# tangent-T/FACL

Measured on AMD Instinct MI355X. Metric: contrastive-step clips/sec (B=32,T=24,N=2048) at 1/2/4/8 MI355X, higher is better.
Workload: dtype f32

## Files before the change

### facl_amd/_lib.py

```python
import ctypes
import os

import torch

_HERE = os.path.dirname(os.path.abspath(__file__))
_LIB = None

c_p = ctypes.c_void_p
c_i = ctypes.c_int
c_f = ctypes.c_float
c_d = ctypes.c_double
c_l = ctypes.c_longlong

SIGNATURES = {
    "facl_version": [],
    "facl_fps_f32": [c_p, c_i, c_i, c_i, c_i, c_p, c_p, c_p],
    "facl_fps_f64": [c_p, c_i, c_i, c_i, c_i, c_p, c_p, c_p],
    "facl_fps_reorder": [c_p, c_i, c_i, c_i, c_p, c_i, c_p, c_p],
    "facl_group": [c_p, c_i, c_i, c_i, c_i, c_i, c_f, c_p, c_p, c_p, c_p],
    "facl_group_clips": [c_p, c_i, c_i, c_i, c_i, c_i, c_i, c_f, c_p, c_p, c_p, c_p],
    "facl_gather_rows": [c_p, c_i, c_i, c_i, c_i, c_p, c_i, c_p, c_p, c_i, c_i, c_p],
    "facl_scatter_rows": [c_p, c_i, c_i, c_i, c_i, c_i, c_p, c_i, c_p, c_p],
    "facl_sinkhorn": [c_p, c_i, c_i, c_i, c_p, c_p, c_p],
    "facl_kmeans": [c_p, c_i, c_i, c_i, c_i, c_p, c_p, c_p, c_p],
# ... 68 lines not shown
    "facl_build_views_resident_gp_f32": [c_p, c_p, c_p, c_i, c_p, c_i, c_i, c_i, c_l, c_i, c_p, c_p, c_p, c_p],
    "facl_build_views_resident_gp_f64": [c_p, c_p, c_p, c_i, c_p, c_i, c_i, c_i, c_l, c_i, c_p, c_p, c_p, c_p],
    "facl_sa_bwd0": [c_p, c_p, c_l, c_p, c_p, c_p, c_p, c_p],
    "facl_sa_bwd1": [c_p, c_l, c_p, c_p, c_p, c_p, c_p, c_p, c_p, c_p, c_p, c_p, c_p],
    "facl_sa_bwd_w3": [c_p, c_l, c_p, c_p, c_p, c_p, c_p, c_p, c_p],
    "facl_sa_bwd2": [c_p, c_p, c_p, c_l, c_i, c_p, c_p, c_p, c_p, c_p, c_p, c_p],
    "facl_sa_bwd_consts3": [c_p, c_p, c_p, c_p, c_d, c_p, c_p, c_p],
    "facl_sa_bwd_consts2": [c_p, c_p, c_d, c_p, c_p],
    "facl_bn_bwd_consts": [c_p, c_p, c_i, c_d, c_p, c_p, c_p, c_p],
    "facl_rows_center_wgrad": [c_p, c_p, c_l, c_i, c_p, c_p, c_p],
    "facl_viewmax_fwd": [c_p, c_i, c_i, c_i, c_p, c_p, c_p],
    "facl_viewmax_bwd": [c_p, c_p, c_i, c_i, c_i, c_p, c_p],
    "facl_viewmax_bwd_add": [c_p, c_p, c_i, c_i, c_i, c_p, c_p],
    "facl_sa_bwd_final": [c_p] * 13 + [c_i, c_d] + [c_p] * 9 + [c_p],
    "facl_viewmax_stack": [c_p, c_i, c_i, c_i, c_p, c_p, c_p],
    "facl_fc_bn_stats": [c_p, c_l, c_l, c_i, c_p, c_p, c_p],
    "facl_fc_bn_apply": [c_p, c_l, c_l, c_i, c_p, c_p, c_i, c_i, c_d, c_d, c_p, c_p, c_f, c_f, c_p, c_p, c_p, c_p, c_p],
    "facl_fc_bn_bwd_stats": [c_p, c_p, c_l, c_l, c_i, c_p, c_p, c_p, c_p],
    "facl_fc_bn_bwd_apply": [c_p, c_p, c_l, c_l, c_i, c_p, c_p, c_p, c_d, c_d, c_p, c_p, c_p, c_p, c_p],
    "facl_col_sums": [c_p, c_l, c_i, c_p, c_p],
    "facl_contrast_pair_sum": [c_p, c_i, c_i, c_i, c_i, c_p, c_i, c_p, c_p, c_p, c_p, c_p],
    "facl_gemm_wgrad_acc": [c_p, c_p, c_l, c_i, c_i, c_i, c_p, c_i, c_p],
    "facl_contrast_pair_sum_mask": [c_p, c_i, c_i, c_i, c_i, c_p, c_i, c_i, c_p, c_p, c_p, c_p, c_p],
    "facl_loss_rows_fwd": [c_p, c_l, c_i, c_i, c_f, c_p, c_p, c_p],
    "facl_loss_rows_bwd": [c_p, c_p, c_p, c_l, c_i, c_i, c_f, c_p, c_p],
    "facl_contrast_pair_queue": [c_p, c_p, c_i, c_i, c_i, c_i, c_i, c_p, c_i, c_i, c_p, c_p, c_p, c_p, c_p, c_p, c_p],
    "facl_queue_push": [c_p, c_i, c_i, c_p, c_i, c_p, c_p],
    "facl_ema_apply": [c_i, c_p, c_p, c_p, c_f, c_p],
    "facl_grad_sqnorm": [c_i, c_p, c_p, c_p, c_p],
    "facl_adam_prep_ex": [c_p, c_p, c_f, c_f, c_p, c_i, c_d, c_i, c_i, c_i, c_d, c_p, c_p],
    "facl_adamw_apply": [c_i, c_p, c_p, c_p, c_p, c_p, c_p, c_p, c_f, c_f, c_f, c_f, c_p],
    "facl_mailbox_bytes": [c_i, c_i],
    "facl_mailbox_alloc": [c_l, c_p, c_p],
    "facl_mailbox_open": [c_p, c_p],
    "facl_mailbox_close": [c_p],
    "facl_mailbox_free": [c_p],
    "facl_mailbox_allreduce": [c_p, c_p, c_i, c_i, c_p, c_i, c_i, c_p, c_p, c_p],
    "facl_gen3dv_frames": [c_p, c_i, c_i, c_i, c_p, c_p, c_p, c_p],
    "facl_gen3dv_voxelise": [c_p, c_i, c_i, c_i, c_p, c_p, c_p, c_p, c_i, c_i, c_i, c_l, c_l, c_d, c_p, c_p, c_p, c_p, c_p],
    "facl_gen3dv_volumes": [c_p, c_p, c_p, c_p, c_i, c_i, c_l, c_p, c_p, c_p],
    "facl_gen3dv_filter": [c_p, c_p, c_p, c_i, c_i, c_l, c_i, c_i, c_p, c_p, c_p],
    "facl_gen3dv_compact": [c_p, c_p, c_p, c_p, c_i, c_i, c_l, c_p, c_p, c_p],
    "facl_gen3dv_sample": [c_p, c_p, c_p, c_p, c_p, c_i, c_i, c_l, c_p, c_l, c_i, c_p, c_p, c_p, c_p, c_p, c_p],
    "facl_gen3dv_app": [c_p, c_i, c_i, c_i, c_p, c_p, c_p, c_l, c_p, c_i, c_p, c_l, c_i, c_p, c_p, c_p, c_i, c_i, c_l, c_d,
                        c_p, c_p, c_p, c_p, c_p],
    "facl_knn_ws_bytes": [c_i, c_i, c_i],
    "facl_knn_topk": [c_p, c_i, c_i, c_p, c_i, c_i, c_i, c_i, c_p, c_p, c_p, c_p, c_p],
    "facl_knn_vote": [c_p, c_p, c_p, c_i, c_i, c_i, c_i, c_f, c_p, c_p, c_p],
    "facl_cls_gather_norm_fwd": [c_p, c_i, c_i, c_i, c_p, c_p, c_p],
    "facl_cls_gather_norm_bwd": [c_p, c_p, c_p, c_i, c_i, c_i, c_p, c_p],
    "facl_softmax_ce": [c_p, c_i, c_p, c_i, c_i, c_p, c_p, c_p, c_p, c_p],
    "facl_cls_probs_acc": [c_p, c_i, c_i, c_i, c_p, c_i, c_p],
    "facl_cls_topk": [c_p, c_i, c_i, c_i, c_i, c_p, c_p, c_p, c_p, c_p],
}
RESTYPE_I64 = {"facl_ws_bytes", "facl_gemm_rs_planes_bytes", "facl_mailbox_bytes", "facl_knn_ws_bytes"}


def lib_path():
    return os.environ.get("FACL_LIB") or os.path.join(_HERE, "libfacl_hip.so")


def load_library():
    global _LIB
    if _LIB is not None:
        return _LIB
    path = lib_path()
    if not os.path.exists(path):
        raise RuntimeError(
            f"{path} not found: facl_amd has no CPU/eager fallback. Build it with "
            "`python -m facl_amd.build` (hipcc --offload-arch=gfx950).")
    lib = ctypes.CDLL(path)
    for name, argtypes in SIGNATURES.items():
        fn = getattr(lib, name)
        fn.argtypes = argtypes
        fn.restype = ctypes.c_longlong if name in RESTYPE_I64 else ctypes.c_int
    _LIB = lib
    return lib


_ERR = {-1: "unsupported shape", -2: "NULL pointer", -3: "misaligned pointer", -4: "unsupported configuration"}


def check(rc, what):
    if rc != 0:
        msg = _ERR.get(rc, f"hipError {rc}")
        raise RuntimeError(f"{what} failed: {msg} (code {rc})")


AMAX_WORDS = 2048

SA_D_MIN, SA_D_MAX = 3, 8


def sa_l1_cols(D):
    return 8 if D <= 4 else 12


def sa_bwd2_out(D):
    return 64 * 64 + 64 * sa_l1_cols(D)


def amax_buffers(n, device, zero=True):
    if zero:
        return torch.zeros((n, AMAX_WORDS), dtype=torch.int32, device=device)
    return empty((n, AMAX_WORDS), dtype=torch.int32, device=device)


def ptr(t):
# ... 145 lines not shown
```

### facl_amd/cn3d_model_conbag.py

```python
import math

import torch
import torch.nn as nn

from . import sa_mlp
from . import tail as _tail

nstates_plus_1 = [64, 64, 256]
nstates_plus_2 = [128, 128, 256]
nstates_plus_3 = [256, 512, 1024, 1024, 1024]


class _Affine(nn.Module):

    def __init__(self, shape, fan_in, bias=True):
        super().__init__()
        self.weight = nn.Parameter(torch.empty(shape))
        nn.init.kaiming_uniform_(self.weight, a=math.sqrt(5))
        if bias:
            self.bias = nn.Parameter(torch.empty(shape[0]))
            bound = 1 / math.sqrt(fan_in) if fan_in > 0 else 0
            nn.init.uniform_(self.bias, -bound, bound)
        else:
            self.register_parameter("bias", None)
# ... 65 lines not shown
        if self.pooling == "concatenation":
            self.dim_out = 1024
        self._pool_K = _knn_K
        self._pool_S = self.sample_num_level2 if _sample_num_level1 is None else _sample_num_level1

        self.net3DV_1 = _conv_stack(self.INPUT_FEATURE_NUM, nstates_plus_1)
        self.net3DV_3 = _conv_stack(3 + nstates_plus_2[2], nstates_plus_3[:3])
        self.netR_FC = _Slots([(0, _Affine((nstates_plus_3[4], self.dim_out), self.dim_out)),
                               (1, _BatchNormState(nstates_plus_3[4])),
                               (3, _Affine((self.dim, nstates_plus_3[4]), nstates_plus_3[4]))])
        self.mapping = _Affine((self.num_clusters, self.dim), self.dim, bias=False)
        self.bn_reduce_fn = None

    def _sa_args(self):
        n = self.net3DV_1
        params = [n[0].weight, n[0].bias, n[1].weight, n[1].bias, n[3].weight, n[3].bias, n[4].weight, n[4].bias,
                  n[6].weight, n[6].bias, n[7].weight, n[7].bias]
        buffers = {"rm1": n[1].running_mean, "rv1": n[1].running_var, "rm2": n[4].running_mean,
                   "rv2": n[4].running_var, "rm3": n[7].running_mean, "rv3": n[7].running_var}
        return params, buffers

    def forward(self, xt, yt, loss_mode=0):
        if xt.dim() != 4 or yt.dim() != 4:
            raise ValueError("expected xt (M,D,S,K) and yt (M,3,S,1)")
        M, D, S, K = xt.shape
        if D != self.INPUT_FEATURE_NUM:
            raise RuntimeError("input has %d channels, model was built for %d" % (D, self.INPUT_FEATURE_NUM))
        if K != self._pool_K:
            raise RuntimeError("pooling window is %d neighbours, got K=%d" % (self._pool_K, K))
        if S != self._pool_S:
            raise RuntimeError("model pools over %d centroids, got S=%d" % (self._pool_S, S))
        if M % self.gost:
            raise RuntimeError("first dim (%d) must be gost*batch with gost=%d" % (M, self.gost))
        x_rows = xt.permute(0, 2, 3, 1)
        x_rows = x_rows.contiguous().view(M * S * K, D).float()
        centers = yt.permute(0, 2, 1, 3).reshape(M * S, 3)
        training = self.training

        params, buffers = self._sa_args()
        prec = getattr(self, "precision", "f32")
        state = dict(training=training, buffers=buffers, reduce_fn=self.bn_reduce_fn, K=K, precision=prec)
        pooled = sa_mlp.SAMLPFunction.apply(x_rows, state, *params)
        if training:
            for i in (1, 4, 7):
                self.net3DV_1[i].count_batch()
        with _tail.precision(prec):
            return self._tail_forward(pooled, centers, M, S, training, state.get("pooled_amax"))

    def _tail_forward(self, pooled, centers, M, S, training, pooled_amax=None):

        n3 = self.net3DV_3
        widths = (n3[0].weight.shape[1] - 3, n3[0].weight.shape[0], n3[3].weight.shape[0], n3[6].weight.shape[0])
        if _tail.net3dv3_supported(pooled.shape[0], widths, S, _tail.current_precision()):
            x_pre = _tail.net3dv3(pooled, centers, n3, training, S, self.bn_reduce_fn, pooled_amax)
        else:
            h = _tail.linear_bn_relu(pooled, n3[0], n3[1], training, self.bn_reduce_fn, centers=centers)
            h = _tail.linear_bn_relu(h, n3[3], n3[4], training, self.bn_reduce_fn)
            x_pre = _tail.linear_bn_relu_segmax(h, n3[6], n3[7], training, S, self.bn_reduce_fn)
        fc = self.netR_FC
        stacked = _tail.fc_head(x_pre, self.gost, fc[0], fc[1], fc[3], training, self.bn_reduce_fn)
        self._stacked = stacked
        x, x_global = stacked[:M], stacked[M:]
        x_nor, code = _tail.normalize_map(x, self.mapping.weight, lazy=bool(getattr(self, "lazy_code", False)))
        return x, code, x_nor, x_global


class PointNet_Plus_fine(PointNet_Plus):

    def __init__(self, opt, num_clusters=64, gost=10, dim=512, sample_num_level1=32, knn_K=128,
                 normalize_input=True):
        super().__init__(opt, num_clusters=num_clusters, gost=gost, dim=dim, normalize_input=normalize_input,
                         _sample_num_level1=sample_num_level1, _knn_K=knn_K)
```

### facl_amd/csrc/common.h

```cpp
#pragma once
#include <hip/hip_runtime.h>
#include <stdint.h>
#include <stdlib.h>
#include "../../include/facl_hip.h"

#define FACL_WAVE 64

static inline int facl_launch_status() {
    hipError_t e = hipGetLastError();
    return e == hipSuccess ? 0 : (int)e;
}

static inline int facl_env_int(const char* name, int dflt) {
    const char* v = getenv(name);
    return v ? atoi(v) : dflt;
}

static inline int facl_set_dynamic_lds(bool (&done)[64], const void* const* fns, int nfns, int bytes) {
    int dev = 0;
    if (hipGetDevice(&dev) != hipSuccess || dev < 0 || dev >= 64) dev = 0;
    if (done[dev]) return 0;
    for (int i = 0; i < nfns; ++i) {
        hipError_t e = hipFuncSetAttribute(fns[i], hipFuncAttributeMaxDynamicSharedMemorySize, bytes);
        if (e != hipSuccess) return (int)e;
// ... 50 lines not shown

__device__ __forceinline__ double wave_sum_f64(double v) {
#pragma unroll
    for (int o = 32; o > 0; o >>= 1) v += __shfl_xor(v, o, 64);
    return v;
}

typedef float f32x16 __attribute__((ext_vector_type(16)));
typedef float f32x32 __attribute__((ext_vector_type(32)));
#define MFMA32(a, b, c) __builtin_amdgcn_mfma_f32_32x32x2f32((a), (b), (c), 0, 0, 0)
__device__ __forceinline__ constexpr int rowmap(int r, int h) { return (r & 3) + 8 * (r >> 2) + 4 * h; }

#define FACL_UNIT 64
#define FACL_UNIT_ELEMS 4096

template <int D>
__device__ __forceinline__ float l1_chain(const float4* row, const float (&xv)[8]) {
    const float4 w0 = row[0], w1 = row[1];
    const float w[8] = {w0.x, w0.y, w0.z, w0.w, w1.x, w1.y, w1.z, w1.w};
    float v = fmaf(w[0], xv[0], row[2].x);
#pragma unroll
    for (int i = 1; i < D; ++i) v = fmaf(w[i], xv[i], v);
    return v;
}

#define FACL_WS_ROWS 4096
#define FACL_WS_TICKET_BYTES 4096

typedef __bf16 bf16x8 __attribute__((ext_vector_type(8)));
typedef __bf16 bf16x2v __attribute__((ext_vector_type(2)));
typedef float f32x2v __attribute__((ext_vector_type(2)));
#define MFMA_BF16(a, b, c) __builtin_amdgcn_mfma_f32_32x32x16_bf16((a), (b), (c), 0, 0, 0)
#define FACL_SB_PA {2, 0, 1, 1, 0, 0}
#define FACL_SB_PB {0, 2, 1, 0, 1, 0}
#define FACL_SB3_PA {0, 1, 0}
#define FACL_SB3_PB {1, 0, 0}

__device__ __forceinline__ unsigned pk_bf16(float x0, float x1) {
    const f32x2v v = {x0, x1};
    return __builtin_bit_cast(unsigned, __builtin_convertvector(v, bf16x2v));
}
__device__ __forceinline__ float sub_f32(float a, float b) {
    float d;
    asm("v_sub_f32 %0, %1, %2" : "=v"(d) : "v"(a), "v"(b));
    return d;
}
__device__ __forceinline__ void split_pair(float x0, float x1, unsigned& hi, unsigned& mi, unsigned& lo) {
    hi = pk_bf16(x0, x1);
    const float r0 = sub_f32(x0, __builtin_bit_cast(float, hi << 16)), r1 = sub_f32(x1, __builtin_bit_cast(float, hi & 0xffff0000u));
    mi = pk_bf16(r0, r1);
    const float s0 = sub_f32(r0, __builtin_bit_cast(float, mi << 16)), s1 = sub_f32(r1, __builtin_bit_cast(float, mi & 0xffff0000u));
    lo = pk_bf16(s0, s1);
}
__device__ __forceinline__ bf16x8 as_bf16x8(unsigned a, unsigned b, unsigned c, unsigned d) {
    const uint4 u = make_uint4(a, b, c, d);
    return __builtin_bit_cast(bf16x8, u);
}

typedef _Float16 f16x8h __attribute__((ext_vector_type(8)));
typedef _Float16 f16x2h __attribute__((ext_vector_type(2)));
#define MFMA_F16(a, b, c) __builtin_amdgcn_mfma_f32_32x32x16_f16((a), (b), (c), 0, 0, 0)
#define FACL_H3_PA {1, 0, 0}
#define FACL_H3_PB {0, 1, 0}
#define FACL_AMAX_SLOTS 64
#define FACL_AMAX_STRIDE 32
static_assert(FACL_AMAX_SLOTS * FACL_AMAX_STRIDE == FACL_AMAX_WORDS, "amax buffer layout");

__device__ __forceinline__ void split_pair_h(float x0, float x1, unsigned& hi, unsigned& lo) {
    const f32x2v v = {x0, x1};
    const f16x2h h = __builtin_convertvector(v, f16x2h);
    hi = __builtin_bit_cast(unsigned, h);
    float r0, r1;
    asm("v_fma_mix_f32 %0, %1, -1.0, %2 op_sel:[0,0,0] op_sel_hi:[1,0,0]" : "=v"(r0) : "v"(hi), "v"(x0));
    asm("v_fma_mix_f32 %0, %1, -1.0, %2 op_sel:[1,0,0] op_sel_hi:[1,0,0]" : "=v"(r1) : "v"(hi), "v"(x1));
    const f32x2v r = {r0, r1};
    lo = __builtin_bit_cast(unsigned, __builtin_convertvector(r, f16x2h));
}
__device__ __forceinline__ f16x8h as_f16x8(unsigned a, unsigned b, unsigned c, unsigned d) {
    const uint4 u = make_uint4(a, b, c, d);
    return __builtin_bit_cast(f16x8h, u);
}

__device__ __forceinline__ int h3_se(unsigned b) {
    int se = 267 - (int)((b >> 23) & 0xff);
    se = se > 167 ? 167 : se;
    return se < 87 ? 87 : se;
}
__device__ __forceinline__ int h3_se_wide(unsigned b) {
    int se = 267 - (int)((b >> 23) & 0xff);
    se = se > 207 ? 207 : se;
    return se < 47 ? 47 : se;
}
__device__ __forceinline__ float pow2_biased(int e) { return __uint_as_float((unsigned)e << 23); }
template <int CTRL, int RMASK>
__device__ __forceinline__ float facl_dpp_max_step(float v) {
    const int o = __builtin_amdgcn_update_dpp(__builtin_bit_cast(int, v), __builtin_bit_cast(int, v), CTRL, RMASK, 0xf, false);
    return fmaxf(v, __builtin_bit_cast(float, o));
}
__device__ __forceinline__ float facl_wave_max_nonneg(float v) {
    v = facl_dpp_max_step<0x111, 0xf>(v); v = facl_dpp_max_step<0x112, 0xf>(v); v = facl_dpp_max_step<0x114, 0xf>(v);
    v = facl_dpp_max_step<0x118, 0xf>(v); v = facl_dpp_max_step<0x142, 0xa>(v); v = facl_dpp_max_step<0x143, 0xc>(v);
    return __builtin_bit_cast(float, __builtin_amdgcn_readlane(__builtin_bit_cast(int, v), 63));
}

__device__ __forceinline__ float h3_unscale(int seA, int seB) { return pow2_biased(381 - seA - seB); }
__device__ __forceinline__ unsigned amax_bits(const unsigned* amax) {
// ... 21 lines not shown
```

### facl_amd/csrc/fchead.hip

```cpp
#include "rows_common.h"

namespace {

constexpr int FC_SL = 32;

__device__ __forceinline__ void fc_slice(int s, int M, int R, int na, int& r0, int& r1, int& seg) {
    if (s < na) { seg = 0; r0 = s * FC_SL; r1 = r0 + FC_SL < M ? r0 + FC_SL : M; }
    else { seg = 1; r0 = M + (s - na) * FC_SL; r1 = r0 + FC_SL < R ? r0 + FC_SL : R; }
    if (r0 > r1) r0 = r1;
}

__global__ __launch_bounds__(256) void k_fc_stats(const float* __restrict__ y, int M, int R, int na, int C4,
                                                  double* __restrict__ part) {
    const int lane = threadIdx.x & 63, ph = threadIdx.x >> 6;
    const int c4 = blockIdx.x * 64 + lane;
    __shared__ double red[3][64][8];
    int r0, r1, seg;
    fc_slice(blockIdx.y, M, R, na, r0, r1, seg);
    double acc[8] = {};
    if (c4 < C4)
        for (int r = r0 + ph; r < r1; r += 4)
            lane_each<4>([&](int e, float v) { acc[2 * e] += (double)v; acc[2 * e + 1] += (double)v * (double)v; },
                         reinterpret_cast<const float4*>(y)[(size_t)r * C4 + c4]);
    if (phase_sum(acc, red, lane, ph, c4 < C4)) {
// ... 4 lines not shown
}

__global__ void k_fc_reduce(const double* __restrict__ part, int na, int nb, int V, double* __restrict__ sums2) {
    const int v = blockIdx.x * blockDim.x + threadIdx.x;
    if (v >= V) return;
    double a = 0, b = 0;
    for (int s = 0; s < na; ++s) a += part[(size_t)s * V + v];
    for (int s = na; s < na + nb; ++s) b += part[(size_t)s * V + v];
    sums2[v] = a;
    sums2[V + v] = b;
}

__device__ __forceinline__ void fc_slice_sums(const double* __restrict__ part, int na, int nb, int C, int c, int ph, double (&acc)[4]) {
    const int V = 2 * C;
    if (c >= C) return;
    for (int t = ph; t < na; t += 4) { acc[0] += part[(size_t)t * V + 2 * c]; acc[1] += part[(size_t)t * V + 2 * c + 1]; }
    for (int t = na + ph; t < na + nb; t += 4) { acc[2] += part[(size_t)t * V + 2 * c]; acc[3] += part[(size_t)t * V + 2 * c + 1]; }
}

__global__ __launch_bounds__(256) void k_fc_finalize(const double* __restrict__ part, int na, int nb, int C, double count_a,
                                                     double count_b, const float* __restrict__ gamma, const float* __restrict__ beta,
                                                     float eps, float momentum, float* __restrict__ running_mean,
                                                     float* __restrict__ running_var, float* __restrict__ bnc2) {
    const int lane = threadIdx.x & 63, ph = threadIdx.x >> 6;
    const int c = blockIdx.x * 64 + lane;
    __shared__ double red[3][64][4];
    double acc[4] = {};
    fc_slice_sums(part, na, nb, C, c, ph, acc);
    if (!phase_sum(acc, red, lane, ph, c < C)) return;
    const double g = gamma[c], b = beta[c];
    float rm = running_mean ? running_mean[c] : 0.f, rv = running_var ? running_var[c] : 0.f;
#pragma unroll
    for (int seg = 0; seg < 2; ++seg) {
        const double s = acc[2 * seg], q = acc[2 * seg + 1];
        const double count = seg ? count_b : count_a;
        const double mean = s / count;
        double var = q / count - mean * mean;
        if (var < 0) var = 0;
        const double invstd = 1.0 / sqrt(var + (double)eps);
        float* o = bnc2 + (size_t)seg * 5 * C;
        o[c] = (float)mean;
        o[C + c] = (float)invstd;
        o[2 * C + c] = (float)(g * invstd);
        o[3 * C + c] = (float)(b - mean * g * invstd);
        o[4 * C + c] = g < 0 ? -1.0f : 1.0f;
        const double unb = count > 1 ? var * count / (count - 1) : var;
        rm = (float)((1.0 - momentum) * rm + momentum * mean);
        rv = (float)((1.0 - momentum) * rv + momentum * unb);
    }
    if (running_mean) { running_mean[c] = rm; running_var[c] = rv; }
}

__global__ __launch_bounds__(256) void k_fc_apply(const float* __restrict__ y, int M, int R, int C4,
                                                  const float* __restrict__ bnc2, float* __restrict__ out) {
    const int c4 = blockIdx.x * 256 + threadIdx.x;
    if (c4 >= C4) return;
    const int C = 4 * C4;
    const float4 sa = reinterpret_cast<const float4*>(bnc2 + 2 * C)[c4], ta = reinterpret_cast<const float4*>(bnc2 + 3 * C)[c4];
    const float4 sb = reinterpret_cast<const float4*>(bnc2 + 7 * C)[c4], tb = reinterpret_cast<const float4*>(bnc2 + 8 * C)[c4];
    for (int r = blockIdx.y; r < R; r += gridDim.y) {
        const float4 sc = r < M ? sa : sb, sh = r < M ? ta : tb;
        reinterpret_cast<float4*>(out)[(size_t)r * C4 + c4] = lane_map<4>(bn_relu, sc, reinterpret_cast<const float4*>(y)[(size_t)r * C4 + c4], sh);
    }
}

__global__ __launch_bounds__(256) void k_fc_bwd_stats(const float* __restrict__ dout, const float* __restrict__ y, int M, int R,
                                                      int na, int C4, const float* __restrict__ bnc2, double* __restrict__ part) {
    const int lane = threadIdx.x & 63, ph = threadIdx.x >> 6;
    const int c4 = blockIdx.x * 64 + lane;
    __shared__ double red[3][64][8];
    int r0, r1, seg;
    fc_slice(blockIdx.y, M, R, na, r0, r1, seg);
    double acc[8] = {};
    if (c4 < C4) bn_bwd_stats_rows<4>(dout, y, C4, c4, bnc2 + (size_t)seg * 20 * C4, r0 + ph, r1, 4, acc);
    if (phase_sum(acc, red, lane, ph, c4 < C4)) {
        double* pr = part + (size_t)blockIdx.y * 8 * C4 + 8 * c4;
#pragma unroll
        for (int e = 0; e < 8; ++e) pr[e] = acc[e];
    }
}

__global__ __launch_bounds__(256) void k_fc_bwd_consts(const double* __restrict__ part, int na, int nb,
                                                       const double* __restrict__ sums_g, int C, double count_a, double count_b,
                                                       float* __restrict__ dbeta, float* __restrict__ dgamma,
                                                       float* __restrict__ kk2) {
    const int lane = threadIdx.x & 63, ph = threadIdx.x >> 6;
    const int c = blockIdx.x * 64 + lane;
    const int V = 2 * C;
    __shared__ double red[3][64][4];
    double acc[4] = {};
    fc_slice_sums(part, na, nb, C, c, ph, acc);
    if (!phase_sum(acc, red, lane, ph, c < C)) return;
#pragma unroll
    for (int seg = 0; seg < 2; ++seg) {
        const double g0 = sums_g ? sums_g[(size_t)seg * V + 2 * c] : acc[2 * seg];
        const double g1 = sums_g ? sums_g[(size_t)seg * V + 2 * c + 1] : acc[2 * seg + 1];
        const float inv = (float)(1.0 / (seg ? count_b : count_a));
        kk2[(size_t)seg * V + c] = (float)g0 * inv;
        kk2[(size_t)seg * V + C + c] = (float)g1 * inv;
    }
    dbeta[c] = (float)acc[0] + (float)acc[2];
    dgamma[c] = (float)acc[1] + (float)acc[3];
}

__global__ __launch_bounds__(256) void k_fc_bwd_apply(const float* __restrict__ dout, const float* __restrict__ y, int M, int R,
                                                      int C4, const float* __restrict__ bnc2, const float* __restrict__ kk2,
                                                      float* __restrict__ dy) {
    const int c4 = blockIdx.x * 256 + threadIdx.x;
    if (c4 >= C4) return;
    const int C = 4 * C4;
    const BnLanes<4> q[2] = {bn_lanes<4>(bnc2, C, c4), bn_lanes<4>(bnc2 + 5 * C, C, c4)};
    const KkLanes<4> k[2] = {kk_lanes<4>(kk2, C, c4), kk_lanes<4>(kk2 + 2 * C, C, c4)};
    for (int r = blockIdx.y; r < R; r += gridDim.y) {
        const int s = r < M ? 0 : 1;
        const size_t o = (size_t)r * C4 + c4;
        reinterpret_cast<float4*>(dy)[o] = lane_map<4>(bn_relu_bwd, reinterpret_cast<const float4*>(dout)[o], reinterpret_cast<const float4*>(y)[o],
                                                       q[s].mean, q[s].inv, q[s].scale, q[s].shift, k[s].k1, k[s].k2);
    }
}

__global__ __launch_bounds__(1024) void k_col_sums(const float* __restrict__ x, int R, int C4, float* __restrict__ out) {
    __shared__ double red[64][16][4];
    const int qd = threadIdx.x & 15, ph = threadIdx.x >> 4;
    const int c4 = blockIdx.x * 16 + qd;
    double a0 = 0, a1 = 0, a2 = 0, a3 = 0;
    if (c4 < C4)
        for (int r = ph; r < R; r += 64) {
            const float4 v = reinterpret_cast<const float4*>(x)[(size_t)r * C4 + c4];
            a0 += (double)v.x; a1 += (double)v.y; a2 += (double)v.z; a3 += (double)v.w;
        }
    red[ph][qd][0] = a0; red[ph][qd][1] = a1; red[ph][qd][2] = a2; red[ph][qd][3] = a3;
    __syncthreads();
    if (ph < 8) {
#pragma unroll
        for (int e = 0; e < 4; ++e) {
            double t = red[ph][qd][e];
#pragma unroll
            for (int k = 1; k < 8; ++k) t += red[ph + 8 * k][qd][e];
            red[ph][qd][e] = t;
        }
    }
    __syncthreads();
    if (ph == 0 && c4 < C4) {
        float o[4];
#pragma unroll
        for (int e = 0; e < 4; ++e) {
            double t = red[0][qd][e];
#pragma unroll
            for (int k = 1; k < 8; ++k) t += red[k][qd][e];
            o[e] = (float)t;
        }
        reinterpret_cast<float4*>(out)[c4] = make_float4(o[0], o[1], o[2], o[3]);
    }
}

__global__ __launch_bounds__(256) void k_viewmax_stack(const float* __restrict__ x, int G, int B, int C4, float* __restrict__ h,
                                                       int* __restrict__ arg) {
    __shared__ float4 sb[3][64];
    __shared__ int4 si[3][64];
    const int it = threadIdx.x & 63, ph = threadIdx.x >> 6;
    const int i = blockIdx.x * 64 + it;
    const bool live = i < B * C4;
    const int b = live ? i / C4 : 0, c4 = live ? i - b * C4 : 0;
    const int per = (G + 3) >> 2;
    const int g0 = ph * per, g1 = g0 + per < G ? g0 + per : G;
    float4 best = make_float4(0.f, 0.f, 0.f, 0.f);
    int4 bi = make_int4(-1, -1, -1, -1);
    if (live && g0 < g1) {
        const size_t o0 = ((size_t)g0 * B + b) * C4 + c4;
        best = reinterpret_cast<const float4*>(x)[o0];
        reinterpret_cast<float4*>(h)[o0] = best;
        bi = make_int4(g0, g0, g0, g0);
        for (int g = g0 + 1; g < g1; ++g) {
            const size_t o = ((size_t)g * B + b) * C4 + c4;
            const float4 v = reinterpret_cast<const float4*>(x)[o];
            reinterpret_cast<float4*>(h)[o] = v;
            first_max_wins(best, bi, v, g);
        }
    }
    if (ph) { sb[ph - 1][it] = best; si[ph - 1][it] = bi; }
    __syncthreads();
    if (ph == 0 && live) {
#pragma unroll
        for (int t = 0; t < 3; ++t) {
            const float4 v = sb[t][it];
            const int4 vi = si[t][it];
            if (vi.x < 0) continue;
            first_max_wins(best, bi, v, vi);
        }
        reinterpret_cast<float4*>(h)[((size_t)G * B + b) * C4 + c4] = best;
        reinterpret_cast<int4*>(arg)[i] = bi;
    }
}

inline bool fc_shape_ok(int64_t M, int64_t R, int C) {
    return M >= FC_SL && !(M % FC_SL) && R > M && R <= 0x7fffffff && C >= 4 && !(C & 3);
}
inline int fc_na(int64_t M) { return (int)(M / FC_SL); }
inline int fc_nb(int64_t M, int64_t R) { return (int)((R - M + FC_SL - 1) / FC_SL); }

}

extern "C" int64_t facl_ws_bytes(void);

extern "C" int facl_fc_bn_stats(const float* y, int64_t M, int64_t R, int C, double* sums2, void* ws, void* stream) {
    if (!y || !ws) return FACL_E_NULL;
    if (!fc_shape_ok(M, R, C)) return FACL_E_CONFIG;
    if (!aligned16(y)) return FACL_E_ALIGN;
    const int na = fc_na(M), nb = fc_nb(M, R);
    if ((size_t)(na + nb) * 2 * C * sizeof(double) > (size_t)facl_ws_bytes()) return FACL_E_CONFIG;
    hipStream_t st = (hipStream_t)stream;
    hipLaunchKernelGGL(k_fc_stats, dim3((C / 4 + 63) / 64, na + nb), dim3(256), 0, st, y, (int)M, (int)R, na, C / 4, (double*)ws);
    if (sums2) hipLaunchKernelGGL(k_fc_reduce, dim3((2 * C + 255) / 256), dim3(256), 0, st, (const double*)ws, na, nb, 2 * C, sums2);
    return facl_launch_status();
}

extern "C" int facl_fc_bn_apply(const float* y, int64_t M, int64_t R, int C, const double* sums2, const double* part,
                                int nslices_a, int nslices_b, double count_a, double count_b, const float* gamma,
                                const float* beta, float eps, float momentum, float* running_mean, float* running_var,
                                float* bnc2, float* a, void* stream) {
    if (!y || !gamma || !beta || !bnc2 || !a || (!sums2 && !part)) return FACL_E_NULL;
    if (M < 1 || R <= M || R > 0x7fffffff || C < 4 || (C & 3) || count_a < 1 || count_b < 1) return FACL_E_SHAPE;
    if (!sums2 && (nslices_a < 1 || nslices_b < 1)) return FACL_E_SHAPE;
    if (!aligned16(y, a, bnc2)) return FACL_E_ALIGN;
    hipStream_t st = (hipStream_t)stream;
    hipLaunchKernelGGL(k_fc_finalize, dim3((C + 63) / 64), dim3(256), 0, st, sums2 ? sums2 : part, sums2 ? 1 : nslices_a,
                       sums2 ? 1 : nslices_b, C, count_a, count_b, gamma, beta, eps, momentum, running_mean, running_var, bnc2);
    const int gx = (C / 4 + 255) / 256;
    int gy = 1024 / gx;
    if (gy > R) gy = (int)R;
    hipLaunchKernelGGL(k_fc_apply, dim3(gx, gy), dim3(256), 0, st, y, (int)M, (int)R, C / 4, bnc2, a);
    return facl_launch_status();
}

extern "C" int facl_fc_bn_bwd_stats(const float* dact, const float* y, int64_t M, int64_t R, int C, const float* bnc2,
                                    double* sums2, void* ws, void* stream) {
    if (!dact || !y || !bnc2 || !ws) return FACL_E_NULL;
    if (!fc_shape_ok(M, R, C)) return FACL_E_CONFIG;
    if (!aligned16(y, dact, bnc2)) return FACL_E_ALIGN;
    const int na = fc_na(M), nb = fc_nb(M, R);
    if ((size_t)(na + nb) * 2 * C * sizeof(double) > (size_t)facl_ws_bytes()) return FACL_E_CONFIG;
    hipStream_t st = (hipStream_t)stream;
    hipLaunchKernelGGL(k_fc_bwd_stats, dim3((C / 4 + 63) / 64, na + nb), dim3(256), 0, st, dact, y, (int)M, (int)R, na, C / 4, bnc2,
                       (double*)ws);
    if (sums2) hipLaunchKernelGGL(k_fc_reduce, dim3((2 * C + 255) / 256), dim3(256), 0, st, (const double*)ws, na, nb, 2 * C, sums2);
    return facl_launch_status();
}

extern "C" int facl_fc_bn_bwd_apply(const float* dact, const float* y, int64_t M, int64_t R, int C, const float* bnc2,
                                    const double* sums2_g, const void* ws, double count_a, double count_b, float* dgamma,
                                    float* dbeta, float* kk2, float* dy, void* stream) {
    if (!dact || !y || !bnc2 || !ws || !dgamma || !dbeta || !kk2 || !dy) return FACL_E_NULL;
    if (!fc_shape_ok(M, R, C)) return FACL_E_CONFIG;
    if (count_a < 1 || count_b < 1) return FACL_E_SHAPE;
    if (!aligned16(y, dact, bnc2, kk2, dy)) return FACL_E_ALIGN;
    const int na = fc_na(M), nb = fc_nb(M, R);
    hipStream_t st = (hipStream_t)stream;
    hipLaunchKernelGGL(k_fc_bwd_consts, dim3((C + 63) / 64), dim3(256), 0, st, (const double*)ws, na, nb, sums2_g, C, count_a,
                       count_b, dbeta, dgamma, kk2);
    const int gx = (C / 4 + 255) / 256;
    int gy = 1024 / gx;
    if (gy > R) gy = (int)R;
    hipLaunchKernelGGL(k_fc_bwd_apply, dim3(gx, gy), dim3(256), 0, st, dact, y, (int)M, (int)R, C / 4, bnc2, kk2, dy);
    return facl_launch_status();
}

extern "C" int facl_col_sums(const float* x, int64_t R, int C, float* out, void* stream) {
    if (!x || !out) return FACL_E_NULL;
    if (R < 1 || R > 0x7fffffff || C < 4 || (C & 3)) return FACL_E_SHAPE;
    if (!aligned16(x, out)) return FACL_E_ALIGN;
    hipLaunchKernelGGL(k_col_sums, dim3((C / 4 + 15) / 16), dim3(1024), 0, (hipStream_t)stream, x, (int)R, C / 4, out);
    return facl_launch_status();
}

extern "C" int facl_viewmax_stack(const float* x, int G, int B, int C, float* h, int32_t* arg, void* stream) {
    if (!x || !h || !arg) return FACL_E_NULL;
    if (G < 1 || B < 1 || C < 4 || (C & 3)) return FACL_E_SHAPE;
    if (!aligned16(x, h, arg)) return FACL_E_ALIGN;
    const int n = B * (C / 4);
    hipLaunchKernelGGL(k_viewmax_stack, dim3((n + 63) / 64), dim3(256), 0, (hipStream_t)stream, x, G, B, C / 4, h, arg);
    return facl_launch_status();
}
```

### facl_amd/csrc/gemm.hip

```cpp
#include "common.h"

int facl_reduce_rows(const double* part, int rows, int V, double* out, hipStream_t st);

namespace {

constexpr int BK = 32;
constexpr int LDK = BK + 4;
enum { KC = 0, IC = 1 };

struct GemmArgs {
    const float* A = nullptr; int lda = 0;
    const float* B = nullptr; int ldb = 0;
    float* C = nullptr; int ldc = 0;
    int MI = 0, NJ = 0, KK = 0;
    const float* bias = nullptr;
    const float* pscale = nullptr; const float* pshift = nullptr;
    const float* xa = nullptr; const float* xb = nullptr; int ldxb = 0;
    double* part = nullptr;
    int kchunk = 0;
    const float* sgn = nullptr; float* smax = nullptr; int* sarg = nullptr;
    int prec = 0;
    const unsigned* amax = nullptr;
    const unsigned* amax_b = nullptr;
    int accum = 0;
};

template <int LAY, int T>
__device__ __forceinline__ void load_tile(const float* __restrict__ P, int ld, int idx0, int nidx, int k0, int kend,
                                          float4 (&r)[2 * T], int tid) {
    if (LAY == IC) {
#pragma unroll
        for (int i = 0; i < 2 * T; ++i) {
            const int k = k0 + tid / (16 * T) + (16 / T) * i, idx = idx0 + 4 * (tid % (16 * T));
            if (k < kend && idx + 3 < nidx) r[i] = *reinterpret_cast<const float4*>(P + (size_t)k * ld + idx);
            else {
                float t[4];
#pragma unroll
                for (int e = 0; e < 4; ++e) t[e] = (k < kend && idx + e < nidx) ? P[(size_t)k * ld + idx + e] : 0.f;
                r[i] = make_float4(t[0], t[1], t[2], t[3]);
            }
        }
    } else {
#pragma unroll
        for (int i = 0; i < 2 * T; ++i) {
            const int idx = idx0 + (tid >> 3) + 32 * i, k = k0 + 4 * (tid & 7);
            if (idx < nidx && k + 3 < kend) r[i] = *reinterpret_cast<const float4*>(P + (size_t)idx * ld + k);
            else {
                float t[4];
#pragma unroll
                for (int e = 0; e < 4; ++e) t[e] = (idx < nidx && k + e < kend) ? P[(size_t)idx * ld + k + e] : 0.f;
                r[i] = make_float4(t[0], t[1], t[2], t[3]);
            }
        }
    }
}

template <int LAY, bool PRO, int TT>
__device__ __forceinline__ void store_tile(float* __restrict__ T, const float4 (&r)[2 * TT], int tid, int k0,
                                           const float* __restrict__ ps, const float* __restrict__ pt) {
    constexpr int LDT = 64 * TT + 4;
    if (LAY == IC) {
#pragma unroll
        for (int i = 0; i < 2 * TT; ++i) {
            const int k = tid / (16 * TT) + (16 / TT) * i;
            *reinterpret_cast<float4*>(&T[k * LDT + 4 * (tid % (16 * TT))]) = r[i];
        }
    } else {
#pragma unroll
        for (int i = 0; i < 2 * TT; ++i) {
            const int k = 4 * (tid & 7), il = (tid >> 3) + 32 * i;
            float v[4] = {r[i].x, r[i].y, r[i].z, r[i].w};
            if (PRO) {
                const float4 s = *reinterpret_cast<const float4*>(ps + k0 + k);
                const float4 t = *reinterpret_cast<const float4*>(pt + k0 + k);
                v[0] = relu_nan(fmaf(s.x, v[0], t.x)); v[1] = relu_nan(fmaf(s.y, v[1], t.y));
                v[2] = relu_nan(fmaf(s.z, v[2], t.z)); v[3] = relu_nan(fmaf(s.w, v[3], t.w));
            }
// ... 417 lines not shown
        }
}
template <int T, int NP>
__device__ __forceinline__ void write_tile_ic8(unsigned short* __restrict__ S, const unsigned (&pk)[12 * T], int tid) {
    constexpr int PLANE = 64 * T * SBROW;
    const int il = tid % (64 * T), kc = tid / (64 * T);
#pragma unroll
    for (int i = 0; i < T; ++i) {
        unsigned short* d = S + il * SBROW + 8 * (kc + (4 / T) * i);
#pragma unroll
        for (int p = 0; p < (NP == 4 ? 2 : NP); ++p)
            *reinterpret_cast<uint4*>(d + p * PLANE) =
                make_uint4(pk[12 * i + 4 * p], pk[12 * i + 4 * p + 1], pk[12 * i + 4 * p + 2], pk[12 * i + 4 * p + 3]);
    }
}

template <bool PRO, int T, int NP>
__device__ __forceinline__ void split_tile_kc4(const float4 (&r)[2 * T], unsigned (&pk)[12 * T], int tid, int k0,
                                               const float* __restrict__ ps, const float* __restrict__ pt, float sc = 1.f) {
#pragma unroll
    for (int i = 0; i < 2 * T; ++i) {
        float v[4] = {r[i].x, r[i].y, r[i].z, r[i].w};
        if (PRO) {
            const int k = 4 * (tid & 7);
            const float4 s = *reinterpret_cast<const float4*>(ps + k0 + k);
            const float4 t = *reinterpret_cast<const float4*>(pt + k0 + k);
            v[0] = relu_nan(fmaf(s.x, v[0], t.x)); v[1] = relu_nan(fmaf(s.y, v[1], t.y));
            v[2] = relu_nan(fmaf(s.z, v[2], t.z)); v[3] = relu_nan(fmaf(s.w, v[3], t.w));
        }
        if (NP == 4) {
            split_pair_h(v[0] * sc, v[1] * sc, pk[6 * i], pk[6 * i + 2]);
            split_pair_h(v[2] * sc, v[3] * sc, pk[6 * i + 1], pk[6 * i + 3]);
        } else if (NP >= 2) {
            split_pair(v[0], v[1], pk[6 * i], pk[6 * i + 2], pk[6 * i + 4]);
            split_pair(v[2], v[3], pk[6 * i + 1], pk[6 * i + 3], pk[6 * i + 5]);
        } else {
            pk[6 * i] = pk_f16(v[0], v[1]);
            pk[6 * i + 1] = pk_f16(v[2], v[3]);
        }
    }
}
template <int T, int NP>
__device__ __forceinline__ void write_tile_kc4(unsigned short* __restrict__ S, const unsigned (&pk)[12 * T], int tid) {
    constexpr int PLANE = 64 * T * SBROW;
#pragma unroll
    for (int i = 0; i < 2 * T; ++i) {
        unsigned short* d = S + ((tid >> 3) + 32 * i) * SBROW + 4 * (tid & 7);
#pragma unroll
        for (int p = 0; p < (NP == 4 ? 2 : NP); ++p) *reinterpret_cast<uint2*>(d + p * PLANE) = make_uint2(pk[6 * i + 2 * p], pk[6 * i + 2 * p + 1]);
    }
}


template <int LAY, int T, int NP, bool PRO>
struct SplitOperand {
    static constexpr int NPL = NP == 4 ? 2 : NP;
    static constexpr int PLANE = 64 * T * SBROW;
    const float* P; int ld, idx0, nidx;
    const float* ps; const float* pt;
    float psi = 1.f, pti = 0.f;
    float4 r4[2 * T];
    float r8[8 * T];
    unsigned pk[12 * T];
    __device__ __forceinline__ SplitOperand(const float* P_, int ld_, int idx0_, int nidx_, const float* ps_, const float* pt_, int tid)
        : P(P_), ld(ld_), idx0(idx0_), nidx(nidx_), ps(ps_), pt(pt_) {
        if (PRO && LAY == IC) {
            int j = idx0 + tid % (64 * T);
            j = j < nidx ? j : nidx - 1;
            psi = ps[j]; pti = pt[j];
        }
    }
    template <bool FULL>
    __device__ __forceinline__ void fetch(int k0, int kend, int tid) {
        if (LAY == KC) load_tile_kc4<T, FULL>(P, ld, idx0, nidx, k0, kend, r4, tid);
        else load_tile_ic8<T, FULL>(P, ld, idx0, nidx, k0, kend, r8, tid);
    }
    __device__ __forceinline__ float absmax() const {
        float m = 0.f;
        if (LAY == KC) {
#pragma unroll
            for (int i = 0; i < 2 * T; ++i) m = fmaxf(fmaxf(m, fmaxf(fabsf(r4[i].x), fabsf(r4[i].y))), fmaxf(fabsf(r4[i].z), fabsf(r4[i].w)));
        } else {
#pragma unroll
            for (int i = 0; i < 8 * T; ++i) m = fmaxf(m, fabsf(r8[i]));
        }
        return m;
    }
    __device__ __forceinline__ void split(int k0, float sc, int tid) {
        if (LAY == KC) split_tile_kc4<PRO, T, NP>(r4, pk, tid, k0, ps, pt, sc);
        else split_tile_ic8<T, NP, PRO>(r8, pk, psi, pti, sc);
    }
    __device__ __forceinline__ void write(unsigned short* S, int tid) const {
        if (LAY == KC) write_tile_kc4<T, NP>(S, pk, tid);
        else write_tile_ic8<T, NP>(S, pk, tid);
    }
    static __device__ __forceinline__ bf16x8 frag(const unsigned short* S, int p, int row, int kk, int h) {
        return *reinterpret_cast<const bf16x8*>(S + p * PLANE + row * SBROW + 16 * kk + 8 * h);
    }
};

template <class OA, class OB>
__device__ __forceinline__ void fetch_stage(OA& A, OB& B, int k0, int kend, int tid) {
    if (k0 + BK <= kend) { A.template fetch<true>(k0, kend, tid); B.template fetch<true>(k0, kend, tid); }
    else { A.template fetch<false>(k0, kend, tid); B.template fetch<false>(k0, kend, tid); }
}

template <int NP, int TM, int TN, class OA, class OB>
__device__ __forceinline__ void mfma_block(const unsigned short* sA, const unsigned short* sB, int kk, int wr, int wc, int q, int h,
                                           f32x16 (&acc)[TM][TN]) {
    constexpr int NPL = OA::NPL;
    bf16x8 af[TM][NPL], bf[TN][NPL];
#pragma unroll
    for (int a = 0; a < TM; ++a)
#pragma unroll
        for (int p = 0; p < NPL; ++p) af[a][p] = OA::frag(sA, p, 32 * TM * wr + 32 * a + q, kk, h);
#pragma unroll
    for (int b = 0; b < TN; ++b)
#pragma unroll
        for (int p = 0; p < NPL; ++p) bf[b][p] = OB::frag(sB, p, 32 * TN * wc + 32 * b + q, kk, h);
    constexpr int PA6[6] = FACL_SB_PA, PB6[6] = FACL_SB_PB, PA3[3] = FACL_SB3_PA, PB3[3] = FACL_SB3_PB, HA[3] = FACL_H3_PA, HB[3] = FACL_H3_PB;
#pragma unroll
    for (int t = 0; t < (NP == 3 ? 6 : NP == 1 ? 1 : 3); ++t)
#pragma unroll
        for (int a = 0; a < TM; ++a)
#pragma unroll
            for (int b = 0; b < TN; ++b) {
                if constexpr (NP == 4) acc[a][b] = MFMA_F16(__builtin_bit_cast(f16x8h, af[a][HA[t]]), __builtin_bit_cast(f16x8h, bf[b][HB[t]]), acc[a][b]);
                else if constexpr (NP == 1) acc[a][b] = MFMA_F16(__builtin_bit_cast(f16x8h, af[a][0]), __builtin_bit_cast(f16x8h, bf[b][0]), acc[a][b]);
                else acc[a][b] = MFMA_BF16(af[a][NP == 3 ? PA6[t] : PA3[t]], bf[b][NP == 3 ? PB6[t] : PB3[t]], acc[a][b]);
            }
}

template <int LA, int LB, bool PRO, int TM, int TN, int NP = 3>
__global__ __launch_bounds__(256, NP == 1 ? 3 : 2) void k_gemm_sb(GemmArgs g) {
    constexpr int BM = 64 * TM, BN = 64 * TN;
    constexpr int APL = BM * SBROW, BPL = BN * SBROW;
    constexpr int STG = NP == 1 ? 4 * 32 * (32 * TN + 4) : 4 * (32 * TM) * (32 * TN + 4);
    static_assert(NP != 4 || (LA == IC && LB == IC), "fp16x3 is wired for the weight gradient (both operands idx-contiguous)");
    constexpr int TILE_F = ((NP == 1 ? 1 : NP == 4 ? 2 : 3) * (APL + BPL) * 2 + 3) / 4;
    constexpr int SMEM = TILE_F > STG ? TILE_F : STG;
    __shared__ __attribute__((aligned(16))) float smem[SMEM];
    unsigned short* const sA = reinterpret_cast<unsigned short*>(smem);
    unsigned short* const sB = sA + (NP == 1 ? 1 : NP == 4 ? 2 : 3) * APL;
    const int tid = threadIdx.x, lane = tid & 63, wave = tid >> 6, h = lane >> 5, q = lane & 31;
    const int wr = wave >> 1, wc = wave & 1;
    const TileId tile = xcd_tile();
    float sca = 1.f, scb = 1.f, uns = 1.f;
    if (NP == 4) {
        const int seA = h3_se_wide_of(g.amax), seB = h3_se_of(g.amax_b);
        sca = pow2_biased(seA); scb = pow2_biased(seB); uns = h3_unscale(seA, seB);
    }
    const int i0 = tile.y * BM, j0 = tile.x * BN;
    const int kbeg = tile.z * g.kchunk;
    const int kend = (kbeg + g.kchunk < g.KK) ? kbeg + g.kchunk : g.KK;

    f32x16 acc[TM][TN];
#pragma unroll
    for (int a = 0; a < TM; ++a)
#pragma unroll
        for (int b = 0; b < TN; ++b)
#pragma unroll
            for (int r = 0; r < 16; ++r) acc[a][b][r] = 0.f;

    using OpA = SplitOperand<LA, TM, NP, PRO && LA == KC>;
    using OpB = SplitOperand<LB, TN, NP, PRO && LA == IC && LB == IC>;
    OpA opa(g.A, g.lda, i0, g.MI, g.pscale, g.pshift, tid);
    OpB opb(g.B, g.ldb, j0, g.NJ, g.pscale, g.pshift, tid);
    auto fetch = [&](int k0) { fetch_stage(opa, opb, k0, kend, tid); };
    auto split = [&](int k0) { opa.split(k0, sca, tid); opb.split(k0, scb, tid); };
    auto write = [&]() { opa.write(sA, tid); opb.write(sB, tid); };
    auto mfma = [&](int kk) { mfma_block<NP, TM, TN, OpA, OpB>(sA, sB, kk, wr, wc, q, h, acc); };
    fetch(kbeg);
    split(kbeg);
    write();
    __syncthreads();
    for (int k0 = kbeg; k0 < kend; k0 += BK) {
        const int kn = (k0 + BK < kend) ? k0 + BK : k0;
        fetch(kn);
        __builtin_amdgcn_sched_barrier(0);
        mfma(0);
        __builtin_amdgcn_sched_barrier(0);
        mfma(1);
        split(kn);
        __syncthreads();
        write();
        __syncthreads();
    }
    if constexpr (NP == 4) {
#pragma unroll
        for (int a = 0; a < TM; ++a)
#pragma unroll
            for (int b = 0; b < TN; ++b)
#pragma unroll
                for (int r = 0; r < 16; ++r) acc[a][b][r] *= uns;
    }
    if constexpr (NP == 1) gemm_epilogue_h<TM, TN>(g, acc, smem, i0, j0, wave, lane, tile.y, tile.z);
    else gemm_epilogue<TM, TN>(g, acc, smem, i0, j0, wave, lane, tile.y, tile.z);
}

template <int LA, int LB, bool PRO, int NP, int KG>
__global__ __launch_bounds__(256 * KG, 1) void k_gemm_sbk(GemmArgs g) {
    constexpr int NPL = NP == 4 ? 2 : NP;
    constexpr int PL = 64 * SBROW;
    constexpr int TILE_F = NPL * 2 * PL * 2 / 4;
    constexpr int STG = 4 * 32 * 36;
    constexpr int MXOFF = KG * TILE_F > STG + (KG - 1) * 4096 ? KG * TILE_F : STG + (KG - 1) * 4096;
    static_assert(NP != 4 || !PRO, "the self-scaled form takes the maximum of the raw registers: no prologue");
    extern __shared__ __attribute__((aligned(16))) float smem[];
    const int grp = __builtin_amdgcn_readfirstlane((int)(threadIdx.x >> 8));
    const int tid = threadIdx.x & 255, lane = tid & 63, wave = tid >> 6, h = lane >> 5, q = lane & 31;
    const int wr = wave >> 1, wc = wave & 1;
    unsigned short* const sA = reinterpret_cast<unsigned short*>(smem + grp * TILE_F);
    unsigned short* const sB = sA + NPL * PL;
    const TileId tile = xcd_tile();
    const int i0 = tile.y * 64, j0 = tile.x * 64;
    const int kbeg = tile.z * g.kchunk;
    const int kend = (kbeg + g.kchunk < g.KK) ? kbeg + g.kchunk : g.KK;
    const int nst = (kend - kbeg + BK - 1) / BK, nit = (nst + KG - 1) / KG;

    f32x16 acc[1][1];
#pragma unroll
    for (int r = 0; r < 16; ++r) acc[0][0][r] = 0.f;

    using OpA = SplitOperand<LA, 1, NP, PRO && LA == KC>;
    using OpB = SplitOperand<LB, 1, NP, PRO && LA == IC && LB == IC>;
    OpA opa(g.A, g.lda, i0, g.MI, g.pscale, g.pshift, tid);
    OpB opb(g.B, g.ldb, j0, g.NJ, g.pscale, g.pshift, tid);
    auto fetch = [&](int k0) { fetch_stage(opa, opb, k0, kend, tid); };
    float* const mxs = smem + MXOFF;
    float uns_nxt = 1.f;
    auto split = [&](int k0) {
        float sca = 1.f, scb = 1.f;
        if constexpr (NP == 4) {
            float ma = facl_wave_max_nonneg(opa.absmax()), mb = facl_wave_max_nonneg(opb.absmax());
            if (lane == 0) { mxs[(grp * 4 + wave) * 2] = ma; mxs[(grp * 4 + wave) * 2 + 1] = mb; }
            __syncthreads();
            const float4 m01 = *reinterpret_cast<const float4*>(mxs + grp * 8), m23 = *reinterpret_cast<const float4*>(mxs + grp * 8 + 4);
            ma = fmaxf(fmaxf(m01.x, m01.z), fmaxf(m23.x, m23.z));
            mb = fmaxf(fmaxf(m01.y, m01.w), fmaxf(m23.y, m23.w));
            const int seA = h3_se(__float_as_uint(ma)), seB = h3_se(__float_as_uint(mb));
            sca = pow2_biased(seA); scb = pow2_biased(seB);
            uns_nxt = h3_unscale(seA, seB);
        }
        opa.split(k0, sca, tid); opb.split(k0, scb, tid);
    };
    auto write = [&]() { opa.write(sA, tid); opb.write(sB, tid); };
    f32x16 stg_acc[1][1];
    auto mfma = [&](int kk) { mfma_block<NP, 1, 1, OpA, OpB>(sA, sB, kk, wr, wc, q, h, NP == 4 ? stg_acc : acc); };
    auto kof = [&](int it) {
        int s = grp + KG * it;
        s = s < nst ? s : nst - 1;
        return kbeg + s * BK;
    };
    { const int k0 = kof(0); fetch(k0); split(k0); write(); }
    __syncthreads();
    float uns_cur = uns_nxt;
    for (int it = 0; it < nit; ++it) {
        const int kn = kof(it + 1 < nit ? it + 1 : it);
        fetch(kn);
        if (grp + KG * it < nst) {
            if constexpr (NP == 4) {
#pragma unroll
                for (int r = 0; r < 16; ++r) stg_acc[0][0][r] = 0.f;
            }
            mfma(0);
            mfma(1);
            if constexpr (NP == 4) {
#pragma unroll
                for (int r = 0; r < 16; ++r) acc[0][0][r] = fmaf(stg_acc[0][0][r], uns_cur, acc[0][0][r]);
            }
        }
        split(kn);
        if constexpr (NP != 4) __syncthreads();
        write();
        __syncthreads();
        uns_cur = uns_nxt;
    }
    float* red = smem + STG;
    if (grp > 0) {
#pragma unroll
        for (int r = 0; r < 16; ++r) red[(grp - 1) * 4096 + wave * 1024 + r * 64 + lane] = acc[0][0][r];
    }
    __syncthreads();
    if (grp > 0) return;
#pragma unroll
    for (int gg = 0; gg < KG - 1; ++gg)
#pragma unroll
        for (int r = 0; r < 16; ++r) acc[0][0][r] += red[gg * 4096 + wave * 1024 + r * 64 + lane];
    gemm_epilogue<1, 1>(g, acc, smem, i0, j0, wave, lane, tile.y, tile.z);
}

constexpr int SBK_KG = 4;
template <int LA, int LB, bool PRO, int NP>
int launch_sbk(const GemmArgs& g, int nz, hipStream_t st) {
    constexpr int TILE_F = (NP == 4 ? 2 : NP) * 2 * 64 * SBROW * 2 / 4, STG = 4 * 32 * 36;
    constexpr int F = SBK_KG * TILE_F > STG + (SBK_KG - 1) * 4096 ? SBK_KG * TILE_F : STG + (SBK_KG - 1) * 4096;
    constexpr int lds = (F + SBK_KG * 8) * 4;
    const dim3 grid((g.NJ + 63) / 64, (g.MI + 63) / 64, nz);
    return facl_launch_dynamic_lds<k_gemm_sbk<LA, LB, PRO, NP, SBK_KG>>(grid, dim3(256 * SBK_KG), lds, st, g);
}

bool use_f32_mfma() {
    static const int use_f32 = facl_env_int("FACL_GEMM_F32", 0);
    return use_f32 != 0;
}

enum TileFamily { SBK, T128, T64 };
struct TileChoice { TileFamily family; int rows_per_part; bool fills128; };
TileChoice choose_tile(const GemmArgs& g, int nz) {
    static const int nosbk = facl_env_int("FACL_GEMM_NOSBK", 0);
    const long long t64 = (long long)((g.NJ + 63) / 64) * ((g.MI + 63) / 64) * nz;
    const bool fills128 = (long long)((g.NJ + 127) / 128) * ((g.MI + 127) / 128) * nz >= 256;
    if (!nosbk && t64 <= 320 && g.kchunk >= 2 * SBK_KG * BK) return {SBK, 32, fills128};
    return fills128 ? TileChoice{T128, 64, true} : TileChoice{T64, 32, false};
}

template <int LA, int LB, bool PRO, int NP>
int launch_split(const GemmArgs& g, int nz, const TileChoice& tc, hipStream_t st) {
    if (tc.family == SBK) return launch_sbk<LA, LB, PRO, NP>(g, nz, st);
    if (tc.family == T128)
        hipLaunchKernelGGL((k_gemm_sb<LA, LB, PRO, 2, 2, NP>), dim3((g.NJ + 127) / 128, (g.MI + 127) / 128, nz), dim3(256), 0, st, g);
    else hipLaunchKernelGGL((k_gemm_sb<LA, LB, PRO, 1, 1, NP>), dim3((g.NJ + 63) / 64, (g.MI + 63) / 64, nz), dim3(256), 0, st, g);
    return facl_launch_status();
}

template <int LA, int LB, bool PRO>
int launch(const GemmArgs& g, int nz, hipStream_t st, int* rows_per_part) {
    const TileChoice tc = choose_tile(g, nz);
    if (rows_per_part) *rows_per_part = tc.rows_per_part;
    if (g.prec == 1) return launch_split<LA, LB, PRO, 1>(g, nz, tc, st);
    if (g.prec == 2) return launch_split<LA, LB, PRO, 2>(g, nz, tc, st);
    if (!use_f32_mfma()) {
        if constexpr (!PRO) {
            static const int sbk_h3 = facl_env_int("FACL_SBK_H3", 0);
            if (tc.family == SBK && sbk_h3) return launch_sbk<LA, LB, false, 4>(g, nz, st);
        }
        return launch_split<LA, LB, PRO, 3>(g, nz, tc, st);
    }
    static const int use_dma = facl_env_int("FACL_GEMM_DMA", 1);
    const bool dma_ok = use_dma && !PRO && LA == IC && LB == IC && !(g.lda & 3) && !(g.ldb & 3) && !(g.MI & 3) &&
                        !(g.NJ & 3) && !(((uintptr_t)g.A | (uintptr_t)g.B) & 15);
    if (rows_per_part) *rows_per_part = tc.fills128 ? 64 : 32;
    if (tc.fills128) {
        const dim3 grid((g.NJ + 127) / 128, (g.MI + 127) / 128, nz);
        if (dma_ok) hipLaunchKernelGGL((k_gemm_dma<LA, LB, 2, 2>), grid, dim3(256), 0, st, g);
        else hipLaunchKernelGGL((k_gemm<LA, LB, PRO, 2, 2>), grid, dim3(256), 0, st, g);
    } else {
        const dim3 grid((g.NJ + 63) / 64, (g.MI + 63) / 64, nz);
        if (dma_ok) hipLaunchKernelGGL((k_gemm_dma<LA, LB, 1, 1>), grid, dim3(256), 0, st, g);
        else hipLaunchKernelGGL((k_gemm<LA, LB, PRO, 1, 1>), grid, dim3(256), 0, st, g);
    }
    return facl_launch_status();
}

__global__ void k_sum_slices(const float* __restrict__ part, int nz, long long n4, float* __restrict__ out) {
    const long long stride = (long long)gridDim.x * blockDim.x;
    const float4* p4 = reinterpret_cast<const float4*>(part);
    for (long long i = (long long)blockIdx.x * blockDim.x + threadIdx.x; i < n4; i += stride) {
        float4 s = p4[i];
        int z = 1;
        for (; z + 3 < nz; z += 4) {
            const float4 v0 = p4[(size_t)z * n4 + i], v1 = p4[(size_t)(z + 1) * n4 + i];
            const float4 v2 = p4[(size_t)(z + 2) * n4 + i], v3 = p4[(size_t)(z + 3) * n4 + i];
            s.x += v0.x; s.y += v0.y; s.z += v0.z; s.w += v0.w;
            s.x += v1.x; s.y += v1.y; s.z += v1.z; s.w += v1.w;
            s.x += v2.x; s.y += v2.y; s.z += v2.z; s.w += v2.w;
            s.x += v3.x; s.y += v3.y; s.z += v3.z; s.w += v3.w;
        }
        for (; z < nz; ++z) {
            const float4 v = p4[(size_t)z * n4 + i];
            s.x += v.x; s.y += v.y; s.z += v.z; s.w += v.w;
        }
        reinterpret_cast<float4*>(out)[i] = s;
    }
}


__global__ __launch_bounds__(256) void k_sum_slices_par(const float* __restrict__ part, int nz, long long n4, float* __restrict__ out) {
    __shared__ float4 red[3][64];
    const int col = threadIdx.x & 63, ph = threadIdx.x >> 6;
    const long long i = (long long)blockIdx.x * 64 + col;
    const float4* p4 = reinterpret_cast<const float4*>(part);
    const int per = (nz + 3) >> 2;
    const int z0 = ph * per, z1 = z0 + per < nz ? z0 + per : nz;
    float4 s = make_float4(0.f, 0.f, 0.f, 0.f);
    if (i < n4) {
        int z = z0;
        for (; z + 3 < z1; z += 4) {
            const float4 v0 = p4[(size_t)z * n4 + i], v1 = p4[(size_t)(z + 1) * n4 + i];
            const float4 v2 = p4[(size_t)(z + 2) * n4 + i], v3 = p4[(size_t)(z + 3) * n4 + i];
            s.x += v0.x; s.y += v0.y; s.z += v0.z; s.w += v0.w;
            s.x += v1.x; s.y += v1.y; s.z += v1.z; s.w += v1.w;
            s.x += v2.x; s.y += v2.y; s.z += v2.z; s.w += v2.w;
            s.x += v3.x; s.y += v3.y; s.z += v3.z; s.w += v3.w;
        }
        for (; z < z1; ++z) {
            const float4 v = p4[(size_t)z * n4 + i];
            s.x += v.x; s.y += v.y; s.z += v.z; s.w += v.w;
        }
    }
    if (ph) red[ph - 1][col] = s;
    __syncthreads();
    if (ph == 0 && i < n4) {
#pragma unroll
        for (int t = 0; t < 3; ++t) { const float4 v = red[t][col]; s.x += v.x; s.y += v.y; s.z += v.z; s.w += v.w; }
        reinterpret_cast<float4*>(out)[i] = s;
    }
}

}

int facl_sum_slices(const float* slices, int nz, long long n4, float* out, bool par_ok, hipStream_t st) {
    static const int par = facl_env_int("FACL_SUM_SLICES_PAR", 1);
    if (par_ok && par && nz >= 8) {
        hipLaunchKernelGGL(k_sum_slices_par, dim3((unsigned)((n4 + 63) / 64)), dim3(256), 0, st, slices, nz, n4, out);
    } else {
        const int grid = (int)((n4 + 255) / 256 < 2048 ? (n4 + 255) / 256 : 2048);
        hipLaunchKernelGGL(k_sum_slices, dim3(grid), dim3(256), 0, st, slices, nz, n4, out);
    }
    return facl_launch_status();
}

template <class LAUNCH>
static int split_k(GemmArgs g, int nz, float* dW, hipStream_t st, LAUNCH launch_kernel) {
    g.kchunk = (int)(((long long)g.KK + nz - 1) / nz);
    g.kchunk = (g.kchunk + BK - 1) / BK * BK;
    nz = (int)(((long long)g.KK + g.kchunk - 1) / g.kchunk);
    if (int rc = launch_kernel(g, nz)) return rc;
    return facl_sum_slices(g.C, nz, (long long)g.MI * g.NJ / 4, dW, true, st);
}

static bool stats_rows_fit(int64_t M, int N, int rows_per_part, int* prow) {
    *prow = (int)((M + 2 * rows_per_part - 1) / (2 * rows_per_part)) * 2;
    return (size_t)*prow * N * 2 * sizeof(double) <= (size_t)facl_ws_bytes() - FACL_WS_TICKET_BYTES;
}

static int gemm_fwd_p(const float* a, int64_t M, int K, const float* W, int ldw, int N, const float* bias,
                      const float* pscale, const float* pshift, const float* centers, const float* Wc,
                      int ldwc, float* y, double* sums, void* ws, void* stream, int prec) {
    if (!a || !W || !y || (sums && !ws)) return FACL_E_NULL;
    if (M < 1 || M > 0x7fffffff || K < 4 || (K & 3) || N < 1 || (ldw & 3)) return FACL_E_SHAPE;
    if ((pscale == nullptr) != (pshift == nullptr) || (centers == nullptr) != (Wc == nullptr)) return FACL_E_NULL;
    hipStream_t st = (hipStream_t)stream;
    GemmArgs g{a, K, W, ldw, y, N, (int)M, N, K};
    g.bias = bias; g.pscale = pscale; g.pshift = pshift;
    g.xa = centers; g.xb = Wc; g.ldxb = ldwc;
    g.part = sums ? (double*)ws : nullptr;
    g.kchunk = K; g.prec = prec;
    int rpp = 64, prow = 0;
    if (sums && !stats_rows_fit(M, N, choose_tile(g, 1).rows_per_part, &prow)) return FACL_E_SHAPE;
    int rc = pscale ? launch<KC, KC, true>(g, 1, st, &rpp) : launch<KC, KC, false>(g, 1, st, &rpp);
    if (rc || !sums) return rc;
    if (!stats_rows_fit(M, N, rpp, &prow)) return FACL_E_SHAPE;
    return facl_reduce_rows((const double*)ws, prow, 2 * N, sums, st);
}

static int gemm_fwd_segmax_p(const float* a, int64_t M, int K, const float* W, int ldw, int N, const float* bias,
                             const float* sgn, float* y, double* sums, float* ymax, int32_t* arg, void* ws,
                             void* stream, int prec) {
    if (!a || !W || !y || !sgn || !ymax || !arg || (sums && !ws)) return FACL_E_NULL;
    if (M < 64 || M > 0x7fffffff || (M & 63) || K < 4 || (K & 3) || N < 1 || (ldw & 3)) return FACL_E_SHAPE;
    GemmArgs g{a, K, W, ldw, y, N, (int)M, N, K};
    g.bias = bias;
    g.part = sums ? (double*)ws : nullptr;
    g.sgn = sgn; g.smax = ymax; g.sarg = arg;
    g.kchunk = K; g.prec = prec;
    const TileChoice tc = choose_tile(g, 1);
    if (tc.family != T128) return FACL_E_CONFIG;
    hipStream_t st = (hipStream_t)stream;
    int rpp = 64, prow = 0;
    if (sums && !stats_rows_fit(M, N, tc.rows_per_part, &prow)) return FACL_E_SHAPE;
    int rc = launch<KC, KC, false>(g, 1, st, &rpp);
    if (rc || !sums) return rc;
    if (!stats_rows_fit(M, N, rpp, &prow)) return FACL_E_SHAPE;
    return facl_reduce_rows((const double*)ws, prow, 2 * N, sums, st);
}

static int gemm_dgrad_p(const float* dy, int64_t M, int N, const float* W, int ldw, int K, float* da,
                        void* stream, int prec) {
    if (!dy || !W || !da) return FACL_E_NULL;
    if (M < 1 || M > 0x7fffffff || N < 4 || (N & 3) || K < 1) return FACL_E_SHAPE;
    GemmArgs g{dy, N, W, ldw, da, K, (int)M, K, N};
    g.kchunk = N; g.prec = prec;
    return launch<KC, IC, false>(g, 1, (hipStream_t)stream, nullptr);
}

static int gemm_wgrad_p(const float* dy, const float* a, int64_t M, int N, int K, int lda, float* dW,
                        float* slices, int nz, void* stream, int prec) {
    if (!dy || !a || !dW || !slices) return FACL_E_NULL;
    if (M < 1 || M > 0x7fffffff || N < 4 || (N & 3) || K < 4 || (K & 3) || nz < 1 || nz > 1024) return FACL_E_SHAPE;
    hipStream_t st = (hipStream_t)stream;
    GemmArgs g{dy, N, a, lda, dW, K, N, K, (int)M};
    g.kchunk = (int)M; g.prec = prec;
    if (M <= 8192 && choose_tile(g, 1).family == SBK) return launch<IC, IC, false>(g, 1, st, nullptr);
    g.C = slices;
    return split_k(g, nz, dW, st, [&](const GemmArgs& gz, int z) { return launch<IC, IC, false>(gz, z, st, nullptr); });
}

static int gemm_wgrad_pro_p(const float* dy, const float* y, int64_t M, int N, int K, int ldy, const float* pscale,
                            const float* pshift, float* dW, float* slices, int nz, void* stream, int prec) {
    if (!dy || !y || !pscale || !pshift || !dW || !slices) return FACL_E_NULL;
    if (M < 1 || M > 0x7fffffff || N < 4 || (N & 3) || K < 4 || (K & 3) || nz < 1 || nz > 1024) return FACL_E_SHAPE;
    if (use_f32_mfma() || prec == 1) return FACL_E_CONFIG;
    hipStream_t st = (hipStream_t)stream;
    GemmArgs g{dy, N, y, ldy, slices, K, N, K, (int)M};
    g.pscale = pscale; g.pshift = pshift; g.prec = prec;
    return split_k(g, nz, dW, st, [&](const GemmArgs& gz, int z) {
        if (choose_tile(gz, z).family != T128) return (int)FACL_E_CONFIG;
        const dim3 grid((K + 127) / 128, (N + 127) / 128, z);
        if (prec == 2) hipLaunchKernelGGL((k_gemm_sb<IC, IC, true, 2, 2, 2>), grid, dim3(256), 0, st, gz);
        else hipLaunchKernelGGL((k_gemm_sb<IC, IC, true, 2, 2, 3>), grid, dim3(256), 0, st, gz);
        return facl_launch_status();
    });
}

extern "C" int facl_gemm_wgrad_h3(const float* dy, const float* y, int64_t M, int N, int K, int ldy, const float* pscale,
                                  const float* pshift, const uint32_t* amax, const uint32_t* amax_b, float* dW, float* slices,
                                  int nz, void* stream) {
    if (!dy || !y || !amax || !amax_b || !dW || !slices || (pscale == nullptr) != (pshift == nullptr)) return FACL_E_NULL;
    if (M < 1 || M > 0x7fffffff || N < 4 || (N & 3) || K < 4 || (K & 3) || nz < 1 || nz > 1024) return FACL_E_SHAPE;
    if (use_f32_mfma()) return FACL_E_CONFIG;
    hipStream_t st = (hipStream_t)stream;
    GemmArgs g{dy, N, y, ldy, slices, K, N, K, (int)M};
    g.pscale = pscale; g.pshift = pshift; g.amax = amax; g.amax_b = amax_b;
    return split_k(g, nz, dW, st, [&](const GemmArgs& gz, int z) {
        if (choose_tile(gz, z).family != T128) return (int)FACL_E_CONFIG;
        const dim3 grid((K + 127) / 128, (N + 127) / 128, z);
        if (pscale) hipLaunchKernelGGL((k_gemm_sb<IC, IC, true, 2, 2, 4>), grid, dim3(256), 0, st, gz);
        else hipLaunchKernelGGL((k_gemm_sb<IC, IC, false, 2, 2, 4>), grid, dim3(256), 0, st, gz);
        return facl_launch_status();
    });
}

extern "C" int facl_gemm_wgrad_pro(const float* dy, const float* y, int64_t M, int N, int K, int ldy, const float* pscale,
                                   const float* pshift, float* dW, float* slices, int nz, void* stream) {
    return gemm_wgrad_pro_p(dy, y, M, N, K, ldy, pscale, pshift, dW, slices, nz, stream, 0);
}
extern "C" int facl_gemm_wgrad_pro_x3(const float* dy, const float* y, int64_t M, int N, int K, int ldy, const float* pscale,
                                      const float* pshift, float* dW, float* slices, int nz, void* stream) {
    return gemm_wgrad_pro_p(dy, y, M, N, K, ldy, pscale, pshift, dW, slices, nz, stream, 2);
}

extern "C" int facl_gemm_fwd(const float* a, int64_t M, int K, const float* W, int ldw, int N, const float* bias,
                             const float* pscale, const float* pshift, const float* centers, const float* Wc,
                             int ldwc, float* y, double* sums, void* ws, void* stream) {
    return gemm_fwd_p(a, M, K, W, ldw, N, bias, pscale, pshift, centers, Wc, ldwc, y, sums, ws, stream, 0);
}
extern "C" int facl_gemm_fwd_f16(const float* a, int64_t M, int K, const float* W, int ldw, int N, const float* bias,
                                 const float* pscale, const float* pshift, const float* centers, const float* Wc,
                                 int ldwc, float* y, double* sums, void* ws, void* stream) {
    return gemm_fwd_p(a, M, K, W, ldw, N, bias, pscale, pshift, centers, Wc, ldwc, y, sums, ws, stream, 1);
}
extern "C" int facl_gemm_fwd_segmax(const float* a, int64_t M, int K, const float* W, int ldw, int N, const float* bias,
                                    const float* sgn, float* y, double* sums, float* ymax, int32_t* arg, void* ws,
                                    void* stream) {
    return gemm_fwd_segmax_p(a, M, K, W, ldw, N, bias, sgn, y, sums, ymax, arg, ws, stream, 0);
}
extern "C" int facl_gemm_fwd_segmax_f16(const float* a, int64_t M, int K, const float* W, int ldw, int N, const float* bias,
                                        const float* sgn, float* y, double* sums, float* ymax, int32_t* arg, void* ws,
                                        void* stream) {
    return gemm_fwd_segmax_p(a, M, K, W, ldw, N, bias, sgn, y, sums, ymax, arg, ws, stream, 1);
}
extern "C" int facl_gemm_dgrad(const float* dy, int64_t M, int N, const float* W, int ldw, int K, float* da, void* stream) {
    return gemm_dgrad_p(dy, M, N, W, ldw, K, da, stream, 0);
}
extern "C" int facl_gemm_dgrad_f16(const float* dy, int64_t M, int N, const float* W, int ldw, int K, float* da, void* stream) {
    return gemm_dgrad_p(dy, M, N, W, ldw, K, da, stream, 1);
}
extern "C" int facl_gemm_wgrad(const float* dy, const float* a, int64_t M, int N, int K, int lda, float* dW,
                               float* slices, int nz, void* stream) {
    return gemm_wgrad_p(dy, a, M, N, K, lda, dW, slices, nz, stream, 0);
}
extern "C" int facl_gemm_wgrad_f16(const float* dy, const float* a, int64_t M, int N, int K, int lda, float* dW,
                                   float* slices, int nz, void* stream) {
    return gemm_wgrad_p(dy, a, M, N, K, lda, dW, slices, nz, stream, 1);
}

extern "C" int facl_gemm_fwd_x3(const float* a, int64_t M, int K, const float* W, int ldw, int N, const float* bias,
                                const float* pscale, const float* pshift, const float* centers, const float* Wc,
                                int ldwc, float* y, double* sums, void* ws, void* stream) {
    return gemm_fwd_p(a, M, K, W, ldw, N, bias, pscale, pshift, centers, Wc, ldwc, y, sums, ws, stream, 2);
}
extern "C" int facl_gemm_fwd_segmax_x3(const float* a, int64_t M, int K, const float* W, int ldw, int N, const float* bias,
                                       const float* sgn, float* y, double* sums, float* ymax, int32_t* arg, void* ws,
                                       void* stream) {
    return gemm_fwd_segmax_p(a, M, K, W, ldw, N, bias, sgn, y, sums, ymax, arg, ws, stream, 2);
}
extern "C" int facl_gemm_dgrad_x3(const float* dy, int64_t M, int N, const float* W, int ldw, int K, float* da, void* stream) {
    return gemm_dgrad_p(dy, M, N, W, ldw, K, da, stream, 2);
}
extern "C" int facl_gemm_wgrad_x3(const float* dy, const float* a, int64_t M, int N, int K, int lda, float* dW,
                                  float* slices, int nz, void* stream) {
    return gemm_wgrad_p(dy, a, M, N, K, lda, dW, slices, nz, stream, 2);
}

extern "C" int facl_gemm_wgrad_acc(const float* dy, const float* a, int64_t M, int N, int K, int lda, float* dW, int prec,
                                   void* stream) {
    if (!dy || !a || !dW) return FACL_E_NULL;
    if (M < 1 || M > 8192 || N < 4 || (N & 3) || K < 4 || (K & 3) || prec < 0 || prec > 2) return FACL_E_SHAPE;
    GemmArgs g{dy, N, a, lda, dW, K, N, K, (int)M};
    g.kchunk = (int)M; g.prec = prec; g.accum = 1;
    if (choose_tile(g, 1).family != SBK) return FACL_E_CONFIG;
    return launch<IC, IC, false>(g, 1, (hipStream_t)stream, nullptr);
}
```

### facl_amd/csrc/gemm_rs.hip

```cpp
#include "rows_common.h"

int facl_reduce_rows(const double* part, int rows, int V, double* out, hipStream_t st);
int facl_sum_slices(const float* slices, int nz, long long n4, float* out, bool par_ok, hipStream_t st);
extern "C" int64_t facl_ws_bytes(void);

namespace {

constexpr int RS_CT = 8;
constexpr int RS_WAVES = 4;
constexpr int RS_WPP = RS_CT * 3 / RS_WAVES;
constexpr int RS_WSLOT = RS_CT * 3 * 1024;
constexpr int RS_ASLOT = 32 * 128;
constexpr int RS_LDS_W = 2 * RS_WSLOT;
constexpr int RS_LDS_A = RS_WAVES * RS_ASLOT;
constexpr int RS_KMAX = 1024;
#ifndef RS_PREP_IN_ODD
#define RS_PREP_IN_ODD 1
#endif
#ifndef RS_H3_AHEAD2
#define RS_H3_AHEAD2 0
#endif
constexpr int RS_KPRO = 512;
constexpr int RS_LDS = RS_LDS_W + RS_LDS_A + 2 * RS_KPRO * 4;

// ... 47 lines not shown
    if (half) {
#pragma unroll
        for (int t = 0; t < RS_PL_ITEMS; ++t)
#pragma unroll
            for (int j = 0; j < 8; ++j) m = fmaxf(m, fabsf(v[t][j]));
#pragma unroll
        for (int o = 32; o > 0; o >>= 1) m = fmaxf(m, __shfl_xor(m, o, 64));
        if ((threadIdx.x & 63) == 0) red[threadIdx.x >> 6] = m;
        __syncthreads();
        m = fmaxf(fmaxf(red[0], red[1]), fmaxf(red[2], red[3]));
        const int se = h3_se(__float_as_uint(m));
        if (threadIdx.x == 0) hdr[ot] = se;
        sw = pow2_biased(se);
    }
#pragma unroll
    for (int t = 0; t < RS_PL_ITEMS; ++t) {
        const int item = threadIdx.x + 256 * t;
        if (item >= nitems) break;
        const int ln = item & 63, ks = item >> 6;
        unsigned hi[4], mi[4], lo[4];
        if (half) {
#pragma unroll
            for (int j = 0; j < 4; ++j) split_pair_h(v[t][2 * j] * sw, v[t][2 * j + 1] * sw, hi[j], lo[j]);
            uint4* d = out + ((long long)(ks * NT + ot) * 2) * 64 + ln;
            d[0] = make_uint4(hi[0], hi[1], hi[2], hi[3]);
            d[64] = make_uint4(lo[0], lo[1], lo[2], lo[3]);
            continue;
        }
#pragma unroll
        for (int j = 0; j < 4; ++j) split_pair(v[t][2 * j], v[t][2 * j + 1], hi[j], mi[j], lo[j]);
        uint4* d = out + ((long long)(ks * NT + ot) * 3) * 64 + ln;
        d[0] = make_uint4(hi[0], hi[1], hi[2], hi[3]);
        d[64] = make_uint4(mi[0], mi[1], mi[2], mi[3]);
        d[128] = make_uint4(lo[0], lo[1], lo[2], lo[3]);
    }
}

__device__ __forceinline__ void rs_absmax_block(const float* __restrict__ x, long long n, unsigned* __restrict__ amax, int b, int nb) {
    float m = 0.f;
    for (long long i = (long long)b * 256 + threadIdx.x; i < n; i += (long long)nb * 256) m = fmaxf(m, fabsf(x[i]));
#pragma unroll
    for (int o = 32; o > 0; o >>= 1) m = fmaxf(m, __shfl_xor(m, o, 64));
    if ((threadIdx.x & 63) == 0)
        atomicMax(amax + ((b * 4 + (threadIdx.x >> 6)) & (FACL_AMAX_SLOTS - 1)) * FACL_AMAX_STRIDE, __float_as_uint(m));
}

__global__ __launch_bounds__(256) void k_rs_planes(const float* __restrict__ W, long long so, long long sc, int NO, int NC,
                                                   const float* __restrict__ xc, int ldxc, uint4* __restrict__ out, int half,
                                                   int* __restrict__ hdr) {
    rs_planes_tile(W, so, sc, NO, NC, xc, ldxc, out, half, hdr, blockIdx.x);
}

constexpr int RS_MAXJOBS = 8;
struct RsPlaneJobs {
    int n;
    const float* W[RS_MAXJOBS]; long long so[RS_MAXJOBS]; long long sc[RS_MAXJOBS]; int NO[RS_MAXJOBS]; int NC[RS_MAXJOBS];
    const float* xc[RS_MAXJOBS]; int ldxc[RS_MAXJOBS]; uint4* out[RS_MAXJOBS]; int* hdr[RS_MAXJOBS]; int first[RS_MAXJOBS + 1];
    int half[RS_MAXJOBS];
    const float* ax; long long an; unsigned* aamax; int anb;
};
__global__ __launch_bounds__(256) void k_rs_planes_multi(RsPlaneJobs jb) {
    if ((int)blockIdx.x >= jb.first[jb.n]) {
        rs_absmax_block(jb.ax, jb.an, jb.aamax, (int)blockIdx.x - jb.first[jb.n], jb.anb);
        return;
    }
    int j = 0;
#pragma unroll
    for (int t = 1; t < RS_MAXJOBS; ++t) j += (t < jb.n && (int)blockIdx.x >= jb.first[t]) ? 1 : 0;
    rs_planes_tile(jb.W[j], jb.so[j], jb.sc[j], jb.NO[j], jb.NC[j], jb.xc[j], jb.ldxc[j], jb.out[j], jb.half[j], jb.hdr[j],
                   (int)blockIdx.x - jb.first[j]);
}

struct RsTile { int x, y; };
__device__ __forceinline__ RsTile rs_tile() {
    const int nbx = gridDim.x;
    const int L = facl_xcd_tile(blockIdx.x + nbx * blockIdx.y, nbx * gridDim.y);
    RsTile t;
    t.x = L % nbx; t.y = L / nbx;
    return t;
}

__device__ __forceinline__ void rs_dma16(const void* gsrc, unsigned lds_dst) {
    unsigned keep;
    asm volatile("s_mov_b32 %0, m0\n\ts_mov_b32 m0, %2\n\ts_nop 0\n\tglobal_load_lds_dwordx4 %1, off\n\ts_mov_b32 m0, %0"
                 : "=&s"(keep) : "v"(gsrc), "s"(lds_dst) : "memory");
}
__device__ __forceinline__ unsigned lds_addr(const void* p) {
    return (unsigned)(uintptr_t)(const __attribute__((address_space(3))) char*)p;
}

template <bool PRO, bool SEG, bool BST, bool H3 = false, int WV = RS_WAVES>
__global__ __launch_bounds__(64 * WV, WV == 8 ? 1 : 2) void k_gemm_rs(RsArgs g) {
    constexpr int NPL = H3 ? 2 : 3;
    constexpr int WPP = RS_CT * NPL / WV;
    extern __shared__ __attribute__((aligned(16))) char lds[];
    if ((int)(blockIdx.x + gridDim.x * blockIdx.y) < g.first_round) facl_phase_wait(g.phase_ticks);
    const int tid = threadIdx.x, lane = tid & 63, h = lane >> 5, q = lane & 31;
    const int wave = __builtin_amdgcn_readfirstlane(tid >> 6);
    char* const wring = lds;
    char* const abuf = lds + RS_LDS_W + wave * RS_ASLOT;
    float* const tab = reinterpret_cast<float*>(lds + RS_LDS_W + WV * RS_ASLOT);
    const unsigned wring_a = __builtin_amdgcn_readfirstlane(lds_addr(wring));
    const unsigned abuf_a = __builtin_amdgcn_readfirstlane(lds_addr(abuf));
    const RsTile tile = rs_tile();
    const int cb = tile.x;
    const int row0 = (tile.y * WV + wave) * 32;
    const int nks = g.K >> 4, nst = g.K >> 5;
    const int nks_all = nks + (g.centers ? 1 : 0);
    int seA = 127;
    if (H3) seA = h3_se_wide_of(g.amax);
    const float sA = pow2_biased(seA);


    const uint4* wsrc = g.Wp + ((size_t)(RS_CT * cb) * NPL + wave * WPP) * 64 + lane;
// ... 525 lines not shown
    static const int w8 = facl_env_int("FACL_RS_W8", 0);
    return (h3 && w8) ? 8 : RS_WAVES;
}

template <bool PRO, bool SEG, bool BST, bool H3, int WV>
int rs_launch_k(const RsArgs& g, hipStream_t st) {
    const dim3 grid(g.N / 256, (g.M + 32 * WV - 1) / (32 * WV));
    return facl_launch_dynamic_lds<k_gemm_rs<PRO, SEG, BST, H3, WV>>(grid, dim3(64 * WV), WV == 8 ? RS_LDS8 : RS_LDS, st, g);
}
template <bool H3, int WV>
int rs_launch_form(const RsArgs& g, hipStream_t st) {
    if (g.by) return rs_launch_k<false, false, true, H3, WV>(g, st);
    if (g.pscale && g.smax) return rs_launch_k<true, true, false, H3, WV>(g, st);
    if (g.pscale) return rs_launch_k<true, false, false, H3, WV>(g, st);
    if (g.smax) return rs_launch_k<false, true, false, H3, WV>(g, st);
    return rs_launch_k<false, false, false, H3, WV>(g, st);
}

int rs_launch(const RsArgs& g0, hipStream_t st) {
    RsArgs g = g0;
    {
        static const int per_ks = facl_env_int("FACL_RS_PHASE", 30);
        const long long wgs = (long long)(g.N / 256) * ((g.M + 32 * rs_waves(g.h3) - 1) / (32 * rs_waves(g.h3)));
        g.first_round = 512;
        g.phase_ticks = (per_ks > 0 && wgs > g.first_round && rs_waves(g.h3) == RS_WAVES) ? per_ks * (g.K >> 4) + 500 : 0;
    }
    if (rs_waves(g.h3) == 8) return rs_launch_form<true, 8>(g, st);
    return g.h3 ? rs_launch_form<true, RS_WAVES>(g, st) : rs_launch_form<false, RS_WAVES>(g, st);
}

}

static int64_t rs_planes_only_bytes(int N, int K, int with_centers) {
    return (int64_t)(K / 16 + (with_centers ? 1 : 0)) * (N / 32) * 3 * 64 * 16;
}
extern "C" int64_t facl_gemm_rs_planes_bytes(int N, int K, int with_centers) {
    if (N < 32 || K < 16) return 0;
    return rs_planes_only_bytes(N, K, with_centers) + (((int64_t)(N / 32) * 4 + 255) / 256) * 256;
}

extern "C" int facl_gemm_rs_planes(const float* W, int ldw, int N, int K, int transposed, const float* Wc, int ldwc,
                                   int half, void* planes, void* stream) {
    if (!W || !planes) return FACL_E_NULL;
    if (N < 1 || K < 1 || ldw < K) return FACL_E_SHAPE;
    const int NO = transposed ? K : N, NC = transposed ? N : K;
    if ((NO & 31) || (NC & 15) || (transposed && Wc) || NC / 16 + (Wc ? 1 : 0) > RS_PL_ITEMS * 4) return FACL_E_SHAPE;
    const long long so = transposed ? 1 : ldw, sc = transposed ? ldw : 1;
    int* hdr = (int*)((char*)planes + rs_planes_only_bytes(NO, NC, Wc ? 1 : 0));
    hipLaunchKernelGGL(k_rs_planes, dim3(NO / 32), dim3(256), 0, (hipStream_t)stream, W, so, sc, NO, NC, Wc, ldwc, (uint4*)planes,
                       half ? 1 : 0, hdr);
    return facl_launch_status();
}

extern "C" int facl_gemm_rs_planes_multi(int n, const float* const* W, const int* ldw, const int* N, const int* K,
                                         const int* transposed, const float* const* Wc, const int* ldwc, const int* half,
                                         void* const* planes, const float* absmax_x, int64_t absmax_n, uint32_t* absmax_amax,
                                         void* stream) {
    if (!W || !ldw || !N || !K || !transposed || !Wc || !ldwc || !half || !planes) return FACL_E_NULL;
    if ((absmax_x == nullptr) != (absmax_amax == nullptr)) return FACL_E_NULL;
    if (n < 1 || n > RS_MAXJOBS || (absmax_x && absmax_n < 1)) return FACL_E_SHAPE;
    RsPlaneJobs jb;
    jb.n = n;
    jb.first[0] = 0;
    for (int j = 0; j < RS_MAXJOBS; ++j) {
        if (j >= n) { jb.W[j] = nullptr; jb.xc[j] = nullptr; jb.out[j] = nullptr; jb.hdr[j] = nullptr; jb.so[j] = jb.sc[j] = 0; jb.NO[j] = jb.NC[j] = 32; jb.ldxc[j] = 0; jb.half[j] = 0; jb.first[j + 1] = jb.first[j]; continue; }
        if (!W[j] || !planes[j]) return FACL_E_NULL;
        if (N[j] < 1 || K[j] < 1 || ldw[j] < K[j]) return FACL_E_SHAPE;
        const int NO = transposed[j] ? K[j] : N[j], NC = transposed[j] ? N[j] : K[j];
        if ((NO & 31) || (NC & 15) || (transposed[j] && Wc[j]) || NC / 16 + (Wc[j] ? 1 : 0) > RS_PL_ITEMS * 4) return FACL_E_SHAPE;
        jb.W[j] = W[j]; jb.so[j] = transposed[j] ? 1 : ldw[j]; jb.sc[j] = transposed[j] ? ldw[j] : 1;
        jb.NO[j] = NO; jb.NC[j] = NC; jb.xc[j] = Wc[j]; jb.ldxc[j] = ldwc[j]; jb.out[j] = (uint4*)planes[j];
        jb.hdr[j] = (int*)((char*)planes[j] + rs_planes_only_bytes(NO, NC, Wc[j] ? 1 : 0));
        jb.half[j] = half[j] ? 1 : 0;
        jb.first[j + 1] = jb.first[j] + NO / 32;
    }
    jb.ax = absmax_x; jb.an = absmax_n; jb.aamax = absmax_amax;
    jb.anb = absmax_x ? (int)((absmax_n + 4095) / 4096 < 16 ? (absmax_n + 4095) / 4096 : 16) : 0;
    hipLaunchKernelGGL(k_rs_planes_multi, dim3(jb.first[n] + jb.anb), dim3(256), 0, (hipStream_t)stream, jb);
    return facl_launch_status();
}

extern "C" int facl_gemm_rs_supported(int64_t M, int K, int N) {
    return (M >= 2048 && M <= 0x7fffffff && K >= 64 && K <= RS_KMAX && !(K & 31) && N >= 256 && !(N & 255)) ? 1 : 0;
}

extern "C" int facl_gemm_rs_fwd(const float* a, int64_t M, int K, const void* planes, int half, const uint32_t* amax_a, int N,
                                const float* bias, const float* pscale, const float* pshift, const float* centers, float* y,
                                double* sums, const float* sgn, float* ymax, int32_t* arg, void* ws, void* stream) {
    if (!a || !planes || !y || (sums && !ws) || (half && !amax_a)) return FACL_E_NULL;
    if (!facl_gemm_rs_supported(M, K, N)) return FACL_E_SHAPE;
    if ((pscale == nullptr) != (pshift == nullptr)) return FACL_E_NULL;
    if (pscale && K > RS_KPRO) return FACL_E_SHAPE;
    if ((sgn == nullptr) != (ymax == nullptr) || (sgn == nullptr) != (arg == nullptr)) return FACL_E_NULL;
    if (sgn && (M & 63)) return FACL_E_SHAPE;
    if (((uintptr_t)a | (uintptr_t)planes) & 15) return FACL_E_ALIGN;
    const int rpw = 32 * rs_waves(half ? 1 : 0);
    const int prow = (int)((M + rpw - 1) / rpw);
    if (sums && (size_t)prow * N * 2 * sizeof(double) > ((size_t)facl_ws_bytes() - FACL_WS_TICKET_BYTES)) return FACL_E_SHAPE;
    hipStream_t st = (hipStream_t)stream;
    const int* wse = (const int*)((const char*)planes + rs_planes_only_bytes(N, K, centers ? 1 : 0));
    RsArgs g{a, K, (int)M, K, (const uint4*)planes, N / 32, N};
    g.C = y; g.ldc = N;
    g.bias = bias; g.pscale = pscale; g.pshift = pshift; g.centers = centers;
    g.part = sums ? (double*)ws : nullptr;
    g.sgn = sgn; g.smax = ymax; g.sarg = arg;
    g.h3 = half ? 1 : 0; g.amax = amax_a; g.wse = wse;
    int rc = rs_launch(g, st);
    if (rc || !sums) return rc;
    return facl_reduce_rows((const double*)ws, prow, 2 * N, sums, st);
}

extern "C" int facl_gemm_rs_dgrad(const float* dy, int64_t M, int N, const void* planes, int half, const uint32_t* amax,
                                  int K, float* da, void* stream) {
    if (!dy || !planes || !da || (half && !amax)) return FACL_E_NULL;
    if (!facl_gemm_rs_supported(M, N, K)) return FACL_E_SHAPE;
    if (((uintptr_t)dy | (uintptr_t)planes) & 15) return FACL_E_ALIGN;
    const int* wse = (const int*)((const char*)planes + rs_planes_only_bytes(K, N, 0));
    RsArgs g{dy, N, (int)M, N, (const uint4*)planes, K / 32, K};
    g.C = da; g.ldc = K;
    g.h3 = half ? 1 : 0; g.amax = amax; g.wse = wse;
    return rs_launch(g, (hipStream_t)stream);
}

extern "C" int facl_gemm_rs_dgrad_bnstats(const float* dy, int64_t M, int N, const void* planes, int half,
                                          const uint32_t* amax, int K, float* da, const float* y, const float* bnc,
                                          double* sums, void* ws, void* stream) {
    if (!dy || !planes || !da || !y || !bnc || !sums || !ws || (half && !amax)) return FACL_E_NULL;
    if (!facl_gemm_rs_supported(M, N, K)) return FACL_E_SHAPE;
    if (((uintptr_t)dy | (uintptr_t)planes) & 15) return FACL_E_ALIGN;
    const int rpw = 32 * rs_waves(half ? 1 : 0);
    const int prow = (int)((M + rpw - 1) / rpw);
    if ((size_t)prow * K * 2 * sizeof(double) > ((size_t)facl_ws_bytes() - FACL_WS_TICKET_BYTES)) return FACL_E_SHAPE;
// ... 51 lines not shown
```

### facl_amd/tail.py

```python
import os
import threading

import torch

from . import _lib
from .sa_mlp import BN_EPS, BN_MOMENTUM, _Workspace, _bn_eval, _bn_finalize, act_amax_eval


PRECISIONS = ("f32", "f16", "x3", "x3b")
_SUFFIX = {"f32": "", "f16": "_f16", "x3": "_x3", "x3b": ""}
_LABEL = {"f32": "", "f16": " f16", "x3": " x3", "x3b": ""}
_SCOPE = threading.local()


class precision:

    def __init__(self, p):
        if p not in PRECISIONS:
            raise ValueError("precision must be one of %s" % (PRECISIONS,))
        self.p = p

    def __enter__(self):
        stack = _SCOPE.__dict__.setdefault("stack", [])
        stack.append(self.p)
        return self

    def __exit__(self, *exc):
        _SCOPE.stack.pop()
        return False


def current_precision():
    stack = getattr(_SCOPE, "stack", None)
    return stack[-1] if stack else "f32"


def backward_precision(p):
    return "x3" if p == "x3b" else p


def _fn(lib, name, prec):
    return getattr(lib, name + _SUFFIX[prec])


def _env_on(name, default="1"):
    return os.environ.get(name, default) != "0"


def gemm_fwd(a, W, bias, want_stats=False, centers=None, Wc=None, prec=None):
    lib = _lib.load_library()
    M, K = a.shape
    N = W.shape[0]
    y = _lib.empty((M, N), dtype=torch.float32, device=a.device)
    sums = _lib.empty((N, 2), dtype=torch.float64, device=a.device) if want_stats else None
    ws = _Workspace.get(a.device)
    prec = current_precision() if prec is None else prec
    with _lib.timed("facl_gemm_fwd %dx%dx%d%s" % (M, K, N, _LABEL[prec])):
        _lib.check(_fn(lib, "facl_gemm_fwd", prec)(_lib.ptr(a), M, K, _lib.ptr(W), W.stride(0), N, _lib.ptr(bias), None, None,
                                     _lib.ptr(centers), _lib.ptr(Wc), 3 if Wc is not None else 0, _lib.ptr(y),
                                     _lib.ptr(sums), _lib.ptr(ws), _lib.stream()), "facl_gemm_fwd")
    return y, sums


def gemm_dgrad(dy, W, prec=None):
    lib = _lib.load_library()
    M, N = dy.shape
    K = W.shape[1]
    da = _lib.empty((M, K), dtype=torch.float32, device=dy.device)
    prec = current_precision() if prec is None else prec
    with _lib.timed("facl_gemm_dgrad %dx%dx%d%s" % (M, N, K, _LABEL[prec])):
        _lib.check(_fn(lib, "facl_gemm_dgrad", prec)(_lib.ptr(dy), M, N, W.data_ptr(), W.stride(0), K, _lib.ptr(da), _lib.stream()),
                   "facl_gemm_dgrad")
    return da


def _wgrad_slices(M, N, K):
    tiles = ((N + 127) // 128) * ((K + 127) // 128)
    return max(1, min((M + 255) // 256, 512 // tiles))


def _wgrad_h3(dy, a, bnc, amax, amax_b, dW, slices, nz):
    lib = _lib.load_library()
    M, N = dy.shape
    K = a.shape[1]
    ps, pt = (bnc[2], bnc[3]) if bnc is not None else (None, None)
    with _lib.timed("facl_gemm_wgrad %dx%dx%d h3" % (M, N, K)):
        rc = lib.facl_gemm_wgrad_h3(_lib.ptr(dy), _lib.ptr(a), M, N, K, a.stride(0), _lib.ptr(ps), _lib.ptr(pt), _lib.ptr(amax),
                                    _lib.ptr(amax_b), _lib.ptr(dW), _lib.ptr(slices), nz, _lib.stream())
    if rc == -4:
        return False
    _lib.check(rc, "facl_gemm_wgrad_h3")
    return True


def gemm_wgrad(dy, a, prec=None, amax=None, amax_b=None):
    lib = _lib.load_library()
    M, N = dy.shape
    K = a.shape[1]
    nz = _wgrad_slices(M, N, K)
    dW = _lib.empty((N, K), dtype=torch.float32, device=dy.device)
    slices = _lib.empty(nz * N * K, dtype=torch.float32, device=dy.device)
    prec = current_precision() if prec is None else prec
    if amax is not None and amax_b is not None and prec == "f32" and _wgrad_h3(dy, a, None, amax, amax_b, dW, slices, nz):
        return dW
    with _lib.timed("facl_gemm_wgrad %dx%dx%d%s" % (M, N, K, _LABEL[prec])):
        _lib.check(_fn(lib, "facl_gemm_wgrad", prec)(_lib.ptr(dy), _lib.ptr(a), M, N, K, a.stride(0), _lib.ptr(dW), _lib.ptr(slices), nz,
                                       _lib.stream()), "facl_gemm_wgrad")
    return dW


def _stats(y, ws):
    lib = _lib.load_library()
    R, C = y.shape
    sums = _lib.empty((C, 2), dtype=torch.float64, device=y.device)
    _lib.check(lib.facl_rows_stats(_lib.ptr(y), R, C, _lib.ptr(sums), _lib.ptr(ws), _lib.stream()), "facl_rows_stats")
    return sums


def _bn_bwd_consts(sums, C, count, reduce_fn):
    lib = _lib.load_library()
    f32 = dict(dtype=torch.float32, device=sums.device)
    dbeta, dgamma, kk = _lib.empty(C, **f32), _lib.empty(C, **f32), _lib.empty((2, C), **f32)
    sums_g = reduce_fn(sums.clone()) if reduce_fn is not None else sums
    _lib.check(lib.facl_bn_bwd_consts(_lib.ptr(sums), _lib.ptr(sums_g), C, float(count), _lib.ptr(dbeta), _lib.ptr(dgamma),
                                      _lib.ptr(kk), _lib.stream()), "facl_bn_bwd_consts")
    return dbeta, dgamma, kk


def _bn_relu_backward(da, y, bnc, count, reduce_fn, ws, sums=None, amax=None):
    lib = _lib.load_library()
    R, C = y.shape
    if sums is None:
        sums = _lib.empty((C, 2), dtype=torch.float64, device=y.device)
        _lib.check(lib.facl_rows_bwd_stats(_lib.ptr(da), _lib.ptr(y), R, C, _lib.ptr(bnc), _lib.ptr(sums), _lib.ptr(ws),
                                           _lib.stream()), "facl_rows_bwd_stats")
    dbeta, dgamma, kk = _bn_bwd_consts(sums, C, count, reduce_fn)
    dy = _lib.empty_like(y)
    _lib.check(lib.facl_rows_bwd_apply_amax(_lib.ptr(da), _lib.ptr(y), R, C, _lib.ptr(bnc), _lib.ptr(kk), _lib.ptr(dy),
                                            _lib.ptr(amax), _lib.stream()), "facl_rows_bwd_apply_amax")
    return dy, dgamma, dbeta


def _first_layer_wgrad(dy, h, centers, ws, prec, amax=None, amax_b=None):
    lib = _lib.load_library()
    R, C = dy.shape
    dWh = gemm_wgrad(dy, h, prec=prec, amax=amax, amax_b=amax_b)
    dWc = _lib.empty((C, 3), dtype=torch.float64, device=dy.device)
    _lib.check(lib.facl_rows_center_wgrad(_lib.ptr(dy), _lib.ptr(centers), R, C, _lib.ptr(dWc), _lib.ptr(ws), _lib.stream()),
               "facl_rows_center_wgrad")
    return torch.cat((dWc.float(), dWh), dim=1)


def _forward_bn_consts(y, bn, training, reduce_fn, ws, sums=None, aamax=None):
    R, C = y.shape
    if not training:
        bnc = _bn_eval(C, bn.weight.detach(), bn.bias.detach(), bn.running_mean, bn.running_var)
# ... 109 lines not shown
        sums = _lib.empty((C, 2), dtype=torch.float64, device=y.device)
        _lib.check(lib.facl_segmax_bwd_stats(_lib.ptr(dxpre), _lib.ptr(xpre), _lib.ptr(y), _lib.ptr(arg), M, S, C,
                                             _lib.ptr(bnc), _lib.ptr(sums), _lib.ptr(ws), _lib.stream()),
                   "facl_segmax_bwd_stats")
        dbeta, dgamma, kk = _bn_bwd_consts(sums, C, ctx.count, ctx.reduce_fn)
        dy = _lib.empty_like(y)
        _lib.check(lib.facl_segmax_bwd_apply(_lib.ptr(dxpre), _lib.ptr(xpre), _lib.ptr(y), _lib.ptr(arg), M, S, C,
                                             _lib.ptr(bnc), _lib.ptr(kk), _lib.ptr(dy), _lib.stream()),
                   "facl_segmax_bwd_apply")
        dW = gemm_wgrad(dy, h, prec=bp)
        dh = gemm_dgrad(dy, W, prec=bp)
        return dh, dW, None, dgamma, dbeta, None, None, None, None


def linear_bn_relu(h, affine, bn, training, reduce_fn=None, centers=None):
    W = affine.weight.view(affine.weight.shape[0], -1)
    return _LinearBNReLU.apply(h, W, affine.bias, bn.weight, bn.bias, bn, training, reduce_fn, centers)


class _Linear(torch.autograd.Function):

    @staticmethod
    def forward(ctx, h, W, b):
        ctx.prec = current_precision()
        h, W = h.contiguous(), W.contiguous()
        y, _ = gemm_fwd(h, W, b, prec=ctx.prec)
        ctx.save_for_backward(h, W)
        return y

    @staticmethod
    def backward(ctx, dy):
        bp = backward_precision(ctx.prec)
        h, W = ctx.saved_tensors
        dy = dy.contiguous()
        return gemm_dgrad(dy, W, prec=bp), gemm_wgrad(dy, h, prec=bp), dy.sum(0)


_FC_FUSED = _env_on("FACL_FC_FUSED")


class _FCHead(torch.autograd.Function):

    @staticmethod
    def forward(ctx, x_pre, G, W1, b1, gamma, beta, bn, W2, b2, training, reduce_fn):
        ctx.prec = current_precision()
        lib = _lib.load_library()
        _lib.require_cuda(x_pre)
        ws = _Workspace.get(x_pre.device)
        x_pre = x_pre.contiguous()
        M, Cin = x_pre.shape
        B = M // G
        h = _lib.empty((M + B, Cin), dtype=torch.float32, device=x_pre.device)
        arg = _lib.empty((B, Cin), dtype=torch.int32, device=x_pre.device)
        _lib.check(lib.facl_viewmax_stack(_lib.ptr(x_pre), G, B, Cin, _lib.ptr(h), _lib.ptr(arg), _lib.stream()), "facl_viewmax_stack")
        _lib.tap("view_arg", arg)
        W1, W2 = W1.contiguous(), W2.contiguous()
        R, C = M + B, W1.shape[0]
        segs = ((0, M), (M, R))
        fused = _FC_FUSED and training and M % 32 == 0 and C % 4 == 0
        ctx.fused = fused
        if fused:
            f32 = dict(dtype=torch.float32, device=x_pre.device)
            world = 1 if reduce_fn is None else reduce_fn.world_size
            counts = [float(M) * world, float(B) * world]
            sums2 = part = None
            na = nb = 0
            y = gemm_fwd(h, W1, b1, prec=ctx.prec)[0]
            if reduce_fn is not None:
                sums2 = _lib.empty((2, C, 2), dtype=torch.float64, device=y.device)
            _lib.check(lib.facl_fc_bn_stats(_lib.ptr(y), M, R, C, _lib.ptr(sums2), _lib.ptr(ws), _lib.stream()), "facl_fc_bn_stats")
            if reduce_fn is not None:
                reduce_fn(sums2)
            else:
                part, na, nb = ws, M // 32, (B + 31) // 32
            a = _lib.empty_like(y)
            bnc2 = _lib.empty((2, 5, C), **f32)
            _lib.check(lib.facl_fc_bn_apply(_lib.ptr(y), M, R, C, _lib.ptr(sums2), _lib.ptr(part), na, nb, counts[0], counts[1],
                                            _lib.ptr(gamma.detach()), _lib.ptr(beta.detach()), BN_EPS, BN_MOMENTUM,
                                            _lib.ptr(bn.running_mean), _lib.ptr(bn.running_var), _lib.ptr(bnc2), _lib.ptr(a),
                                            _lib.stream()), "facl_fc_bn_apply")
            bn.count_batch()
            bn.count_batch()
            bncs = [bnc2]
        else:
            y, _ = gemm_fwd(h, W1, b1, prec=ctx.prec)
            a = _lib.empty_like(y)
            bncs, counts = [], []
            if training:
                sums2 = _lib.empty((2, C, 2), dtype=torch.float64, device=y.device)
                for i, (r0, r1) in enumerate(segs):
                    _lib.check(lib.facl_rows_stats(_lib.ptr(y[r0:r1]), r1 - r0, C, _lib.ptr(sums2[i]), _lib.ptr(ws), _lib.stream()),
                               "facl_rows_stats")
                world = 1
                if reduce_fn is not None:
                    reduce_fn(sums2)
                    world = reduce_fn.world_size
            for i, (r0, r1) in enumerate(segs):
                if training:
                    count = float(r1 - r0) * world
                    bnc = _bn_finalize(sums2[i], C, count, gamma.detach(), beta.detach(), bn.running_mean, bn.running_var)
                    bn.count_batch()
                else:
                    bnc, count = _forward_bn_consts(y[r0:r1], bn, False, None, ws)
                _lib.check(lib.facl_rows_bn_relu(_lib.ptr(y[r0:r1]), r1 - r0, C, _lib.ptr(bnc[2]), _lib.ptr(bnc[3]),
                                                 _lib.ptr(a[r0:r1]), _lib.stream()), "facl_rows_bn_relu")
                bncs.append(bnc)
                counts.append(count)
        _lib.tap_relu("relu_fc", a=a)
        out, _ = gemm_fwd(a, W2, b2, prec=ctx.prec)
        ctx.save_for_backward(h, W1, y, a, W2, arg, *bncs)
        ctx.segs, ctx.counts, ctx.reduce_fn, ctx.training, ctx.G = segs, counts, reduce_fn, training, G
        return out

    @staticmethod
    def backward(ctx, dout):
        bp = backward_precision(ctx.prec)
        if not ctx.training:
            raise RuntimeError("backward through the eval-mode (folded BN) encoder is not supported")
        lib = _lib.load_library()
        h, W1, y, a, W2, arg, *bncs = ctx.saved_tensors
        bnc2 = bncs[0] if ctx.fused else None
        bnc_a, bnc_b = (bnc2[0], bnc2[1]) if ctx.fused else bncs
        ws = _Workspace.get(y.device)
        R, C = y.shape
        M = ctx.segs[0][1]
        B = R - M
        dout = dout.contiguous()
        f32 = dict(dtype=torch.float32, device=y.device)
        side = ctx.reduce_fn is None
        with _lib.fork(enabled=side) as f2:
            dW2 = gemm_wgrad(dout, a, prec=bp)
            if dout.shape[1] % 4 == 0:
                db2 = _lib.empty(dout.shape[1], **f32)
                _lib.check(lib.facl_col_sums(_lib.ptr(dout), R, dout.shape[1], _lib.ptr(db2), _lib.stream()), "facl_col_sums")
            else:
                db2 = dout.sum(0)
        dact = gemm_dgrad(dout, W2, prec=bp)
        dy = _lib.empty_like(y)
        if ctx.fused:
            sums2 = sums2_g = None
            if ctx.reduce_fn is not None:
                sums2 = _lib.empty((2, C, 2), dtype=torch.float64, device=y.device)
            _lib.check(lib.facl_fc_bn_bwd_stats(_lib.ptr(dact), _lib.ptr(y), M, R, C, _lib.ptr(bnc2), _lib.ptr(sums2), _lib.ptr(ws),
                                                _lib.stream()), "facl_fc_bn_bwd_stats")
            if ctx.reduce_fn is not None:
                sums2_g = ctx.reduce_fn(sums2)
            dgamma, dbeta, kk2 = _lib.empty(C, **f32), _lib.empty(C, **f32), _lib.empty((2, 2, C), **f32)
            _lib.check(lib.facl_fc_bn_bwd_apply(_lib.ptr(dact), _lib.ptr(y), M, R, C, _lib.ptr(bnc2), _lib.ptr(sums2_g), _lib.ptr(ws),
                                                ctx.counts[0], ctx.counts[1], _lib.ptr(dgamma), _lib.ptr(dbeta), _lib.ptr(kk2),
                                                _lib.ptr(dy), _lib.stream()), "facl_fc_bn_bwd_apply")
        else:
            sums2 = _lib.empty((2, C, 2), dtype=torch.float64, device=y.device)
            for i, ((r0, r1), bnc) in enumerate(zip(ctx.segs, (bnc_a, bnc_b))):
                _lib.check(lib.facl_rows_bwd_stats(_lib.ptr(dact[r0:r1]), _lib.ptr(y[r0:r1]), r1 - r0, C, _lib.ptr(bnc),
                                                   _lib.ptr(sums2[i]), _lib.ptr(ws), _lib.stream()), "facl_rows_bwd_stats")
            sums2_g = ctx.reduce_fn(sums2.clone()) if ctx.reduce_fn is not None else sums2
            dbe, dga, kk = _lib.empty((2, C), **f32), _lib.empty((2, C), **f32), _lib.empty((2, 2, C), **f32)
            for i, ((r0, r1), bnc, count) in enumerate(zip(ctx.segs, (bnc_a, bnc_b), ctx.counts)):
                _lib.check(lib.facl_bn_bwd_consts(_lib.ptr(sums2[i]), _lib.ptr(sums2_g[i]), C, float(count), _lib.ptr(dbe[i]),
                                                  _lib.ptr(dga[i]), _lib.ptr(kk[i]), _lib.stream()), "facl_bn_bwd_consts")
                _lib.check(lib.facl_rows_bwd_apply(_lib.ptr(dact[r0:r1]), _lib.ptr(y[r0:r1]), r1 - r0, C, _lib.ptr(bnc),
                                                   _lib.ptr(kk[i]), _lib.ptr(dy[r0:r1]), _lib.stream()), "facl_rows_bwd_apply")
            dgamma, dbeta = dga[0] + dga[1], dbe[0] + dbe[1]
        with _lib.fork(enabled=side) as f1:
            dW1 = gemm_wgrad(dy, h, prec=bp)
        dh = gemm_dgrad(dy, W1, prec=bp)
        _lib.check(lib.facl_viewmax_bwd_add(dh[M:].data_ptr(), _lib.ptr(arg), ctx.G, B, dh.shape[1], _lib.ptr(dh), _lib.stream()),
                   "facl_viewmax_bwd_add")
        f2.join(dW2, db2)
        f1.join(dW1)
        return dh[:M], None, dW1, None, dgamma, dbeta, None, dW2, db2, None, None


def fc_head(x_pre, G, affine1, bn, affine2, training, reduce_fn=None):
    return _FCHead.apply(x_pre, G, affine1.weight, affine1.bias, bn.weight, bn.bias, bn, affine2.weight, affine2.bias,
                         training, reduce_fn)


class _NormalizeMap(torch.autograd.Function):

    @staticmethod
    def forward(ctx, x, Wm, lazy=False):
        lib = _lib.load_library()
        _lib.require_cuda(x)
        x, Wm = x.contiguous(), Wm.contiguous()
        M, C = x.shape
        K = Wm.shape[0]
        xn = _lib.empty_like(x)
        code = _lib.empty((M, K), dtype=torch.float32, device=x.device)
        with _lib.fork(enabled=lazy) as f:
            _lib.check(lib.facl_normalize_map(_lib.ptr(x), M, C, _lib.ptr(Wm), K, _lib.ptr(xn), _lib.ptr(code), _lib.stream()),
                       "facl_normalize_map")
        if f.on:
            _lib._PENDING.append((f, (xn, code)))
        ctx.save_for_backward(x, xn, Wm)
        return xn, code

    @staticmethod
    def backward(ctx, dxn, dcode):
        x, xn, Wm = ctx.saved_tensors
        dxn_t = dcode @ Wm if dxn is None else dxn + dcode @ Wm
        dWm = dcode.t() @ xn
        nrm = x.norm(dim=1, keepdim=True).clamp_min(1e-12)
        dx = (dxn_t - xn * (dxn_t * xn).sum(1, keepdim=True)) / nrm
        return dx, dWm, None


def normalize_map(x, mapping_weight, lazy=False):
    return _NormalizeMap.apply(x, mapping_weight, lazy)


class _ViewMax(torch.autograd.Function):

    @staticmethod
    def forward(ctx, x_pre, G):
        lib = _lib.load_library()
        _lib.require_cuda(x_pre)
        x_pre = x_pre.contiguous()
        B, C = x_pre.shape[0] // G, x_pre.shape[1]
        out = _lib.empty((B, C), dtype=torch.float32, device=x_pre.device)
        arg = _lib.empty((B, C), dtype=torch.int32, device=x_pre.device)
        _lib.check(lib.facl_viewmax_fwd(_lib.ptr(x_pre), G, B, C, _lib.ptr(out), _lib.ptr(arg), _lib.stream()), "facl_viewmax_fwd")
        ctx.save_for_backward(arg)
        ctx.G = G
        return out

    @staticmethod
    def backward(ctx, dout):
        lib = _lib.load_library()
        arg, = ctx.saved_tensors
        B, C = arg.shape
        dout = dout.contiguous()
        dx = _lib.empty((ctx.G * B, C), dtype=torch.float32, device=dout.device)
        _lib.check(lib.facl_viewmax_bwd(_lib.ptr(dout), _lib.ptr(arg), ctx.G, B, C, _lib.ptr(dx), _lib.stream()), "facl_viewmax_bwd")
        return dx, None


def view_max(x_pre, G):
    return _ViewMax.apply(x_pre, G)


def linear(h, affine):
    return _Linear.apply(h, affine.weight, affine.bias)


def linear_bn_relu_segmax(h, affine, bn, training, S, reduce_fn=None):
    W = affine.weight.view(affine.weight.shape[0], -1)
    xpre, _ = _LinearBNSegmax.apply(h, W, affine.bias, bn.weight, bn.bias, bn, training, reduce_fn, S)
    return xpre


def rs_planes(W, transposed, centers_cols=None, half=False):
    lib = _lib.load_library()
    N, K = W.shape
    nb = lib.facl_gemm_rs_planes_bytes(K if transposed else N, N if transposed else K, 0 if centers_cols is None else 1)
    planes = _lib.empty(nb, dtype=torch.uint8, device=W.device)
    _lib.check(lib.facl_gemm_rs_planes(W.data_ptr(), W.stride(0), N, K, 1 if transposed else 0,
                                       None if centers_cols is None else centers_cols.data_ptr(),
                                       0 if centers_cols is None else centers_cols.stride(0), 1 if half else 0,
                                       _lib.ptr(planes), _lib.stream()), "facl_gemm_rs_planes")
    return planes


def rs_planes_multi(jobs, absmax=None):
    jobs = [(j + (False,))[:4] for j in jobs]
    import ctypes
    lib = _lib.load_library()
    n = len(jobs)
    outs = []
    for W, tr, xc, _h in jobs:
        N, K = W.shape
        nb = lib.facl_gemm_rs_planes_bytes(K if tr else N, N if tr else K, 0 if xc is None else 1)
        outs.append(_lib.empty(nb, dtype=torch.uint8, device=W.device))
    vp, ip = ctypes.c_void_p * n, ctypes.c_int * n
    _lib.check(lib.facl_gemm_rs_planes_multi(
        n, vp(*[j[0].data_ptr() for j in jobs]), ip(*[j[0].stride(0) for j in jobs]), ip(*[j[0].shape[0] for j in jobs]),
        ip(*[j[0].shape[1] for j in jobs]), ip(*[1 if j[1] else 0 for j in jobs]),
        vp(*[None if j[2] is None else j[2].data_ptr() for j in jobs]),
        ip(*[0 if j[2] is None else j[2].stride(0) for j in jobs]), ip(*[1 if j[3] else 0 for j in jobs]),
        vp(*[o.data_ptr() for o in outs]), None if absmax is None else _lib.ptr(absmax[0]),
        0 if absmax is None else absmax[0].numel(), None if absmax is None else _lib.ptr(absmax[1]), _lib.stream()),
        "facl_gemm_rs_planes_multi")
    return outs


FWD_H3 = _env_on("FACL_FWD_H3")
BWD_H3 = _env_on("FACL_BWD_H3")


def _rs_fwd(a, planes, N, bias, pro, centers, want_stats, seg_sgn, ws, half=False, amax_a=None):
    lib = _lib.load_library()
    M, K = a.shape
    y = _lib.empty((M, N), dtype=torch.float32, device=a.device)
    sums = _lib.empty((N, 2), dtype=torch.float64, device=a.device) if want_stats else None
    ymax = arg = None
    if seg_sgn is not None:
        ymax = _lib.empty((M // 64, N), dtype=torch.float32, device=a.device)
        arg = _lib.empty((M // 64, N), dtype=torch.int32, device=a.device)
    ps, pt = (pro[2], pro[3]) if pro is not None else (None, None)
    with _lib.timed("facl_gemm_rs_fwd %dx%dx%d%s" % (M, K, N, " h3" if half else "")):
        _lib.check(lib.facl_gemm_rs_fwd(_lib.ptr(a), M, K, _lib.ptr(planes), 1 if half else 0, _lib.ptr(amax_a), N, _lib.ptr(bias), _lib.ptr(ps), _lib.ptr(pt),
                                        _lib.ptr(centers), _lib.ptr(y), _lib.ptr(sums), _lib.ptr(seg_sgn), _lib.ptr(ymax),
                                        _lib.ptr(arg), _lib.ptr(ws), _lib.stream()), "facl_gemm_rs_fwd")
    return y, sums, ymax, arg


_FUSE_BNSTATS = _env_on("FACL_RS_BNSTATS")


def _rs_dgrad(dy, W, prec, planes=None, bn_y=None, bn_c=None, ws=None, amax=None):
    if prec != "f32":
        return gemm_dgrad(dy, W, prec=prec), None
    lib = _lib.load_library()
    M, N = dy.shape
    K = W.shape[1]
    half = 0 if amax is None else 1
    if planes is None:
        planes = rs_planes(W, True, half=bool(half))
    da = _lib.empty((M, K), dtype=torch.float32, device=dy.device)
    sums = None
    with _lib.timed("facl_gemm_rs_dgrad %dx%dx%d%s" % (M, N, K, " h3" if half else "")):
# ... 148 lines not shown
```

### include/facl_hip.h

```cpp
#ifndef FACL_HIP_H
#define FACL_HIP_H

#include <stdint.h>

#ifdef __cplusplus
extern "C" {
#endif

#define FACL_E_SHAPE  (-1)
#define FACL_E_NULL   (-2)
#define FACL_E_ALIGN  (-3)
#define FACL_E_CONFIG (-4)

int facl_version(void);

int facl_fps_f32(const float* xyz, int M, int N, int ld, int m, const int32_t* start,
                 int32_t* out_idx, void* stream);
int facl_fps_f64(const double* xyz, int M, int N, int ld, int m, const int32_t* start,
                 int32_t* out_idx, void* stream);

int facl_fps_reorder(const float* points, int M, int N, int D, const int32_t* picks, int m,
                     float* out, void* stream);

int facl_group(const float* points, int M, int N, int D, int S, int K, float r2,
// ... 59 lines not shown
                      const double* R1_g, const double* mom_l, const float* bnc1, const float* W1,
                      const float* b1, int D, double P, float* dW3, float* dg3, float* dbe3, float* dW2,
                      float* dg2, float* dbe2, float* dW1, float* dg1, float* dbe1, void* stream);

int facl_rows_stats(const float* y, int64_t R, int C, double* sums, void* ws, void* stream);
int facl_rows_bn_relu(const float* y, int64_t R, int C, const float* scale, const float* shift, float* out,
                      void* stream);
int facl_rows_segmax(const float* y, int64_t M, int S, int C, const float* bnc, float* out, int32_t* arg,
                     void* stream);
int facl_rows_bwd_stats(const float* dout, const float* y, int64_t R, int C, const float* bnc, double* sums,
                        void* ws, void* stream);
int facl_viewmax_fwd(const float* x, int G, int B, int C, float* out, int32_t* arg, void* stream);
int facl_viewmax_bwd(const float* dout, const int32_t* arg, int G, int B, int C, float* dx, void* stream);
int facl_viewmax_bwd_add(const float* dout, const int32_t* arg, int G, int B, int C, float* dx, void* stream);
int facl_viewmax_stack(const float* x, int G, int B, int C, float* h, int32_t* arg, void* stream);

int facl_fc_bn_stats(const float* y, int64_t M, int64_t R, int C, double* sums2, void* ws, void* stream);
int facl_fc_bn_apply(const float* y, int64_t M, int64_t R, int C, const double* sums2, const double* part, int nslices_a,
                     int nslices_b, double count_a, double count_b, const float* gamma, const float* beta, float eps,
                     float momentum, float* running_mean, float* running_var, float* bnc2, float* a_out, void* stream);
int facl_fc_bn_bwd_stats(const float* dact, const float* y, int64_t M, int64_t R, int C, const float* bnc2, double* sums2,
                         void* ws, void* stream);
int facl_fc_bn_bwd_apply(const float* dact, const float* y, int64_t M, int64_t R, int C, const float* bnc2,
                         const double* sums2_g, const void* ws, double count_a, double count_b, float* dgamma, float* dbeta,
                         float* kk2, float* dy, void* stream);
int facl_col_sums(const float* x, int64_t R, int C, float* out, void* stream);
int facl_rows_center_wgrad(const float* dy, const float* centers, int64_t R, int C, double* dWc, void* ws,
                           void* stream);
int facl_rows_bwd_apply(const float* dout, const float* y, int64_t R, int C, const float* bnc,
                        const float* kk, float* dy, void* stream);
int facl_segmax_bwd_stats(const float* dxpre, const float* xpre, const float* y, const int32_t* arg,
                          int64_t M, int S, int C, const float* bnc, double* sums, void* ws, void* stream);
int facl_segmax_bwd_stats_ymax(const float* dxpre, const float* xpre, const float* ymax, int64_t M, int C,
                               const float* bnc, double* sums, void* ws, uint32_t* zamax, int zwords, void* stream);
int facl_segmax_bwd_apply(const float* dxpre, const float* xpre, const float* y, const int32_t* arg,
                          int64_t M, int S, int C, const float* bnc, const float* kk, float* dy, void* stream);
#define FACL_AMAX_WORDS 2048
int facl_rows_bwd_apply_amax(const float* dout, const float* y, int64_t R, int C, const float* bnc, const float* kk,
                             float* dy, uint32_t* amax, void* stream);
int facl_segmax_bwd_apply_amax(const float* dxpre, const float* xpre, const float* y, const int32_t* arg, int64_t M, int S,
                               int C, const float* bnc, const float* kk, float* dy, uint32_t* amax, void* stream);

int facl_gemm_fwd(const float* a, int64_t M, int K, const float* W, int ldw, int N, const float* bias,
                  const float* pscale, const float* pshift, const float* centers, const float* Wc,
                  int ldwc, float* y, double* sums, void* ws, void* stream);
int facl_gemm_fwd_segmax(const float* a, int64_t M, int K, const float* W, int ldw, int N, const float* bias,
                         const float* sgn, float* y, double* sums, float* ymax, int32_t* arg, void* ws,
                         void* stream);
int facl_gemm_dgrad(const float* dy, int64_t M, int N, const float* W, int ldw, int K, float* da,
                    void* stream);
int facl_gemm_wgrad(const float* dy, const float* a, int64_t M, int N, int K, int lda, float* dW,
                    float* slices, int nz, void* stream);
int facl_gemm_wgrad_acc(const float* dy, const float* a, int64_t M, int N, int K, int lda, float* dW, int prec, void* stream);
int facl_gemm_fwd_f16(const float* a, int64_t M, int K, const float* W, int ldw, int N, const float* bias,
                      const float* pscale, const float* pshift, const float* centers, const float* Wc, int ldwc,
                      float* y, double* sums, void* ws, void* stream);
int facl_gemm_fwd_segmax_f16(const float* a, int64_t M, int K, const float* W, int ldw, int N, const float* bias,
                             const float* sgn, float* y, double* sums, float* ymax, int32_t* arg, void* ws,
                             void* stream);
int facl_gemm_dgrad_f16(const float* dy, int64_t M, int N, const float* W, int ldw, int K, float* da,
                        void* stream);
int facl_gemm_wgrad_f16(const float* dy, const float* a, int64_t M, int N, int K, int lda, float* dW,
                        float* slices, int nz, void* stream);
int facl_gemm_wgrad_pro(const float* dy, const float* y, int64_t M, int N, int K, int ldy, const float* pscale,
                        const float* pshift, float* dW, float* slices, int nz, void* stream);
int facl_gemm_wgrad_pro_x3(const float* dy, const float* y, int64_t M, int N, int K, int ldy, const float* pscale,
                           const float* pshift, float* dW, float* slices, int nz, void* stream);
int facl_gemm_wgrad_h3(const float* dy, const float* y, int64_t M, int N, int K, int ldy, const float* pscale,
                       const float* pshift, const uint32_t* amax, const uint32_t* amax_b, float* dW, float* slices, int nz,
                       void* stream);
int facl_gemm_rs_wgrad_slices(int64_t M, int N, int K);
int facl_gemm_rs_wgrad(const float* dy, const float* y, int64_t M, int N, int K, const float* pscale, const float* pshift,
                       const uint32_t* amax, const uint32_t* amax_b, float* dW, float* slices, void* stream);
int64_t facl_gemm_rs_planes_bytes(int N, int K, int with_centers);
int facl_gemm_rs_planes(const float* W, int ldw, int N, int K, int transposed, const float* Wc, int ldwc, int half,
                        void* planes, void* stream);
int facl_gemm_rs_planes_multi(int n, const float* const* W, const int* ldw, const int* N, const int* K,
                              const int* transposed, const float* const* Wc, const int* ldwc, const int* half,
                              void* const* planes, const float* absmax_x, int64_t absmax_n, uint32_t* absmax_amax,
                              void* stream);
int facl_gemm_rs_supported(int64_t M, int K, int N);
int facl_gemm_rs_fwd(const float* a, int64_t M, int K, const void* planes, int half, const uint32_t* amax_a, int N,
                     const float* bias, const float* pscale, const float* pshift, const float* centers, float* y, double* sums,
                     const float* sgn, float* ymax, int32_t* arg, void* ws, void* stream);
int facl_gemm_rs_dgrad(const float* dy, int64_t M, int N, const void* planes, int half, const uint32_t* amax, int K,
                       float* da, void* stream);
int facl_gemm_rs_dgrad_bnstats(const float* dy, int64_t M, int N, const void* planes, int half, const uint32_t* amax, int K,
                               float* da, const float* y, const float* bnc, double* sums, void* ws, void* stream);
int facl_gemm_fwd_x3(const float* a, int64_t M, int K, const float* W, int ldw, int N, const float* bias,
                     const float* pscale, const float* pshift, const float* centers, const float* Wc, int ldwc,
                     float* y, double* sums, void* ws, void* stream);
int facl_gemm_fwd_segmax_x3(const float* a, int64_t M, int K, const float* W, int ldw, int N, const float* bias,
                            const float* sgn, float* y, double* sums, float* ymax, int32_t* arg, void* ws,
                            void* stream);
int facl_gemm_dgrad_x3(const float* dy, int64_t M, int N, const float* W, int ldw, int K, float* da,
                       void* stream);
int facl_gemm_wgrad_x3(const float* dy, const float* a, int64_t M, int N, int K, int lda, float* dW,
                       float* slices, int nz, void* stream);
int facl_sa_fwd3_x3(const float* y2f, int64_t nunits, const float* scale2, const float* shift2, const float* W3,
                    const float* b3, const float* sgn3, float* ymax, uint8_t* arg, double* sums3, void* ws,
                    void* stream);

int facl_gather_rows(const float* feat, int ldf, int M, int S1, int C, const int32_t* idx, int rows_per_cloud,
                     const float* xyz, float* out, int ldo, int col_off, void* stream);
int facl_scatter_rows(const float* drows, int ldd, int col_off, int M, int S1, int C, const int32_t* idx,
                      int rows_per_cloud, float* dfeat, void* stream);

int facl_contrast(const float* sim, int R, int J, int B, int Bk, int nA, int nS, int slot_rows,
                  const int32_t* poscol, int clip_offset, float* dsim, double* loss, void* ws, void* stream);
int facl_contrast_pair(const float* sim, int G, int B, int Bk, int J, const int64_t* order, int clip_offset,
                       float* dsim, double* losses, void* ws, void* stream);
int facl_contrast_pair_sum(const float* sim, int G, int B, int Bk, int J, const int64_t* order, int clip_offset,
                           float* dsim, double* losses, float* losses32, void* ws, void* stream);
int facl_contrast_pair_sum_mask(const float* sim, int G, int B, int Bk, int J, const int64_t* order, int clip_offset,
                                int mask_mode, float* dsim, double* losses, float* losses32, void* ws, void* stream);
int facl_loss_rows_fwd(const float* x, int64_t R, int C, int normalize, float s, float* n, float* inv_norm, void* stream);
int facl_loss_rows_bwd(const float* dn, const float* n, const float* inv_norm, int64_t R, int C, int normalize, float s,
                       float* dx, void* stream);
int facl_contrast_pair_queue(const float* sim, const float* sim_q, int G, int B, int Bk, int J, int L, const int64_t* order,
                             int clip_offset, int mask_mode, const int32_t* qstate, float* dsim, float* dsim_q, double* losses,
                             float* losses32, void* ws, void* stream);
int facl_queue_push(const float* rows, int P, int C, float* queue, int L, int32_t* qstate, void* stream);
int facl_scale_rows2(const float* src, float* dst, int64_t R1, int64_t R, int J, const float* g1, const float* g2,
                     void* stream);

int facl_normalize_map(const float* x, int64_t M, int C, const float* Wm, int K, float* x_nor, float* code,
                       void* stream);

int64_t facl_mailbox_bytes(int R, int n_max);
int facl_mailbox_alloc(int64_t bytes, void** ptr, void* handle64);
int facl_mailbox_open(const void* handle64, void** ptr);
int facl_mailbox_close(void* ptr);
int facl_mailbox_free(void* ptr);
// ... 111 lines not shown
```

Before: 10780.

## Precompute bf16 split planes for FC head operands in producer kernels

```diff
diff --git a/facl_amd/_lib.py b/facl_amd/_lib.py
--- a/facl_amd/_lib.py
+++ b/facl_amd/_lib.py
@@ -144,8 +144,18 @@
     "facl_softmax_ce": [c_p, c_i, c_p, c_i, c_i, c_p, c_p, c_p, c_p, c_p],
     "facl_cls_probs_acc": [c_p, c_i, c_i, c_i, c_p, c_i, c_p],
     "facl_cls_topk": [c_p, c_i, c_i, c_i, c_i, c_p, c_p, c_p, c_p, c_p],
+    "facl_gemm_planes_bytes": [c_l, c_l],
+    "facl_gemm_fwd_pl": [c_p, c_l, c_i, c_p, c_i, c_i, c_p, c_p, c_p, c_p, c_p, c_i, c_p, c_p, c_p, c_p, c_p, c_p],
+    "facl_gemm_dgrad_pl": [c_p, c_l, c_i, c_p, c_i, c_i, c_p, c_p, c_p, c_p],
+    "facl_gemm_wgrad_pl": [c_p, c_p, c_l, c_i, c_i, c_i, c_p, c_p, c_i, c_p, c_p, c_p],
+    "facl_gemm_wgrad_acc_pl": [c_p, c_p, c_l, c_i, c_i, c_i, c_p, c_i, c_p, c_p, c_p],
+    "facl_viewmax_stack_pl": [c_p, c_i, c_i, c_i, c_p, c_p, c_p, c_p],
+    "facl_fc_bn_apply_pl": [c_p, c_l, c_l, c_i, c_p, c_p, c_i, c_i, c_d, c_d, c_p, c_p, c_f, c_f, c_p, c_p, c_p, c_p, c_p, c_p],
+    "facl_fc_bn_bwd_apply_pl": [c_p, c_p, c_l, c_l, c_i, c_p, c_p, c_p, c_d, c_d, c_p, c_p, c_p, c_p, c_p, c_p],
+    "facl_gemm_rs_planes_multi_ew": [c_i, c_p, c_p, c_p, c_p, c_p, c_p, c_p, c_p, c_p, c_p, c_l, c_p,
+                                     c_i, c_p, c_p, c_p, c_p, c_p, c_p],
 }
-RESTYPE_I64 = {"facl_ws_bytes", "facl_gemm_rs_planes_bytes", "facl_mailbox_bytes", "facl_knn_ws_bytes"}
+RESTYPE_I64 = {"facl_ws_bytes", "facl_gemm_rs_planes_bytes", "facl_mailbox_bytes", "facl_knn_ws_bytes", "facl_gemm_planes_bytes"}
 
 
 def lib_path():
diff --git a/facl_amd/cn3d_model_conbag.py b/facl_amd/cn3d_model_conbag.py
--- a/facl_amd/cn3d_model_conbag.py
+++ b/facl_amd/cn3d_model_conbag.py
@@ -141,6 +141,9 @@
         n3 = self.net3DV_3
         widths = (n3[0].weight.shape[1] - 3, n3[0].weight.shape[0], n3[3].weight.shape[0], n3[6].weight.shape[0])
         if _tail.net3dv3_supported(pooled.shape[0], widths, S, _tail.current_precision()):
+            fcw = self.netR_FC
+            if training and fcw[0].weight.dim() == 2 and fcw[3].weight.dim() == 2:
+                _tail.request_weight_planes(fcw[0].weight, fcw[3].weight)
             x_pre = _tail.net3dv3(pooled, centers, n3, training, S, self.bn_reduce_fn, pooled_amax)
         else:
             h = _tail.linear_bn_relu(pooled, n3[0], n3[1], training, self.bn_reduce_fn, centers=centers)
@@ -148,6 +151,7 @@
             x_pre = _tail.linear_bn_relu_segmax(h, n3[6], n3[7], training, S, self.bn_reduce_fn)
         fc = self.netR_FC
         stacked = _tail.fc_head(x_pre, self.gost, fc[0], fc[1], fc[3], training, self.bn_reduce_fn)
+        _tail.request_weight_planes()
         self._stacked = stacked
         x, x_global = stacked[:M], stacked[M:]
         x_nor, code = _tail.normalize_map(x, self.mapping.weight, lazy=bool(getattr(self, "lazy_code", False)))
diff --git a/facl_amd/csrc/common.h b/facl_amd/csrc/common.h
--- a/facl_amd/csrc/common.h
+++ b/facl_amd/csrc/common.h
@@ -126,6 +126,16 @@
     const float s0 = sub_f32(r0, __builtin_bit_cast(float, mi << 16)), s1 = sub_f32(r1, __builtin_bit_cast(float, mi & 0xffff0000u));
     lo = pk_bf16(s0, s1);
 }
+__host__ __device__ inline long long facl_planes_ld(long long C) { return (C + 1) & ~1LL; }
+__host__ __device__ inline long long facl_planes_stride(long long R, long long C) { return (R * facl_planes_ld(C) + 7) & ~7LL; }
+__device__ __forceinline__ void facl_planes_store4(unsigned short* __restrict__ pl, long long ps, size_t off, float4 v) {
+    unsigned h0, m0, l0, h1, m1, l1;
+    split_pair(v.x, v.y, h0, m0, l0);
+    split_pair(v.z, v.w, h1, m1, l1);
+    *reinterpret_cast<uint2*>(pl + off) = make_uint2(h0, h1);
+    *reinterpret_cast<uint2*>(pl + ps + off) = make_uint2(m0, m1);
+    *reinterpret_cast<uint2*>(pl + 2 * ps + off) = make_uint2(l0, l1);
+}
 __device__ __forceinline__ bf16x8 as_bf16x8(unsigned a, unsigned b, unsigned c, unsigned d) {
     const uint4 u = make_uint4(a, b, c, d);
     return __builtin_bit_cast(bf16x8, u);
diff --git a/facl_amd/csrc/fchead.hip b/facl_amd/csrc/fchead.hip
--- a/facl_amd/csrc/fchead.hip
+++ b/facl_amd/csrc/fchead.hip
@@ -80,7 +80,8 @@
 }
 
 __global__ __launch_bounds__(256) void k_fc_apply(const float* __restrict__ y, int M, int R, int C4,
-                                                  const float* __restrict__ bnc2, float* __restrict__ out) {
+                                                  const float* __restrict__ bnc2, float* __restrict__ out,
+                                                  unsigned short* __restrict__ pl, long long ps) {
     const int c4 = blockIdx.x * 256 + threadIdx.x;
     if (c4 >= C4) return;
     const int C = 4 * C4;
@@ -88,7 +89,9 @@
     const float4 sb = reinterpret_cast<const float4*>(bnc2 + 7 * C)[c4], tb = reinterpret_cast<const float4*>(bnc2 + 8 * C)[c4];
     for (int r = blockIdx.y; r < R; r += gridDim.y) {
         const float4 sc = r < M ? sa : sb, sh = r < M ? ta : tb;
-        reinterpret_cast<float4*>(out)[(size_t)r * C4 + c4] = lane_map<4>(bn_relu, sc, reinterpret_cast<const float4*>(y)[(size_t)r * C4 + c4], sh);
+        const float4 v = lane_map<4>(bn_relu, sc, reinterpret_cast<const float4*>(y)[(size_t)r * C4 + c4], sh);
+        reinterpret_cast<float4*>(out)[(size_t)r * C4 + c4] = v;
+        if (pl) facl_planes_store4(pl, ps, ((size_t)r * C4 + c4) * 4, v);
     }
 }
 
@@ -133,7 +136,7 @@
 
 __global__ __launch_bounds__(256) void k_fc_bwd_apply(const float* __restrict__ dout, const float* __restrict__ y, int M, int R,
                                                       int C4, const float* __restrict__ bnc2, const float* __restrict__ kk2,
-                                                      float* __restrict__ dy) {
+                                                      float* __restrict__ dy, unsigned short* __restrict__ pl, long long ps) {
     const int c4 = blockIdx.x * 256 + threadIdx.x;
     if (c4 >= C4) return;
     const int C = 4 * C4;
@@ -142,8 +145,10 @@
     for (int r = blockIdx.y; r < R; r += gridDim.y) {
         const int s = r < M ? 0 : 1;
         const size_t o = (size_t)r * C4 + c4;
-        reinterpret_cast<float4*>(dy)[o] = lane_map<4>(bn_relu_bwd, reinterpret_cast<const float4*>(dout)[o], reinterpret_cast<const float4*>(y)[o],
-                                                       q[s].mean, q[s].inv, q[s].scale, q[s].shift, k[s].k1, k[s].k2);
+        const float4 v = lane_map<4>(bn_relu_bwd, reinterpret_cast<const float4*>(dout)[o], reinterpret_cast<const float4*>(y)[o],
+                                     q[s].mean, q[s].inv, q[s].scale, q[s].shift, k[s].k1, k[s].k2);
+        reinterpret_cast<float4*>(dy)[o] = v;
+        if (pl) facl_planes_store4(pl, ps, o * 4, v);
     }
 }
 
@@ -183,7 +188,7 @@
 }
 
 __global__ __launch_bounds__(256) void k_viewmax_stack(const float* __restrict__ x, int G, int B, int C4, float* __restrict__ h,
-                                                       int* __restrict__ arg) {
+                                                       int* __restrict__ arg, unsigned short* __restrict__ pl, long long ps) {
     __shared__ float4 sb[3][64];
     __shared__ int4 si[3][64];
     const int it = threadIdx.x & 63, ph = threadIdx.x >> 6;
@@ -198,11 +203,13 @@
         const size_t o0 = ((size_t)g0 * B + b) * C4 + c4;
         best = reinterpret_cast<const float4*>(x)[o0];
         reinterpret_cast<float4*>(h)[o0] = best;
+        if (pl) facl_planes_store4(pl, ps, o0 * 4, best);
         bi = make_int4(g0, g0, g0, g0);
         for (int g = g0 + 1; g < g1; ++g) {
             const size_t o = ((size_t)g * B + b) * C4 + c4;
             const float4 v = reinterpret_cast<const float4*>(x)[o];
             reinterpret_cast<float4*>(h)[o] = v;
+            if (pl) facl_planes_store4(pl, ps, o * 4, v);
             first_max_wins(best, bi, v, g);
         }
     }
@@ -217,6 +224,7 @@
             first_max_wins(best, bi, v, vi);
         }
         reinterpret_cast<float4*>(h)[((size_t)G * B + b) * C4 + c4] = best;
+        if (pl) facl_planes_store4(pl, ps, (((size_t)G * B + b) * C4 + c4) * 4, best);
         reinterpret_cast<int4*>(arg)[i] = bi;
     }
 }
@@ -243,22 +251,37 @@
     return facl_launch_status();
 }
 
-extern "C" int facl_fc_bn_apply(const float* y, int64_t M, int64_t R, int C, const double* sums2, const double* part,
-                                int nslices_a, int nslices_b, double count_a, double count_b, const float* gamma,
-                                const float* beta, float eps, float momentum, float* running_mean, float* running_var,
-                                float* bnc2, float* a, void* stream) {
+static int fc_bn_apply(const float* y, int64_t M, int64_t R, int C, const double* sums2, const double* part,
+                       int nslices_a, int nslices_b, double count_a, double count_b, const float* gamma,
+                       const float* beta, float eps, float momentum, float* running_mean, float* running_var,
+                       float* bnc2, float* a, void* a_planes, void* stream) {
     if (!y || !gamma || !beta || !bnc2 || !a || (!sums2 && !part)) return FACL_E_NULL;
     if (M < 1 || R <= M || R > 0x7fffffff || C < 4 || (C & 3) || count_a < 1 || count_b < 1) return FACL_E_SHAPE;
     if (!sums2 && (nslices_a < 1 || nslices_b < 1)) return FACL_E_SHAPE;
-    if (!aligned16(y, a, bnc2)) return FACL_E_ALIGN;
+    if (!aligned16(y, a, bnc2) || ((uintptr_t)a_planes & 15)) return FACL_E_ALIGN;
     hipStream_t st = (hipStream_t)stream;
     hipLaunchKernelGGL(k_fc_finalize, dim3((C + 63) / 64), dim3(256), 0, st, sums2 ? sums2 : part, sums2 ? 1 : nslices_a,
                        sums2 ? 1 : nslices_b, C, count_a, count_b, gamma, beta, eps, momentum, running_mean, running_var, bnc2);
     const int gx = (C / 4 + 255) / 256;
     int gy = 1024 / gx;
     if (gy > R) gy = (int)R;
-    hipLaunchKernelGGL(k_fc_apply, dim3(gx, gy), dim3(256), 0, st, y, (int)M, (int)R, C / 4, bnc2, a);
-    return facl_launch_status();
+    hipLaunchKernelGGL(k_fc_apply, dim3(gx, gy), dim3(256), 0, st, y, (int)M, (int)R, C / 4, bnc2, a, (unsigned short*)a_planes,
+                       facl_planes_stride(R, C));
+    return facl_launch_status();
+}
+extern "C" int facl_fc_bn_apply(const float* y, int64_t M, int64_t R, int C, const double* sums2, const double* part,
+                                int nslices_a, int nslices_b, double count_a, double count_b, const float* gamma,
+                                const float* beta, float eps, float momentum, float* running_mean, float* running_var,
+                                float* bnc2, float* a, void* stream) {
+    return fc_bn_apply(y, M, R, C, sums2, part, nslices_a, nslices_b, count_a, count_b, gamma, beta, eps, momentum, running_mean,
+                       running_var, bnc2, a, nullptr, stream);
+}
+extern "C" int facl_fc_bn_apply_pl(const float* y, int64_t M, int64_t R, int C, const double* sums2, const double* part,
+                                   int nslices_a, int nslices_b, double count_a, double count_b, const float* gamma,
+                                   const float* beta, float eps, float momentum, float* running_mean, float* running_var,
+                                   float* bnc2, float* a, void* stream, void* a_planes) {
+    return fc_bn_apply(y, M, R, C, sums2, part, nslices_a, nslices_b, count_a, count_b, gamma, beta, eps, momentum, running_mean,
+                       running_var, bnc2, a, a_planes, stream);
 }
 
 extern "C" int facl_fc_bn_bwd_stats(const float* dact, const float* y, int64_t M, int64_t R, int C, const float* bnc2,
@@ -275,13 +298,13 @@
     return facl_launch_status();
 }
 
-extern "C" int facl_fc_bn_bwd_apply(const float* dact, const float* y, int64_t M, int64_t R, int C, const float* bnc2,
-                                    const double* sums2_g, const void* ws, double count_a, double count_b, float* dgamma,
-                                    float* dbeta, float* kk2, float* dy, void* stream) {
+static int fc_bn_bwd_apply(const float* dact, const float* y, int64_t M, int64_t R, int C, const float* bnc2,
+                           const double* sums2_g, const void* ws, double count_a, double count_b, float* dgamma,
+                           float* dbeta, float* kk2, float* dy, void* dy_planes, void* stream) {
     if (!dact || !y || !bnc2 || !ws || !dgamma || !dbeta || !kk2 || !dy) return FACL_E_NULL;
     if (!fc_shape_ok(M, R, C)) return FACL_E_CONFIG;
     if (count_a < 1 || count_b < 1) return FACL_E_SHAPE;
-    if (!aligned16(y, dact, bnc2, kk2, dy)) return FACL_E_ALIGN;
+    if (!aligned16(y, dact, bnc2, kk2, dy) || ((uintptr_t)dy_planes & 15)) return FACL_E_ALIGN;
     const int na = fc_na(M), nb = fc_nb(M, R);
     hipStream_t st = (hipStream_t)stream;
     hipLaunchKernelGGL(k_fc_bwd_consts, dim3((C + 63) / 64), dim3(256), 0, st, (const double*)ws, na, nb, sums2_g, C, count_a,
@@ -289,8 +312,19 @@
     const int gx = (C / 4 + 255) / 256;
     int gy = 1024 / gx;
     if (gy > R) gy = (int)R;
-    hipLaunchKernelGGL(k_fc_bwd_apply, dim3(gx, gy), dim3(256), 0, st, dact, y, (int)M, (int)R, C / 4, bnc2, kk2, dy);
-    return facl_launch_status();
+    hipLaunchKernelGGL(k_fc_bwd_apply, dim3(gx, gy), dim3(256), 0, st, dact, y, (int)M, (int)R, C / 4, bnc2, kk2, dy,
+                       (unsigned short*)dy_planes, facl_planes_stride(R, C));
+    return facl_launch_status();
+}
+extern "C" int facl_fc_bn_bwd_apply(const float* dact, const float* y, int64_t M, int64_t R, int C, const float* bnc2,
+                                    const double* sums2_g, const void* ws, double count_a, double count_b, float* dgamma,
+                                    float* dbeta, float* kk2, float* dy, void* stream) {
+    return fc_bn_bwd_apply(dact, y, M, R, C, bnc2, sums2_g, ws, count_a, count_b, dgamma, dbeta, kk2, dy, nullptr, stream);
+}
+extern "C" int facl_fc_bn_bwd_apply_pl(const float* dact, const float* y, int64_t M, int64_t R, int C, const float* bnc2,
+                                       const double* sums2_g, const void* ws, double count_a, double count_b, float* dgamma,
+                                       float* dbeta, float* kk2, float* dy, void* stream, void* dy_planes) {
+    return fc_bn_bwd_apply(dact, y, M, R, C, bnc2, sums2_g, ws, count_a, count_b, dgamma, dbeta, kk2, dy, dy_planes, stream);
 }
 
 extern "C" int facl_col_sums(const float* x, int64_t R, int C, float* out, void* stream) {
@@ -301,11 +335,15 @@
     return facl_launch_status();
 }
 
-extern "C" int facl_viewmax_stack(const float* x, int G, int B, int C, float* h, int32_t* arg, void* stream) {
+extern "C" int facl_viewmax_stack_pl(const float* x, int G, int B, int C, float* h, int32_t* arg, void* stream, void* h_planes) {
     if (!x || !h || !arg) return FACL_E_NULL;
     if (G < 1 || B < 1 || C < 4 || (C & 3)) return FACL_E_SHAPE;
-    if (!aligned16(x, h, arg)) return FACL_E_ALIGN;
+    if (!aligned16(x, h, arg) || ((uintptr_t)h_planes & 15)) return FACL_E_ALIGN;
     const int n = B * (C / 4);
-    hipLaunchKernelGGL(k_viewmax_stack, dim3((n + 63) / 64), dim3(256), 0, (hipStream_t)stream, x, G, B, C / 4, h, arg);
-    return facl_launch_status();
-}
+    hipLaunchKernelGGL(k_viewmax_stack, dim3((n + 63) / 64), dim3(256), 0, (hipStream_t)stream, x, G, B, C / 4, h, arg,
+                       (unsigned short*)h_planes, facl_planes_stride((long long)G * B + B, C));
+    return facl_launch_status();
+}
+extern "C" int facl_viewmax_stack(const float* x, int G, int B, int C, float* h, int32_t* arg, void* stream) {
+    return facl_viewmax_stack_pl(x, G, B, C, h, arg, stream, nullptr);
+}
diff --git a/facl_amd/csrc/gemm.hip b/facl_amd/csrc/gemm.hip
--- a/facl_amd/csrc/gemm.hip
+++ b/facl_amd/csrc/gemm.hip
@@ -23,6 +23,9 @@
     const unsigned* amax = nullptr;
     const unsigned* amax_b = nullptr;
     int accum = 0;
+    const unsigned short* Apl = nullptr; const unsigned short* Bpl = nullptr;
+    int ldap = 0, ldbp = 0;
+    long long psa = 0, psb = 0;
 };
 
 template <int LAY, int T>
@@ -546,18 +549,96 @@
 }
 
 
-template <int LAY, int T, int NP, bool PRO>
+template <int T, bool FULL>
+__device__ __forceinline__ void load_planes_kc4(const unsigned short* __restrict__ Q, int ld, long long ps, int idx0, int nidx,
+                                                int k0, int kend, unsigned (&pk)[12 * T], int tid) {
+    const int k = k0 + 4 * (tid & 7);
+    const int kc = FULL ? k : (k + 3 < kend ? k : kend - 4);
+#pragma unroll
+    for (int i = 0; i < 2 * T; ++i) {
+        int idx = idx0 + (tid >> 3) + 32 * i;
+        idx = idx < nidx ? idx : nidx - 1;
+        const unsigned short* s = Q + (size_t)idx * ld + kc;
+#pragma unroll
+        for (int p = 0; p < 3; ++p) {
+            uint2 v = *reinterpret_cast<const uint2*>(s + (size_t)p * ps);
+            if (!FULL && k >= kend) v = make_uint2(0u, 0u);
+            pk[6 * i + 2 * p] = v.x; pk[6 * i + 2 * p + 1] = v.y;
+        }
+    }
+}
+template <int T>
+__device__ __forceinline__ void ic_item(int e, int& pr, int& ch) {
+    pr = (e & 15) + 16 * ((e >> 6) % (2 * T));
+    ch = ((e >> 4) & 3) + 4 * (e / (128 * T));
+}
+template <int T, bool FULL>
+__device__ __forceinline__ void load_planes_ic(const unsigned short* __restrict__ Q, int ld, long long ps, int idx0, int nidx,
+                                               int k0, int kend, unsigned (&rp)[12 * T], int tid) {
+    const int last = (nidx - 1) & ~1;
+#pragma unroll
+    for (int i = 0; i < T; ++i) {
+        int pr, ch;
+        ic_item<T>(tid + 256 * i, pr, ch);
+        int idx = idx0 + 2 * pr;
+        idx = idx < last ? idx : last;
+#pragma unroll
+        for (int j = 0; j < 4; ++j) {
+            const int k = k0 + 4 * ch + j;
+            const int kk = FULL ? k : (k < kend ? k : kend - 1);
+            const unsigned short* s = Q + (size_t)kk * ld + idx;
+#pragma unroll
+            for (int p = 0; p < 3; ++p) {
+                unsigned v = *reinterpret_cast<const unsigned*>(s + (size_t)p * ps);
+                if (!FULL && k >= kend) v = 0u;
+                rp[12 * i + 4 * p + j] = v;
+            }
+        }
+    }
+}
+template <int T>
+__device__ __forceinline__ void exchange_planes_ic(const unsigned (&rp)[12 * T], unsigned (&pk)[12 * T]) {
+#pragma unroll
+    for (int i = 0; i < 3 * T; ++i) {
+        const unsigned d0 = rp[4 * i], d1 = rp[4 * i + 1], d2 = rp[4 * i + 2], d3 = rp[4 * i + 3];
+        pk[4 * i] = __builtin_amdgcn_perm(d1, d0, 0x05040100u);
+        pk[4 * i + 1] = __builtin_amdgcn_perm(d3, d2, 0x05040100u);
+        pk[4 * i + 2] = __builtin_amdgcn_perm(d1, d0, 0x07060302u);
+        pk[4 * i + 3] = __builtin_amdgcn_perm(d3, d2, 0x07060302u);
+    }
+}
+template <int T>
+__device__ __forceinline__ void write_planes_ic(unsigned short* __restrict__ S, const unsigned (&pk)[12 * T], int tid) {
+    constexpr int PLANE = 64 * T * SBROW;
+#pragma unroll
+    for (int i = 0; i < T; ++i) {
+        int pr, ch;
+        ic_item<T>(tid + 256 * i, pr, ch);
+        unsigned short* d = S + 2 * pr * SBROW + 4 * ch;
+#pragma unroll
+        for (int p = 0; p < 3; ++p) {
+            *reinterpret_cast<uint2*>(d + p * PLANE) = make_uint2(pk[12 * i + 4 * p], pk[12 * i + 4 * p + 1]);
+            *reinterpret_cast<uint2*>(d + p * PLANE + SBROW) = make_uint2(pk[12 * i + 4 * p + 2], pk[12 * i + 4 * p + 3]);
+        }
+    }
+}
+
+template <int LAY, int T, int NP, bool PRO, bool PL = false>
 struct SplitOperand {
+    static_assert(!PL || (NP == 3 && !PRO), "planes hold the three pieces of the raw tensor: bf16x6 without prologue");
     static constexpr int NPL = NP == 4 ? 2 : NP;
     static constexpr int PLANE = 64 * T * SBROW;
     const float* P; int ld, idx0, nidx;
     const float* ps; const float* pt;
     float psi = 1.f, pti = 0.f;
+    const unsigned short* Q; int ldq; long long qs;
     float4 r4[2 * T];
     float r8[8 * T];
+    unsigned rp[12 * T];
     unsigned pk[12 * T];
-    __device__ __forceinline__ SplitOperand(const float* P_, int ld_, int idx0_, int nidx_, const float* ps_, const float* pt_, int tid)
-        : P(P_), ld(ld_), idx0(idx0_), nidx(nidx_), ps(ps_), pt(pt_) {
+    __device__ __forceinline__ SplitOperand(const float* P_, int ld_, int idx0_, int nidx_, const float* ps_, const float* pt_, int tid,
+                                            const unsigned short* Q_ = nullptr, int ldq_ = 0, long long qs_ = 0)
+        : P(P_), ld(ld_), idx0(idx0_), nidx(nidx_), ps(ps_), pt(pt_), Q(Q_), ldq(ldq_), qs(qs_) {
         if (PRO && LAY == IC) {
             int j = idx0 + tid % (64 * T);
             j = j < nidx ? j : nidx - 1;
@@ -566,7 +647,10 @@
     }
     template <bool FULL>
     __device__ __forceinline__ void fetch(int k0, int kend, int tid) {
-        if (LAY == KC) load_tile_kc4<T, FULL>(P, ld, idx0, nidx, k0, kend, r4, tid);
+        if constexpr (PL) {
+            if (LAY == KC) load_planes_kc4<T, FULL>(Q, ldq, qs, idx0, nidx, k0, kend, pk, tid);
+            else load_planes_ic<T, FULL>(Q, ldq, qs, idx0, nidx, k0, kend, rp, tid);
+        } else if (LAY == KC) load_tile_kc4<T, FULL>(P, ld, idx0, nidx, k0, kend, r4, tid);
         else load_tile_ic8<T, FULL>(P, ld, idx0, nidx, k0, kend, r8, tid);
     }
     __device__ __forceinline__ float absmax() const {
@@ -581,11 +665,14 @@
         return m;
     }
     __device__ __forceinline__ void split(int k0, float sc, int tid) {
-        if (LAY == KC) split_tile_kc4<PRO, T, NP>(r4, pk, tid, k0, ps, pt, sc);
+        if constexpr (PL) {
+            if (LAY == IC) exchange_planes_ic<T>(rp, pk);
+        } else if (LAY == KC) split_tile_kc4<PRO, T, NP>(r4, pk, tid, k0, ps, pt, sc);
         else split_tile_ic8<T, NP, PRO>(r8, pk, psi, pti, sc);
     }
     __device__ __forceinline__ void write(unsigned short* S, int tid) const {
-        if (LAY == KC) write_tile_kc4<T, NP>(S, pk, tid);
+        if (PL && LAY == IC) write_planes_ic<T>(S, pk, tid);
+        else if (LAY == KC) write_tile_kc4<T, NP>(S, pk, tid);
         else write_tile_ic8<T, NP>(S, pk, tid);
     }
     static __device__ __forceinline__ bf16x8 frag(const unsigned short* S, int p, int row, int kk, int h) {
@@ -625,7 +712,7 @@
             }
 }
 
-template <int LA, int LB, bool PRO, int TM, int TN, int NP = 3>
+template <int LA, int LB, bool PRO, int TM, int TN, int NP = 3, bool PLA = false, bool PLB = false>
 __global__ __launch_bounds__(256, NP == 1 ? 3 : 2) void k_gemm_sb(GemmArgs g) {
     constexpr int BM = 64 * TM, BN = 64 * TN;
     constexpr int APL = BM * SBROW, BPL = BN * SBROW;
@@ -656,10 +743,10 @@
 #pragma unroll
             for (int r = 0; r < 16; ++r) acc[a][b][r] = 0.f;
 
-    using OpA = SplitOperand<LA, TM, NP, PRO && LA == KC>;
-    using OpB = SplitOperand<LB, TN, NP, PRO && LA == IC && LB == IC>;
-    OpA opa(g.A, g.lda, i0, g.MI, g.pscale, g.pshift, tid);
-    OpB opb(g.B, g.ldb, j0, g.NJ, g.pscale, g.pshift, tid);
+    using OpA = SplitOperand<LA, TM, NP, PRO && LA == KC, PLA>;
+    using OpB = SplitOperand<LB, TN, NP, PRO && LA == IC && LB == IC, PLB>;
+    OpA opa(g.A, g.lda, i0, g.MI, g.pscale, g.pshift, tid, g.Apl, g.ldap, g.psa);
+    OpB opb(g.B, g.ldb, j0, g.NJ, g.pscale, g.pshift, tid, g.Bpl, g.ldbp, g.psb);
     auto fetch = [&](int k0) { fetch_stage(opa, opb, k0, kend, tid); };
     auto split = [&](int k0) { opa.split(k0, sca, tid); opb.split(k0, scb, tid); };
     auto write = [&]() { opa.write(sA, tid); opb.write(sB, tid); };
@@ -692,7 +779,7 @@
     else gemm_epilogue<TM, TN>(g, acc, smem, i0, j0, wave, lane, tile.y, tile.z);
 }
 
-template <int LA, int LB, bool PRO, int NP, int KG>
+template <int LA, int LB, bool PRO, int NP, int KG, bool PLA = false, bool PLB = false>
 __global__ __launch_bounds__(256 * KG, 1) void k_gemm_sbk(GemmArgs g) {
     constexpr int NPL = NP == 4 ? 2 : NP;
     constexpr int PL = 64 * SBROW;
@@ -716,10 +803,10 @@
 #pragma unroll
     for (int r = 0; r < 16; ++r) acc[0][0][r] = 0.f;
 
-    using OpA = SplitOperand<LA, 1, NP, PRO && LA == KC>;
-    using OpB = SplitOperand<LB, 1, NP, PRO && LA == IC && LB == IC>;
-    OpA opa(g.A, g.lda, i0, g.MI, g.pscale, g.pshift, tid);
-    OpB opb(g.B, g.ldb, j0, g.NJ, g.pscale, g.pshift, tid);
+    using OpA = SplitOperand<LA, 1, NP, PRO && LA == KC, PLA>;
+    using OpB = SplitOperand<LB, 1, NP, PRO && LA == IC && LB == IC, PLB>;
+    OpA opa(g.A, g.lda, i0, g.MI, g.pscale, g.pshift, tid, g.Apl, g.ldap, g.psa);
+    OpB opb(g.B, g.ldb, j0, g.NJ, g.pscale, g.pshift, tid, g.Bpl, g.ldbp, g.psb);
     auto fetch = [&](int k0) { fetch_stage(opa, opb, k0, kend, tid); };
     float* const mxs = smem + MXOFF;
     float uns_nxt = 1.f;
@@ -785,13 +872,13 @@
 }
 
 constexpr int SBK_KG = 4;
-template <int LA, int LB, bool PRO, int NP>
+template <int LA, int LB, bool PRO, int NP, bool PLA = false, bool PLB = false>
 int launch_sbk(const GemmArgs& g, int nz, hipStream_t st) {
     constexpr int TILE_F = (NP == 4 ? 2 : NP) * 2 * 64 * SBROW * 2 / 4, STG = 4 * 32 * 36;
     constexpr int F = SBK_KG * TILE_F > STG + (SBK_KG - 1) * 4096 ? SBK_KG * TILE_F : STG + (SBK_KG - 1) * 4096;
     constexpr int lds = (F + SBK_KG * 8) * 4;
     const dim3 grid((g.NJ + 63) / 64, (g.MI + 63) / 64, nz);
-    return facl_launch_dynamic_lds<k_gemm_sbk<LA, LB, PRO, NP, SBK_KG>>(grid, dim3(256 * SBK_KG), lds, st, g);
+    return facl_launch_dynamic_lds<k_gemm_sbk<LA, LB, PRO, NP, SBK_KG, PLA, PLB>>(grid, dim3(256 * SBK_KG), lds, st, g);
 }
 
 bool use_f32_mfma() {
@@ -809,12 +896,12 @@
     return fills128 ? TileChoice{T128, 64, true} : TileChoice{T64, 32, false};
 }
 
-template <int LA, int LB, bool PRO, int NP>
+template <int LA, int LB, bool PRO, int NP, bool PLA = false, bool PLB = false>
 int launch_split(const GemmArgs& g, int nz, const TileChoice& tc, hipStream_t st) {
-    if (tc.family == SBK) return launch_sbk<LA, LB, PRO, NP>(g, nz, st);
+    if (tc.family == SBK) return launch_sbk<LA, LB, PRO, NP, PLA, PLB>(g, nz, st);
     if (tc.family == T128)
-        hipLaunchKernelGGL((k_gemm_sb<LA, LB, PRO, 2, 2, NP>), dim3((g.NJ + 127) / 128, (g.MI + 127) / 128, nz), dim3(256), 0, st, g);
-    else hipLaunchKernelGGL((k_gemm_sb<LA, LB, PRO, 1, 1, NP>), dim3((g.NJ + 63) / 64, (g.MI + 63) / 64, nz), dim3(256), 0, st, g);
+        hipLaunchKernelGGL((k_gemm_sb<LA, LB, PRO, 2, 2, NP, PLA, PLB>), dim3((g.NJ + 127) / 128, (g.MI + 127) / 128, nz), dim3(256), 0, st, g);
+    else hipLaunchKernelGGL((k_gemm_sb<LA, LB, PRO, 1, 1, NP, PLA, PLB>), dim3((g.NJ + 63) / 64, (g.MI + 63) / 64, nz), dim3(256), 0, st, g);
     return facl_launch_status();
 }
 
@@ -828,6 +915,9 @@
         if constexpr (!PRO) {
             static const int sbk_h3 = facl_env_int("FACL_SBK_H3", 0);
             if (tc.family == SBK && sbk_h3) return launch_sbk<LA, LB, false, 4>(g, nz, st);
+            if (g.Apl && g.Bpl) return launch_split<LA, LB, false, 3, true, true>(g, nz, tc, st);
+            if (g.Apl) return launch_split<LA, LB, false, 3, true, false>(g, nz, tc, st);
+            if (g.Bpl) return launch_split<LA, LB, false, 3, false, true>(g, nz, tc, st);
         }
         return launch_split<LA, LB, PRO, 3>(g, nz, tc, st);
     }
@@ -929,14 +1019,30 @@
     return (size_t)*prow * N * 2 * sizeof(double) <= (size_t)facl_ws_bytes() - FACL_WS_TICKET_BYTES;
 }
 
+static bool planes_aligned(const void* p) { return !((uintptr_t)p & 15); }
+static void set_planes(GemmArgs& g, const void* Apl, long long Ar, long long Ac, const void* Bpl, long long Br, long long Bc) {
+    g.Apl = (const unsigned short*)Apl; g.ldap = (int)facl_planes_ld(Ac); g.psa = facl_planes_stride(Ar, Ac);
+    g.Bpl = (const unsigned short*)Bpl; g.ldbp = (int)facl_planes_ld(Bc); g.psb = facl_planes_stride(Br, Bc);
+    if (g.prec != 0 || g.pscale) g.Apl = g.Bpl = nullptr;
+}
+
+extern "C" int64_t facl_gemm_planes_bytes(int64_t R, int64_t C) {
+    if (R < 1 || C < 1) return 0;
+    return 3 * facl_planes_stride(R, C) * 2;
+}
+
 static int gemm_fwd_p(const float* a, int64_t M, int K, const float* W, int ldw, int N, const float* bias,
                       const float* pscale, const float* pshift, const float* centers, const float* Wc,
-                      int ldwc, float* y, double* sums, void* ws, void* stream, int prec) {
+                      int ldwc, float* y, double* sums, void* ws, void* stream, int prec, const void* apl = nullptr,
+                      const void* wpl = nullptr) {
     if (!a || !W || !y || (sums && !ws)) return FACL_E_NULL;
     if (M < 1 || M > 0x7fffffff || K < 4 || (K & 3) || N < 1 || (ldw & 3)) return FACL_E_SHAPE;
     if ((pscale == nullptr) != (pshift == nullptr) || (centers == nullptr) != (Wc == nullptr)) return FACL_E_NULL;
+    if (!planes_aligned(apl) || !planes_aligned(wpl)) return FACL_E_ALIGN;
     hipStream_t st = (hipStream_t)stream;
     GemmArgs g{a, K, W, ldw, y, N, (int)M, N, K};
+    g.prec = prec; g.pscale = pscale;
+    set_planes(g, apl, M, K, wpl, N, K);
     g.bias = bias; g.pscale = pscale; g.pshift = pshift;
     g.xa = centers; g.xb = Wc; g.ldxb = ldwc;
     g.part = sums ? (double*)ws : nullptr;
@@ -971,21 +1077,25 @@
 }
 
 static int gemm_dgrad_p(const float* dy, int64_t M, int N, const float* W, int ldw, int K, float* da,
-                        void* stream, int prec) {
+                        void* stream, int prec, const void* dypl = nullptr, const void* wpl = nullptr) {
     if (!dy || !W || !da) return FACL_E_NULL;
     if (M < 1 || M > 0x7fffffff || N < 4 || (N & 3) || K < 1) return FACL_E_SHAPE;
+    if (!planes_aligned(dypl) || !planes_aligned(wpl)) return FACL_E_ALIGN;
     GemmArgs g{dy, N, W, ldw, da, K, (int)M, K, N};
     g.kchunk = N; g.prec = prec;
+    set_planes(g, dypl, M, N, wpl, N, K);
     return launch<KC, IC, false>(g, 1, (hipStream_t)stream, nullptr);
 }
 
 static int gemm_wgrad_p(const float* dy, const float* a, int64_t M, int N, int K, int lda, float* dW,
-                        float* slices, int nz, void* stream, int prec) {
+                        float* slices, int nz, void* stream, int prec, const void* dypl = nullptr, const void* apl = nullptr) {
     if (!dy || !a || !dW || !slices) return FACL_E_NULL;
     if (M < 1 || M > 0x7fffffff || N < 4 || (N & 3) || K < 4 || (K & 3) || nz < 1 || nz > 1024) return FACL_E_SHAPE;
+    if (!planes_aligned(dypl) || !planes_aligned(apl)) return FACL_E_ALIGN;
     hipStream_t st = (hipStream_t)stream;
     GemmArgs g{dy, N, a, lda, dW, K, N, K, (int)M};
     g.kchunk = (int)M; g.prec = prec;
+    set_planes(g, dypl, M, N, apl, M, K);
     if (M <= 8192 && choose_tile(g, 1).family == SBK) return launch<IC, IC, false>(g, 1, st, nullptr);
     g.C = slices;
     return split_k(g, nz, dW, st, [&](const GemmArgs& gz, int z) { return launch<IC, IC, false>(gz, z, st, nullptr); });
@@ -1088,12 +1198,37 @@
     return gemm_wgrad_p(dy, a, M, N, K, lda, dW, slices, nz, stream, 2);
 }
 
+static int gemm_wgrad_acc_p(const float* dy, const float* a, int64_t M, int N, int K, int lda, float* dW, int prec,
+                            void* stream, const void* dypl, const void* apl) {
+    if (!dy || !a || !dW) return FACL_E_NULL;
+    if (M < 1 || M > 8192 || N < 4 || (N & 3) || K < 4 || (K & 3) || prec < 0 || prec > 2) return FACL_E_SHAPE;
+    if (!planes_aligned(dypl) || !planes_aligned(apl)) return FACL_E_ALIGN;
+    GemmArgs g{dy, N, a, lda, dW, K, N, K, (int)M};
+    g.kchunk = (int)M; g.prec = prec; g.accum = 1;
+    set_planes(g, dypl, M, N, apl, M, K);
+    if (choose_tile(g, 1).family != SBK) return FACL_E_CONFIG;
+    return launch<IC, IC, false>(g, 1, (hipStream_t)stream, nullptr);
+}
 extern "C" int facl_gemm_wgrad_acc(const float* dy, const float* a, int64_t M, int N, int K, int lda, float* dW, int prec,
                                    void* stream) {
-    if (!dy || !a || !dW) return FACL_E_NULL;
-    if (M < 1 || M > 8192 || N < 4 || (N & 3) || K < 4 || (K & 3) || prec < 0 || prec > 2) return FACL_E_SHAPE;
-    GemmArgs g{dy, N, a, lda, dW, K, N, K, (int)M};
-    g.kchunk = (int)M; g.prec = prec; g.accum = 1;
-    if (choose_tile(g, 1).family != SBK) return FACL_E_CONFIG;
-    return launch<IC, IC, false>(g, 1, (hipStream_t)stream, nullptr);
-}
+    return gemm_wgrad_acc_p(dy, a, M, N, K, lda, dW, prec, stream, nullptr, nullptr);
+}
+
+extern "C" int facl_gemm_fwd_pl(const float* a, int64_t M, int K, const float* W, int ldw, int N, const float* bias,
+                                const float* pscale, const float* pshift, const float* centers, const float* Wc,
+                                int ldwc, float* y, double* sums, void* ws, void* stream, const void* a_planes,
+                                const void* w_planes) {
+    return gemm_fwd_p(a, M, K, W, ldw, N, bias, pscale, pshift, centers, Wc, ldwc, y, sums, ws, stream, 0, a_planes, w_planes);
+}
+extern "C" int facl_gemm_dgrad_pl(const float* dy, int64_t M, int N, const float* W, int ldw, int K, float* da, void* stream,
+                                  const void* dy_planes, const void* w_planes) {
+    return gemm_dgrad_p(dy, M, N, W, ldw, K, da, stream, 0, dy_planes, w_planes);
+}
+extern "C" int facl_gemm_wgrad_pl(const float* dy, const float* a, int64_t M, int N, int K, int lda, float* dW,
+                                  float* slices, int nz, void* stream, const void* dy_planes, const void* a_planes) {
+    return gemm_wgrad_p(dy, a, M, N, K, lda, dW, slices, nz, stream, 0, dy_planes, a_planes);
+}
+extern "C" int facl_gemm_wgrad_acc_pl(const float* dy, const float* a, int64_t M, int N, int K, int lda, float* dW, int prec,
+                                      void* stream, const void* dy_planes, const void* a_planes) {
+    return gemm_wgrad_acc_p(dy, a, M, N, K, lda, dW, prec, stream, dy_planes, a_planes);
+}
diff --git a/facl_amd/csrc/gemm_rs.hip b/facl_amd/csrc/gemm_rs.hip
--- a/facl_amd/csrc/gemm_rs.hip
+++ b/facl_amd/csrc/gemm_rs.hip
@@ -123,14 +123,39 @@
 }
 
 constexpr int RS_MAXJOBS = 8;
+constexpr int RS_MAXEW = 4;
+constexpr int RS_EW_PER = 4;
 struct RsPlaneJobs {
     int n;
     const float* W[RS_MAXJOBS]; long long so[RS_MAXJOBS]; long long sc[RS_MAXJOBS]; int NO[RS_MAXJOBS]; int NC[RS_MAXJOBS];
     const float* xc[RS_MAXJOBS]; int ldxc[RS_MAXJOBS]; uint4* out[RS_MAXJOBS]; int* hdr[RS_MAXJOBS]; int first[RS_MAXJOBS + 1];
     int half[RS_MAXJOBS];
     const float* ax; long long an; unsigned* aamax; int anb;
+    int ne; const float* ew[RS_MAXEW]; int eld[RS_MAXEW]; int eC4[RS_MAXEW]; long long en4[RS_MAXEW]; unsigned short* eout[RS_MAXEW];
+    long long eps[RS_MAXEW]; int efirst[RS_MAXEW + 1];
 };
+__device__ __forceinline__ void rs_planes_ew_block(const float* __restrict__ W, int ld, int C4, long long n4,
+                                                   unsigned short* __restrict__ out, long long ps, int b) {
+    float4 v[RS_EW_PER];
+    long long q[RS_EW_PER];
+#pragma unroll
+    for (int t = 0; t < RS_EW_PER; ++t) {
+        q[t] = ((long long)b * RS_EW_PER + t) * 256 + threadIdx.x;
+        if (q[t] < n4) v[t] = *reinterpret_cast<const float4*>(W + (q[t] / C4) * ld + (q[t] % C4) * 4);
+    }
+#pragma unroll
+    for (int t = 0; t < RS_EW_PER; ++t)
+        if (q[t] < n4) facl_planes_store4(out, ps, (size_t)q[t] * 4, v[t]);
+}
 __global__ __launch_bounds__(256) void k_rs_planes_multi(RsPlaneJobs jb) {
+    if ((int)blockIdx.x >= jb.first[jb.n] + jb.anb) {
+        const int b = (int)blockIdx.x - jb.first[jb.n] - jb.anb;
+        int e = 0;
+#pragma unroll
+        for (int t = 1; t < RS_MAXEW; ++t) e += (t < jb.ne && b >= jb.efirst[t]) ? 1 : 0;
+        rs_planes_ew_block(jb.ew[e], jb.eld[e], jb.eC4[e], jb.en4[e], jb.eout[e], jb.eps[e], b - jb.efirst[e]);
+        return;
+    }
     if ((int)blockIdx.x >= jb.first[jb.n]) {
         rs_absmax_block(jb.ax, jb.an, jb.aamax, (int)blockIdx.x - jb.first[jb.n], jb.anb);
         return;
@@ -762,14 +787,29 @@
     return facl_launch_status();
 }
 
-extern "C" int facl_gemm_rs_planes_multi(int n, const float* const* W, const int* ldw, const int* N, const int* K,
-                                         const int* transposed, const float* const* Wc, const int* ldwc, const int* half,
-                                         void* const* planes, const float* absmax_x, int64_t absmax_n, uint32_t* absmax_amax,
-                                         void* stream) {
+static int rs_planes_multi(int n, const float* const* W, const int* ldw, const int* N, const int* K,
+                           const int* transposed, const float* const* Wc, const int* ldwc, const int* half,
+                           void* const* planes, const float* absmax_x, int64_t absmax_n, uint32_t* absmax_amax,
+                           int n_ew, const float* const* ew_W, const int* ew_ld, const int* ew_R, const int* ew_C,
+                           void* const* ew_planes, void* stream) {
     if (!W || !ldw || !N || !K || !transposed || !Wc || !ldwc || !half || !planes) return FACL_E_NULL;
     if ((absmax_x == nullptr) != (absmax_amax == nullptr)) return FACL_E_NULL;
-    if (n < 1 || n > RS_MAXJOBS || (absmax_x && absmax_n < 1)) return FACL_E_SHAPE;
+    if (n < 1 || n > RS_MAXJOBS || (absmax_x && absmax_n < 1) || n_ew < 0 || n_ew > RS_MAXEW) return FACL_E_SHAPE;
+    if (n_ew && (!ew_W || !ew_ld || !ew_R || !ew_C || !ew_planes)) return FACL_E_NULL;
     RsPlaneJobs jb;
+    jb.ne = n_ew;
+    jb.efirst[0] = 0;
+    for (int e = 0; e < RS_MAXEW; ++e) {
+        if (e >= n_ew) { jb.ew[e] = nullptr; jb.eout[e] = nullptr; jb.eld[e] = 0; jb.eC4[e] = 1; jb.en4[e] = 0; jb.eps[e] = 0; jb.efirst[e + 1] = jb.efirst[e]; continue; }
+        if (!ew_W[e] || !ew_planes[e]) return FACL_E_NULL;
+        if (ew_R[e] < 1 || ew_C[e] < 4 || (ew_C[e] & 3) || ew_ld[e] < ew_C[e] || (ew_ld[e] & 3)) return FACL_E_SHAPE;
+        if (((uintptr_t)ew_W[e] | (uintptr_t)ew_planes[e]) & 15) return FACL_E_ALIGN;
+        jb.ew[e] = ew_W[e]; jb.eld[e] = ew_ld[e]; jb.eC4[e] = ew_C[e] / 4; jb.en4[e] = (long long)ew_R[e] * (ew_C[e] / 4);
+        jb.eout[e] = (unsigned short*)ew_planes[e]; jb.eps[e] = facl_planes_stride(ew_R[e], ew_C[e]);
+        const long long nb = (jb.en4[e] + 256 * RS_EW_PER - 1) / (256 * RS_EW_PER);
+        if (nb > (1 << 20)) return FACL_E_SHAPE;
+        jb.efirst[e + 1] = jb.efirst[e] + (int)nb;
+    }
     jb.n = n;
     jb.first[0] = 0;
     for (int j = 0; j < RS_MAXJOBS; ++j) {
@@ -786,8 +826,23 @@
     }
     jb.ax = absmax_x; jb.an = absmax_n; jb.aamax = absmax_amax;
     jb.anb = absmax_x ? (int)((absmax_n + 4095) / 4096 < 16 ? (absmax_n + 4095) / 4096 : 16) : 0;
-    hipLaunchKernelGGL(k_rs_planes_multi, dim3(jb.first[n] + jb.anb), dim3(256), 0, (hipStream_t)stream, jb);
+    hipLaunchKernelGGL(k_rs_planes_multi, dim3(jb.first[n] + jb.anb + jb.efirst[n_ew]), dim3(256), 0, (hipStream_t)stream, jb);
     return facl_launch_status();
+}
+extern "C" int facl_gemm_rs_planes_multi(int n, const float* const* W, const int* ldw, const int* N, const int* K,
+                                         const int* transposed, const float* const* Wc, const int* ldwc, const int* half,
+                                         void* const* planes, const float* absmax_x, int64_t absmax_n, uint32_t* absmax_amax,
+                                         void* stream) {
+    return rs_planes_multi(n, W, ldw, N, K, transposed, Wc, ldwc, half, planes, absmax_x, absmax_n, absmax_amax, 0, nullptr, nullptr,
+                           nullptr, nullptr, nullptr, stream);
+}
+extern "C" int facl_gemm_rs_planes_multi_ew(int n, const float* const* W, const int* ldw, const int* N, const int* K,
+                                            const int* transposed, const float* const* Wc, const int* ldwc, const int* half,
+                                            void* const* planes, const float* absmax_x, int64_t absmax_n, uint32_t* absmax_amax,
+                                            int n_ew, const float* const* ew_W, const int* ew_ld, const int* ew_R, const int* ew_C,
+                                            void* const* ew_planes, void* stream) {
+    return rs_planes_multi(n, W, ldw, N, K, transposed, Wc, ldwc, half, planes, absmax_x, absmax_n, absmax_amax, n_ew, ew_W, ew_ld,
+                           ew_R, ew_C, ew_planes, stream);
 }
 
 extern "C" int facl_gemm_rs_supported(int64_t M, int K, int N) {
diff --git a/facl_amd/tail.py b/facl_amd/tail.py
--- a/facl_amd/tail.py
+++ b/facl_amd/tail.py
@@ -47,7 +47,30 @@
     return os.environ.get(name, default) != "0"
 
 
-def gemm_fwd(a, W, bias, want_stats=False, centers=None, Wc=None, prec=None):
+GEMM_PLANES = _env_on("FACL_GEMM_PLANES", "0")
+
+
+def planes_on(prec):
+    return GEMM_PLANES and prec in ("f32", "x3b")
+
+
+def planes_empty(R, C, device):
+    return _lib.empty(_lib.load_library().facl_gemm_planes_bytes(R, C), dtype=torch.uint8, device=device)
+
+
+_FC_PLANES = threading.local()
+
+
+def request_weight_planes(*weights):
+    _FC_PLANES.req = [w.detach() for w in weights]
+    _FC_PLANES.got = {}
+
+
+def take_weight_planes(W):
+    return getattr(_FC_PLANES, "got", {}).pop((W.data_ptr(), tuple(W.shape)), None)
+
+
+def gemm_fwd(a, W, bias, want_stats=False, centers=None, Wc=None, prec=None, a_pl=None, w_pl=None):
     lib = _lib.load_library()
     M, K = a.shape
     N = W.shape[0]
@@ -55,6 +78,13 @@
     sums = _lib.empty((N, 2), dtype=torch.float64, device=a.device) if want_stats else None
     ws = _Workspace.get(a.device)
     prec = current_precision() if prec is None else prec
+    if (a_pl is not None or w_pl is not None) and planes_on(prec):
+        with _lib.timed("facl_gemm_fwd %dx%dx%d%s" % (M, K, N, _LABEL[prec])):
+            _lib.check(lib.facl_gemm_fwd_pl(_lib.ptr(a), M, K, _lib.ptr(W), W.stride(0), N, _lib.ptr(bias), None, None,
+                                            _lib.ptr(centers), _lib.ptr(Wc), 3 if Wc is not None else 0, _lib.ptr(y),
+                                            _lib.ptr(sums), _lib.ptr(ws), _lib.stream(), _lib.ptr(a_pl), _lib.ptr(w_pl)),
+                       "facl_gemm_fwd_pl")
+        return y, sums
     with _lib.timed("facl_gemm_fwd %dx%dx%d%s" % (M, K, N, _LABEL[prec])):
         _lib.check(_fn(lib, "facl_gemm_fwd", prec)(_lib.ptr(a), M, K, _lib.ptr(W), W.stride(0), N, _lib.ptr(bias), None, None,
                                      _lib.ptr(centers), _lib.ptr(Wc), 3 if Wc is not None else 0, _lib.ptr(y),
@@ -62,12 +92,17 @@
     return y, sums
 
 
-def gemm_dgrad(dy, W, prec=None):
+def gemm_dgrad(dy, W, prec=None, dy_pl=None, w_pl=None):
     lib = _lib.load_library()
     M, N = dy.shape
     K = W.shape[1]
     da = _lib.empty((M, K), dtype=torch.float32, device=dy.device)
     prec = current_precision() if prec is None else prec
+    if (dy_pl is not None or w_pl is not None) and planes_on(prec) and prec == "f32":
+        with _lib.timed("facl_gemm_dgrad %dx%dx%d%s" % (M, N, K, _LABEL[prec])):
+            _lib.check(lib.facl_gemm_dgrad_pl(_lib.ptr(dy), M, N, W.data_ptr(), W.stride(0), K, _lib.ptr(da), _lib.stream(),
+                                              _lib.ptr(dy_pl), _lib.ptr(w_pl)), "facl_gemm_dgrad_pl")
+        return da
     with _lib.timed("facl_gemm_dgrad %dx%dx%d%s" % (M, N, K, _LABEL[prec])):
         _lib.check(_fn(lib, "facl_gemm_dgrad", prec)(_lib.ptr(dy), M, N, W.data_ptr(), W.stride(0), K, _lib.ptr(da), _lib.stream()),
                    "facl_gemm_dgrad")
@@ -93,7 +128,7 @@
     return True
 
 
-def gemm_wgrad(dy, a, prec=None, amax=None, amax_b=None):
+def gemm_wgrad(dy, a, prec=None, amax=None, amax_b=None, dy_pl=None, a_pl=None):
     lib = _lib.load_library()
     M, N = dy.shape
     K = a.shape[1]
@@ -102,6 +137,11 @@
     slices = _lib.empty(nz * N * K, dtype=torch.float32, device=dy.device)
     prec = current_precision() if prec is None else prec
     if amax is not None and amax_b is not None and prec == "f32" and _wgrad_h3(dy, a, None, amax, amax_b, dW, slices, nz):
+        return dW
+    if (dy_pl is not None or a_pl is not None) and planes_on(prec) and prec == "f32":
+        with _lib.timed("facl_gemm_wgrad %dx%dx%d%s" % (M, N, K, _LABEL[prec])):
+            _lib.check(lib.facl_gemm_wgrad_pl(_lib.ptr(dy), _lib.ptr(a), M, N, K, a.stride(0), _lib.ptr(dW), _lib.ptr(slices), nz,
+                                              _lib.stream(), _lib.ptr(dy_pl), _lib.ptr(a_pl)), "facl_gemm_wgrad_pl")
         return dW
     with _lib.timed("facl_gemm_wgrad %dx%dx%d%s" % (M, N, K, _LABEL[prec])):
         _lib.check(_fn(lib, "facl_gemm_wgrad", prec)(_lib.ptr(dy), _lib.ptr(a), M, N, K, a.stride(0), _lib.ptr(dW), _lib.ptr(slices), nz,
@@ -317,20 +357,27 @@
         B = M // G
         h = _lib.empty((M + B, Cin), dtype=torch.float32, device=x_pre.device)
         arg = _lib.empty((B, Cin), dtype=torch.int32, device=x_pre.device)
-        _lib.check(lib.facl_viewmax_stack(_lib.ptr(x_pre), G, B, Cin, _lib.ptr(h), _lib.ptr(arg), _lib.stream()), "facl_viewmax_stack")
-        _lib.tap("view_arg", arg)
         W1, W2 = W1.contiguous(), W2.contiguous()
         R, C = M + B, W1.shape[0]
         segs = ((0, M), (M, R))
         fused = _FC_FUSED and training and M % 32 == 0 and C % 4 == 0
         ctx.fused = fused
+        pl = fused and planes_on(ctx.prec)
+        w1_pl, w2_pl = take_weight_planes(W1), take_weight_planes(W2)
+        if not pl:
+            w1_pl = w2_pl = None
+        h_pl = planes_empty(R, Cin, x_pre.device) if pl else None
+        a_pl = planes_empty(R, C, x_pre.device) if pl else None
+        _lib.check(lib.facl_viewmax_stack_pl(_lib.ptr(x_pre), G, B, Cin, _lib.ptr(h), _lib.ptr(arg), _lib.stream(), _lib.ptr(h_pl)),
+                   "facl_viewmax_stack")
+        _lib.tap("view_arg", arg)
         if fused:
             f32 = dict(dtype=torch.float32, device=x_pre.device)
             world = 1 if reduce_fn is None else reduce_fn.world_size
             counts = [float(M) * world, float(B) * world]
             sums2 = part = None
             na = nb = 0
-            y = gemm_fwd(h, W1, b1, prec=ctx.prec)[0]
+            y = gemm_fwd(h, W1, b1, prec=ctx.prec, a_pl=h_pl, w_pl=w1_pl)[0]
             if reduce_fn is not None:
                 sums2 = _lib.empty((2, C, 2), dtype=torch.float64, device=y.device)
             _lib.check(lib.facl_fc_bn_stats(_lib.ptr(y), M, R, C, _lib.ptr(sums2), _lib.ptr(ws), _lib.stream()), "facl_fc_bn_stats")
@@ -340,10 +387,10 @@
                 part, na, nb = ws, M // 32, (B + 31) // 32
             a = _lib.empty_like(y)
             bnc2 = _lib.empty((2, 5, C), **f32)
-            _lib.check(lib.facl_fc_bn_apply(_lib.ptr(y), M, R, C, _lib.ptr(sums2), _lib.ptr(part), na, nb, counts[0], counts[1],
-                                            _lib.ptr(gamma.detach()), _lib.ptr(beta.detach()), BN_EPS, BN_MOMENTUM,
-                                            _lib.ptr(bn.running_mean), _lib.ptr(bn.running_var), _lib.ptr(bnc2), _lib.ptr(a),
-                                            _lib.stream()), "facl_fc_bn_apply")
+            _lib.check(lib.facl_fc_bn_apply_pl(_lib.ptr(y), M, R, C, _lib.ptr(sums2), _lib.ptr(part), na, nb, counts[0], counts[1],
+                                               _lib.ptr(gamma.detach()), _lib.ptr(beta.detach()), BN_EPS, BN_MOMENTUM,
+                                               _lib.ptr(bn.running_mean), _lib.ptr(bn.running_var), _lib.ptr(bnc2), _lib.ptr(a),
+                                               _lib.stream(), _lib.ptr(a_pl)), "facl_fc_bn_apply")
             bn.count_batch()
             bn.count_batch()
             bncs = [bnc2]
@@ -372,7 +419,8 @@
                 bncs.append(bnc)
                 counts.append(count)
         _lib.tap_relu("relu_fc", a=a)
-        out, _ = gemm_fwd(a, W2, b2, prec=ctx.prec)
+        out, _ = gemm_fwd(a, W2, b2, prec=ctx.prec, a_pl=a_pl, w_pl=w2_pl)
+        ctx.planes = (h_pl, a_pl, w1_pl, w2_pl)
         ctx.save_for_backward(h, W1, y, a, W2, arg, *bncs)
         ctx.segs, ctx.counts, ctx.reduce_fn, ctx.training, ctx.G = segs, counts, reduce_fn, training, G
         return out
@@ -392,15 +440,17 @@
         B = R - M
         dout = dout.contiguous()
         f32 = dict(dtype=torch.float32, device=y.device)
+        h_pl, a_pl, w1_pl, w2_pl = ctx.planes
+        dy_pl = planes_empty(R, C, y.device) if (ctx.fused and planes_on(bp) and bp == "f32") else None
         side = ctx.reduce_fn is None
         with _lib.fork(enabled=side) as f2:
-            dW2 = gemm_wgrad(dout, a, prec=bp)
+            dW2 = gemm_wgrad(dout, a, prec=bp, a_pl=a_pl)
             if dout.shape[1] % 4 == 0:
                 db2 = _lib.empty(dout.shape[1], **f32)
                 _lib.check(lib.facl_col_sums(_lib.ptr(dout), R, dout.shape[1], _lib.ptr(db2), _lib.stream()), "facl_col_sums")
             else:
                 db2 = dout.sum(0)
-        dact = gemm_dgrad(dout, W2, prec=bp)
+        dact = gemm_dgrad(dout, W2, prec=bp, w_pl=w2_pl)
         dy = _lib.empty_like(y)
         if ctx.fused:
             sums2 = sums2_g = None
@@ -411,9 +461,9 @@
             if ctx.reduce_fn is not None:
                 sums2_g = ctx.reduce_fn(sums2)
             dgamma, dbeta, kk2 = _lib.empty(C, **f32), _lib.empty(C, **f32), _lib.empty((2, 2, C), **f32)
-            _lib.check(lib.facl_fc_bn_bwd_apply(_lib.ptr(dact), _lib.ptr(y), M, R, C, _lib.ptr(bnc2), _lib.ptr(sums2_g), _lib.ptr(ws),
-                                                ctx.counts[0], ctx.counts[1], _lib.ptr(dgamma), _lib.ptr(dbeta), _lib.ptr(kk2),
-                                                _lib.ptr(dy), _lib.stream()), "facl_fc_bn_bwd_apply")
+            _lib.check(lib.facl_fc_bn_bwd_apply_pl(_lib.ptr(dact), _lib.ptr(y), M, R, C, _lib.ptr(bnc2), _lib.ptr(sums2_g), _lib.ptr(ws),
+                                                   ctx.counts[0], ctx.counts[1], _lib.ptr(dgamma), _lib.ptr(dbeta), _lib.ptr(kk2),
+                                                   _lib.ptr(dy), _lib.stream(), _lib.ptr(dy_pl)), "facl_fc_bn_bwd_apply")
         else:
             sums2 = _lib.empty((2, C, 2), dtype=torch.float64, device=y.device)
             for i, ((r0, r1), bnc) in enumerate(zip(ctx.segs, (bnc_a, bnc_b))):
@@ -428,8 +478,8 @@
                                                    _lib.ptr(kk[i]), _lib.ptr(dy[r0:r1]), _lib.stream()), "facl_rows_bwd_apply")
             dgamma, dbeta = dga[0] + dga[1], dbe[0] + dbe[1]
         with _lib.fork(enabled=side) as f1:
-            dW1 = gemm_wgrad(dy, h, prec=bp)
-        dh = gemm_dgrad(dy, W1, prec=bp)
+            dW1 = gemm_wgrad(dy, h, prec=bp, dy_pl=dy_pl, a_pl=h_pl)
+        dh = gemm_dgrad(dy, W1, prec=bp, dy_pl=dy_pl, w_pl=w1_pl)
         _lib.check(lib.facl_viewmax_bwd_add(dh[M:].data_ptr(), _lib.ptr(arg), ctx.G, B, dh.shape[1], _lib.ptr(dh), _lib.stream()),
                    "facl_viewmax_bwd_add")
         f2.join(dW2, db2)
@@ -532,6 +582,29 @@
     import ctypes
     lib = _lib.load_library()
     n = len(jobs)
+    ew = [w for w in getattr(_FC_PLANES, "req", [])
+          if w.dim() == 2 and w.is_contiguous() and w.shape[1] % 4 == 0 and w.dtype == torch.float32 and w.data_ptr() % 16 == 0][:4]
+    _FC_PLANES.req = []
+    if ew and GEMM_PLANES:
+        outs = []
+        for W, tr, xc, _h in jobs:
+            N, K = W.shape
+            nb = lib.facl_gemm_rs_planes_bytes(K if tr else N, N if tr else K, 0 if xc is None else 1)
+            outs.append(_lib.empty(nb, dtype=torch.uint8, device=W.device))
+        eouts = [planes_empty(w.shape[0], w.shape[1], w.device) for w in ew]
+        ne = len(ew)
+        vp, ip, evp, eip = ctypes.c_void_p * n, ctypes.c_int * n, ctypes.c_void_p * ne, ctypes.c_int * ne
+        _lib.check(lib.facl_gemm_rs_planes_multi_ew(
+            n, vp(*[j[0].data_ptr() for j in jobs]), ip(*[j[0].stride(0) for j in jobs]), ip(*[j[0].shape[0] for j in jobs]),
+            ip(*[j[0].shape[1] for j in jobs]), ip(*[1 if j[1] else 0 for j in jobs]),
+            vp(*[None if j[2] is None else j[2].data_ptr() for j in jobs]),
+            ip(*[0 if j[2] is None else j[2].stride(0) for j in jobs]), ip(*[1 if j[3] else 0 for j in jobs]),
+            vp(*[o.data_ptr() for o in outs]), None if absmax is None else _lib.ptr(absmax[0]),
+            0 if absmax is None else absmax[0].numel(), None if absmax is None else _lib.ptr(absmax[1]),
+            ne, evp(*[w.data_ptr() for w in ew]), eip(*[w.stride(0) for w in ew]), eip(*[w.shape[0] for w in ew]),
+            eip(*[w.shape[1] for w in ew]), evp(*[o.data_ptr() for o in eouts]), _lib.stream()), "facl_gemm_rs_planes_multi_ew")
+        _FC_PLANES.got = {(w.data_ptr(), tuple(w.shape)): o for w, o in zip(ew, eouts)}
+        return outs
     outs = []
     for W, tr, xc, _h in jobs:
         N, K = W.shape
diff --git a/include/facl_hip.h b/include/facl_hip.h
--- a/include/facl_hip.h
+++ b/include/facl_hip.h
@@ -135,6 +135,24 @@
 int facl_gemm_wgrad(const float* dy, const float* a, int64_t M, int N, int K, int lda, float* dW,
                     float* slices, int nz, void* stream);
 int facl_gemm_wgrad_acc(const float* dy, const float* a, int64_t M, int N, int K, int lda, float* dW, int prec, void* stream);
+int64_t facl_gemm_planes_bytes(int64_t R, int64_t C);
+int facl_gemm_fwd_pl(const float* a, int64_t M, int K, const float* W, int ldw, int N, const float* bias,
+                     const float* pscale, const float* pshift, const float* centers, const float* Wc,
+                     int ldwc, float* y, double* sums, void* ws, void* stream, const void* a_planes, const void* w_planes);
+int facl_gemm_dgrad_pl(const float* dy, int64_t M, int N, const float* W, int ldw, int K, float* da, void* stream,
+                       const void* dy_planes, const void* w_planes);
+int facl_gemm_wgrad_pl(const float* dy, const float* a, int64_t M, int N, int K, int lda, float* dW, float* slices, int nz,
+                       void* stream, const void* dy_planes, const void* a_planes);
+int facl_gemm_wgrad_acc_pl(const float* dy, const float* a, int64_t M, int N, int K, int lda, float* dW, int prec, void* stream,
+                           const void* dy_planes, const void* a_planes);
+int facl_viewmax_stack_pl(const float* x, int G, int B, int C, float* h, int32_t* arg, void* stream, void* h_planes);
+int facl_fc_bn_apply_pl(const float* y, int64_t M, int64_t R, int C, const double* sums2, const double* part, int nslices_a,
+                        int nslices_b, double count_a, double count_b, const float* gamma, const float* beta, float eps,
+                        float momentum, float* running_mean, float* running_var, float* bnc2, float* a_out, void* stream,
+                        void* a_planes);
+int facl_fc_bn_bwd_apply_pl(const float* dact, const float* y, int64_t M, int64_t R, int C, const float* bnc2,
+                            const double* sums2_g, const void* ws, double count_a, double count_b, float* dgamma, float* dbeta,
+                            float* kk2, float* dy, void* stream, void* dy_planes);
 int facl_gemm_fwd_f16(const float* a, int64_t M, int K, const float* W, int ldw, int N, const float* bias,
                       const float* pscale, const float* pshift, const float* centers, const float* Wc, int ldwc,
                       float* y, double* sums, void* ws, void* stream);
@@ -162,6 +180,11 @@
                               const int* transposed, const float* const* Wc, const int* ldwc, const int* half,
                               void* const* planes, const float* absmax_x, int64_t absmax_n, uint32_t* absmax_amax,
                               void* stream);
+int facl_gemm_rs_planes_multi_ew(int n, const float* const* W, const int* ldw, const int* N, const int* K,
+                                 const int* transposed, const float* const* Wc, const int* ldwc, const int* half,
+                                 void* const* planes, const float* absmax_x, int64_t absmax_n, uint32_t* absmax_amax,
+                                 int n_ew, const float* const* ew_W, const int* ew_ld, const int* ew_R, const int* ew_C,
+                                 void* const* ew_planes, void* stream);
 int facl_gemm_rs_supported(int64_t M, int K, int N);
 int facl_gemm_rs_fwd(const float* a, int64_t M, int K, const void* planes, int half, const uint32_t* amax_a, int N,
                      const float* bias, const float* pscale, const float* pshift, const float* centers, float* y, double* sums,
```

Result: no change. 10780, median of 3 (+0.0%).
